# mcan1999/vulkan-raytracing

Measured on AMD Instinct MI355X. Metric: Mrays/sec (primary+secondary) at 1920×1080 depth 4; 1/2/4/8-GPU scaling, higher is better.
Workload: dtype f32

## Files before the change

vulkan_raytracing_amd/api.py:

```python
import ctypes as C

import numpy as np

from . import _native

HIT_DTYPE = np.dtype([("t", np.float32), ("u", np.float32), ("v", np.float32), ("prim", np.int32), ("inst", np.int32)])
MESH_RANGE_DTYPE = np.dtype([("first_float", np.uint64), ("first_index", np.uint64), ("prim_count", np.uint32), ("reserved", np.uint32)])
INSTANCE_DTYPE = np.dtype([("transform", np.float32, 12), ("custom_index_and_mask", np.uint32), ("sbt_offset_and_flags", np.uint32), ("mesh", np.uint64)])
UNIFORMS_DTYPE = np.dtype([("position", np.float32, 4), ("right", np.float32, 4), ("up", np.float32, 4), ("forward", np.float32, 4),
                           ("light_position", np.float32, 3), ("light_intensity", np.float32),
                           ("max_bounce_count", np.uint32), ("samples_per_pixel", np.uint32),
                           ("center_object_type", np.uint32), ("orbiting_object_type", np.uint32),
                           ("orbiting_object_primitive_offset", np.uint32), ("orbiting_object_vertex_offset", np.uint32)])
MATERIAL_DTYPE = np.dtype([("ka", np.float32, 3), ("ns", np.float32), ("kd", np.float32, 3), ("ni", np.float32), ("ks", np.float32, 3), ("type", np.uint32)])
MATERIAL_TYPE_OF_INSTANCE = 0xFFFFFFFF
assert MATERIAL_DTYPE.itemsize == 48
NODEQ_DTYPE = np.dtype([("w", np.uint32, 6), ("child", np.int32, 2)])
TRI_PACKET_DTYPE = np.dtype([("v0", np.float32, 3), ("e1", np.float32, 3), ("e2", np.float32, 3), ("prim", np.uint32), ("pad", np.uint32, 2)])
INSTANCE_DEV_DTYPE = np.dtype([("w2o", np.float32, 12), ("o2w", np.float32, 12), ("blas_root", np.int32), ("mask", np.uint32), ("custom_index", np.int32),
                               ("first_float", np.uint32), ("first_index", np.uint32), ("blas_root4", np.int32), ("q_lo", np.float32, 3), ("q_scale", np.float32, 3),
                               ("type", np.uint32), ("cover_first", np.uint32), ("cover_count", np.uint32), ("pad", np.uint32)])
TLAS_MESH_DTYPE = np.dtype([("blas_root", np.int32), ("blas_root4", np.int32), ("first_float", np.uint32), ("first_index", np.uint32),
                            ("cover_first", np.uint32), ("cover_count", np.uint32), ("prim_count", np.uint32), ("built", np.uint32), ("levels", np.int32),
                            ("q_lo", np.float32, 3), ("q_scale", np.float32, 3), ("lo", np.float32, 3), ("hi", np.float32, 3)])
# ... 225 lines not shown
    def set_uniforms(self, uniforms):
        u = np.ascontiguousarray(uniforms, UNIFORMS_DTYPE).reshape(1)
        self._chk(self.L.rt_set_uniforms(self.h, _p(u)), "rt_set_uniforms")

    def set_skybox(self, faces):
        faces = [np.ascontiguousarray(f, np.uint8) for f in faces]
        assert len(faces) == 6
        h, w = faces[0].shape[:2]
        arr = (C.c_void_p * 6)(*[f.ctypes.data for f in faces])
        self._chk(self.L.rt_set_skybox(self.h, arr, w, h), "rt_set_skybox")

    def trace(self, W, H, counting=False):
        out = np.zeros((H, W, 4), np.uint8 if getattr(self, "_rgba8", False) else np.float32)
        st = RtStats()
        fn = self.L.rt_trace_counting if counting else self.L.rt_trace
        self._chk(fn(self.h, W, H, _p(out), C.byref(st)), "rt_trace")
        return out, st

    def shard_rows(self, H, band_rows, shard, n_shards):
        return self.L.rt_shard_rows(H, band_rows, shard, n_shards)

    def trace_async(self, W, H):
        self._chk(self.L.rt_trace_async(self.h, W, H), "rt_trace_async")
        self._async_shape = (H, W, 4)

    def trace_wait(self, copy=True):
        px = C.c_void_p()
        st = RtStats()
        self._chk(self.L.rt_trace_wait(self.h, C.byref(px), C.byref(st)), "rt_trace_wait")
        H, W, _ = self._async_shape
        ct = C.c_uint8 if getattr(self, "_rgba8", False) else C.c_float
        img = np.ctypeslib.as_array(C.cast(px, C.POINTER(ct)), shape=(H, W, 4))
        return (img.copy() if copy else img), st

    def trace_shard(self, W, H, band_rows, shard, n_shards, d_out_ptr, capacity_bytes, stream_ptr=None):
        self._chk(self.L.rt_trace_shard(self.h, W, H, band_rows, shard, n_shards, C.c_void_p(d_out_ptr), capacity_bytes,
                                        C.c_void_p(stream_ptr) if stream_ptr else None), "rt_trace_shard")

    def set_batch(self, instances, uniforms, update=False):
        inst = np.ascontiguousarray(instances, INSTANCE_DTYPE)
        u = np.ascontiguousarray(uniforms, UNIFORMS_DTYPE).reshape(-1)
        K = len(u)
        inst = inst.reshape(K, -1)
        self._chk(self.L.rt_set_batch(self.h, K, _p(inst), inst.shape[1], _p(u), int(update)), "rt_set_batch")

    def trace_shard_batch(self, W, H, band_rows, shard, n_shards, d_out_ptr, capacity_bytes, stream_ptr=None, frame_stride_bytes=0):
        self._chk(self.L.rt_trace_shard_batch(self.h, W, H, band_rows, shard, n_shards, C.c_void_p(d_out_ptr), frame_stride_bytes, capacity_bytes,
                                              C.c_void_p(stream_ptr) if stream_ptr else None), "rt_trace_shard_batch")

    def assemble_shards(self, d_gathered_ptr, n_shards, shard_stride_bytes, W, H, band_rows, d_frame_ptr, capacity_bytes, stream_ptr=None):
        self._chk(self.L.rt_assemble_shards(self.h, C.c_void_p(d_gathered_ptr), n_shards, shard_stride_bytes, W, H, band_rows, C.c_void_p(d_frame_ptr),
                                            capacity_bytes, C.c_void_p(stream_ptr) if stream_ptr else None), "rt_assemble_shards")

    def synchronize(self):
        self._chk(self.L.rt_synchronize(self.h), "rt_synchronize")

    def stats(self):
        st = RtStats()
        self._chk(self.L.rt_get_stats(self.h, C.byref(st)), "rt_get_stats")
        return st

    def debug_snapshot(self):
        info = np.zeros(SNAPSHOT_INFO_WORDS, np.uint64)
        self._chk(self.L.rt_debug_snapshot(self.h, 0, _p(info), info.nbytes, None), "rt_debug_snapshot")
        i = [int(x) for x in info]

        def item(what, n, dtype):
            a = np.zeros(n, dtype)
            got = C.c_size_t(0)
            self._chk(self.L.rt_debug_snapshot(self.h, what, _p(a) if n else _p(np.zeros(1, np.uint8)), a.nbytes, C.byref(got)), "rt_debug_snapshot")
            assert got.value == a.nbytes, (what, got.value, a.nbytes)
            return a

        bits = info[12:18].astype(np.uint32).view(np.float32)
        return {"n_blas_nodes": i[0], "tlas_base": i[1], "tlas_node_count": i[2], "tlas_stride": i[3], "batch_k": i[4], "inst_per_frame": i[7],
                "tlas_q_lo": bits[:3].copy(), "tlas_q_scale": bits[3:].copy(),
                "blas_nodes": item(1, i[0], NODEQ_DTYPE), "tlas_nodes": item(2, i[18], NODEQ_DTYPE), "packets": item(3, i[5], TRI_PACKET_DTYPE),
                "instances": item(4, i[6], INSTANCE_DEV_DTYPE), "meshes": item(5, i[8], TLAS_MESH_DTYPE), "verts": item(6, i[9], np.float32),
                "idx": item(7, i[10], np.uint32), "cover_boxes": item(8, 6 * i[11], np.float32).reshape(-1, 6)}

    def set_timing(self, on):
        self._chk(self.L.rt_set_timing(self.h, int(on)), "rt_set_timing")

    def set_param(self, name, value):
        self._chk(self.L.rt_set_param(self.h, name.encode(), int(value)), "rt_set_param")
        if name in ("output_rgba8", "output_bgra8"):
            self._rgba8 = bool(value)

    def intersect(self, rays8, any_hit=False, counting=False):
        rays8 = np.ascontiguousarray(rays8, np.float32).reshape(-1, 8)
        out = np.zeros(len(rays8), HIT_DTYPE)
        st = RtStats()
        self._chk(self.L.rt_intersect(self.h, len(rays8), _p(rays8), int(any_hit), _p(out), int(counting), C.byref(st)), "rt_intersect")
        return out, st

    def intersect_device(self, rays, any_hit=False, attributes=False, stream=None, out=None):
        def call(run, hits, attr):
            return self.L.rt_intersect_device(self.h, rays.shape[0], C.c_void_p(rays.data_ptr()), int(any_hit), C.c_void_p(hits.data_ptr()),
                                              C.c_void_p(attr.data_ptr()) if attr is not None else None, C.c_void_p(run.cuda_stream))
        hits, attr = self._device_query(rays, attributes, stream, out, (), call, "rt_intersect_device")
        return RayQuery(hits, attr)

    def intersect_device_flags(self, rays, ray_flags=0, cull_mask=0xFF, words=None, attributes=False, stream=None, out=None):
        import torch
        n = rays.shape[0] if isinstance(rays, torch.Tensor) else 0
        if words is not None:
            if not isinstance(words, torch.Tensor):
                raise TypeError("words must be a torch tensor, got %s" % type(words).__name__)
            if words.dtype not in (torch.int32, getattr(torch, "uint32", torch.int32)):
                raise ValueError("words must be int32 or uint32, not %s" % words.dtype)
            if words.device != getattr(rays, "device", None) or not words.is_contiguous() or tuple(words.shape) != (n,):
                raise ValueError("words must be a contiguous (n,) tensor on the rays' device")

        def call(run, hits, attr):
            return self.L.rt_intersect_device_flags(self.h, n, C.c_void_p(rays.data_ptr()), C.c_void_p(words.data_ptr()) if words is not None and n else None,
                                                    int(ray_flags) & 0xFFFFFFFF, int(cull_mask) & 0xFFFFFFFF, C.c_void_p(hits.data_ptr()),
                                                    C.c_void_p(attr.data_ptr()) if attr is not None else None, C.c_void_p(run.cuda_stream))
        hits, attr = self._device_query(rays, attributes, stream, out, (words,), call, "rt_intersect_device_flags")
        return RayQuery(hits, attr, hit_kind=True)

    def closest_point_device(self, points, cull_mask=0xFF, attributes=False, stream=None, out=None):
        def call(run, hits, attr):
            return self.L.rt_closest_point_device(self.h, points.shape[0], C.c_void_p(points.data_ptr()), int(cull_mask) & 0xFFFFFFFF, C.c_void_p(hits.data_ptr()),
                                                  C.c_void_p(attr.data_ptr()) if attr is not None else None, C.c_void_p(run.cuda_stream))
        hits, attr = self._device_query(points, attributes, stream, out, (), call, "rt_closest_point_device", cols=4)
        return RayQuery(hits, attr, hit_kind=True)

    def closest_point(self, points4, cull_mask=0xFF, counting=False):
        points4 = np.ascontiguousarray(points4, np.float32).reshape(-1, 4)
        out = np.zeros(len(points4), HIT_DTYPE)
        st = RtStats()
        self._chk(self.L.rt_closest_point(self.h, len(points4), _p(points4), int(cull_mask) & 0xFFFFFFFF, _p(out), int(counting), C.byref(st)), "rt_closest_point")
        return out, st

    def sweep_spheres_device(self, sweeps, cull_mask=0xFF, attributes=False, stream=None, out=None):
        def call(run, hits, attr):
            return self.L.rt_sweep_spheres_device(self.h, sweeps.shape[0], C.c_void_p(sweeps.data_ptr()), int(cull_mask) & 0xFFFFFFFF, C.c_void_p(hits.data_ptr()),
                                                  C.c_void_p(attr.data_ptr()) if attr is not None else None, C.c_void_p(run.cuda_stream))
        self._check_rays(sweeps, "sweep_spheres_device", 8, "sweep")
        hits, attr = self._device_query(sweeps, attributes, stream, out, (), call, "rt_sweep_spheres_device")
        return RayQuery(hits, attr, hit_kind=True)

    def sweep_spheres(self, sweeps8, cull_mask=0xFF, counting=False):
        sweeps8 = np.ascontiguousarray(sweeps8, np.float32).reshape(-1, 8)
        out = np.zeros(len(sweeps8), HIT_DTYPE)
        st = RtStats()
        self._chk(self.L.rt_sweep_spheres(self.h, len(sweeps8), _p(sweeps8), int(cull_mask) & 0xFFFFFFFF, _p(out), int(counting), C.byref(st)), "rt_sweep_spheres")
        return out, st

    def point_inside_device(self, points, n_dirs=3, cull_mask=0xFF, counts=False, stream=None, out=None):
        import torch
        self._check_rays(points, "point_inside_device", 4, "point")
        k = int(n_dirs)
        if k not in (1, 3, 5):
            raise ValueError("n_dirs must be 1, 3 or 5, got %d" % k)
        n = points.shape[0]
        cur = torch.cuda.current_stream(points.device)
        if stream is None:
            stream = cur
        shapes = ((n,), (n, k) if counts else None)
        if out is None:
            bufs = [torch.empty(sh, dtype=torch.int32, device=points.device) if sh is not None else None for sh in shapes]
            if stream != cur:
                for t in bufs:
                    if t is not None:
                        t.record_stream(stream)
# ... 322 lines not shown
```

vulkan_raytracing_amd/csrc/kernels.hip:

```cpp
#include <hip/hip_runtime.h>

#include "rt_kernels.h"
#include "../../include/rt_api.h"

namespace rt {

struct F3 { float x, y, z; };
__device__ __forceinline__ F3 mk3(float x, float y, float z) { F3 r; r.x = x; r.y = y; r.z = z; return r; }
__device__ __forceinline__ F3 add3(F3 a, F3 b) { return mk3(a.x + b.x, a.y + b.y, a.z + b.z); }
__device__ __forceinline__ F3 sub3(F3 a, F3 b) { return mk3(a.x - b.x, a.y - b.y, a.z - b.z); }
__device__ __forceinline__ F3 mul3(F3 a, float s) { return mk3(a.x * s, a.y * s, a.z * s); }
__device__ __forceinline__ F3 neg3(F3 a) { return mk3(-a.x, -a.y, -a.z); }
__device__ __forceinline__ float dot3(F3 a, F3 b) { return __builtin_fmaf(a.z, b.z, __builtin_fmaf(a.y, b.y, a.x * b.x)); }
__device__ __forceinline__ F3 cross3(F3 a, F3 b) {
  return mk3(__builtin_fmaf(a.y, b.z, -(a.z * b.y)), __builtin_fmaf(a.z, b.x, -(a.x * b.z)), __builtin_fmaf(a.x, b.y, -(a.y * b.x)));
}
__device__ __forceinline__ float length3(F3 v) { return __builtin_sqrtf(dot3(v, v)); }
__device__ __forceinline__ F3 normalize3(F3 v) { float inv = 1.0f / length3(v); return mul3(v, inv); }
__device__ __forceinline__ F3 fma3(float s, F3 a, F3 b) { return mk3(__builtin_fmaf(s, a.x, b.x), __builtin_fmaf(s, a.y, b.y), __builtin_fmaf(s, a.z, b.z)); }
__device__ __forceinline__ F3 reflect3(F3 I, F3 N) { float k = 2.0f * dot3(N, I); return fma3(-k, N, I); }

__device__ __forceinline__ F3 xform_point(const float* m, F3 p) {
  return mk3(__builtin_fmaf(m[2], p.z, __builtin_fmaf(m[1], p.y, m[0] * p.x)) + m[3],
             __builtin_fmaf(m[6], p.z, __builtin_fmaf(m[5], p.y, m[4] * p.x)) + m[7],
// ... 216 lines not shown
  }
  return true;
}

__device__ __forceinline__ float div255(float x) {
  const float rc = 0x1.010102p-8f;
  const float q = x * rc;
  const float r = __builtin_fmaf(-q, 255.0f, x);
  return __builtin_fmaf(r, rc, q);
}

struct SkyTap { int layer, x, y; };
__device__ __forceinline__ SkyTap sky_neighbour(int layer, int x, int y, int W) {
  const int S = 2 * x + 1 - W, T = 2 * y + 1 - W;
  int px, py, pz;
  switch (layer) {
    case 0: px = W; py = -T; pz = -S; break;
    case 1: px = -W; py = -T; pz = S; break;
    case 2: px = S; py = W; pz = T; break;
    case 3: px = S; py = -W; pz = -T; break;
    case 4: px = S; py = -T; pz = W; break;
    default: px = -S; py = -T; pz = -W; break;
  }
  const int ax = abs(px), ay = abs(py), az = abs(pz);
  int nl, sc, tc, ma;
  if (az >= ax && az >= ay) { ma = az; if (pz >= 0) { nl = 4; sc = px; tc = -py; } else { nl = 5; sc = -px; tc = -py; } }
  else if (ay >= ax)        { ma = ay; if (py >= 0) { nl = 2; sc = px; tc = pz; } else { nl = 3; sc = px; tc = -pz; } }
  else                      { ma = ax; if (px >= 0) { nl = 0; sc = -pz; tc = -py; } else { nl = 1; sc = pz; tc = -py; } }
  SkyTap t;
  t.layer = nl; t.x = min(((sc + ma) * W) / (2 * ma), W - 1); t.y = min(((tc + ma) * W) / (2 * ma), W - 1);
  return t;
}
constexpr uint32_t SKY_CORNER = 0xFFFFFFFFu;
__device__ __noinline__ uint32_t sky_tap_index(int layer, int x, int y, int W, int H) {
  const bool ox = x < 0 || x >= W, oy = y < 0 || y >= H;
  SkyTap t; t.layer = layer; t.x = x; t.y = y;
  if (W != H) { t.x = max(0, min(x, W - 1)); t.y = max(0, min(y, H - 1)); }
  else if (ox && oy) return SKY_CORNER;
  else if (ox || oy) t = sky_neighbour(layer, x, y, W);
  return ((uint32_t)t.layer * (uint32_t)H + (uint32_t)t.y) * (uint32_t)W + (uint32_t)t.x;
}

__device__ __forceinline__ F3 sample_sky(const SceneDev& sc, F3 r) {
  if (sc.sky_w == 0) return mk3(0.f, 0.f, 0.f);
  const float ax = __builtin_fabsf(r.x), ay = __builtin_fabsf(r.y), az = __builtin_fabsf(r.z);
  int layer; float s, t, ma;
  if (az >= ax && az >= ay) { ma = az; if (r.z >= 0.f) { layer = 4; s = r.x; t = -r.y; } else { layer = 5; s = -r.x; t = -r.y; } }
  else if (ay >= ax)        { ma = ay; if (r.y >= 0.f) { layer = 2; s = r.x; t = r.z; } else { layer = 3; s = r.x; t = -r.z; } }
  else                      { ma = ax; if (r.x >= 0.f) { layer = 0; s = -r.z; t = -r.y; } else { layer = 1; s = r.z; t = -r.y; } }
  const float fs = 0.5f * (s / ma + 1.0f), ft = 0.5f * (t / ma + 1.0f);
  const float u = fs * (float)sc.sky_w - 0.5f, v = ft * (float)sc.sky_h - 0.5f;
  const float fu0 = __builtin_floorf(u), fv0 = __builtin_floorf(v);
  const float wu = u - fu0, wv = v - fv0;
  const int W = sc.sky_w, H = sc.sky_h;
  int x0 = (int)fu0, y0 = (int)fv0;
  x0 = max(-1, min(x0, W - 1)); y0 = max(-1, min(y0, H - 1));
  uint32_t i00 = ((uint32_t)layer * (uint32_t)H + (uint32_t)y0) * (uint32_t)W + (uint32_t)x0, i10 = i00 + 1u, i01 = i00 + (uint32_t)W, i11 = i01 + 1u;
  const bool edge = !(x0 >= 0 && x0 + 1 < W && y0 >= 0 && y0 + 1 < H);
  if (edge) {
    i00 = sky_tap_index(layer, x0, y0, W, H); i10 = sky_tap_index(layer, x0 + 1, y0, W, H);
    i01 = sky_tap_index(layer, x0, y0 + 1, W, H); i11 = sky_tap_index(layer, x0 + 1, y0 + 1, W, H);
  }
  auto tap = [&](uint32_t i) -> uchar4 {
    if (RT_NT_STREAMS & 4) { const uint32_t w = __builtin_nontemporal_load(reinterpret_cast<const uint32_t*>(sc.sky) + i); uchar4 r; r.x = w & 255u; r.y = (w >> 8) & 255u; r.z = (w >> 16) & 255u; r.w = w >> 24; return r; }
    return sc.sky[i];
  };
  const uchar4 a = tap(i00 == SKY_CORNER ? 0u : i00), b = tap(i10 == SKY_CORNER ? 0u : i10);
  const uchar4 c = tap(i01 == SKY_CORNER ? 0u : i01), d = tap(i11 == SKY_CORNER ? 0u : i11);
  float c00x = (float)a.x, c00y = (float)a.y, c00z = (float)a.z, c10x = (float)b.x, c10y = (float)b.y, c10z = (float)b.z;
  float c01x = (float)c.x, c01y = (float)c.y, c01z = (float)c.z, c11x = (float)d.x, c11y = (float)d.y, c11z = (float)d.z;
  if (edge) {
    if (i00 == SKY_CORNER) { c00x = ((c10x + c01x) + c11x) / 3.0f; c00y = ((c10y + c01y) + c11y) / 3.0f; c00z = ((c10z + c01z) + c11z) / 3.0f; }
    if (i10 == SKY_CORNER) { c10x = ((c01x + c11x) + c00x) / 3.0f; c10y = ((c01y + c11y) + c00y) / 3.0f; c10z = ((c01z + c11z) + c00z) / 3.0f; }
    if (i01 == SKY_CORNER) { c01x = ((c11x + c00x) + c10x) / 3.0f; c01y = ((c11y + c00y) + c10y) / 3.0f; c01z = ((c11z + c00z) + c10z) / 3.0f; }
    if (i11 == SKY_CORNER) { c11x = ((c00x + c10x) + c01x) / 3.0f; c11y = ((c00y + c10y) + c01y) / 3.0f; c11z = ((c00z + c10z) + c01z) / 3.0f; }
  }
  const float iu = 1.0f - wu, iv = 1.0f - wv;
  float ra = __builtin_fmaf(c10x, wu, c00x * iu), rb = __builtin_fmaf(c11x, wu, c01x * iu);
  float ga = __builtin_fmaf(c10y, wu, c00y * iu), gb = __builtin_fmaf(c11y, wu, c01y * iu);
  float ba = __builtin_fmaf(c10z, wu, c00z * iu), bb = __builtin_fmaf(c11z, wu, c01z * iu);
  return mk3(div255(__builtin_fmaf(rb, wv, ra * iv)), div255(__builtin_fmaf(gb, wv, ga * iv)), div255(__builtin_fmaf(bb, wv, ba * iv)));
}

__device__ __forceinline__ void store_pixel(const FrameDev& f, uint32_t p, float4 px) {
  if (f.out_rgba8) {
    auto q = [](float v) -> unsigned char { v = fminf(fmaxf(v, 0.0f), 1.0f); return (unsigned char)(v * 255.0f + 0.5f); };
    reinterpret_cast<uchar4*>(f.out)[p] = f.out_rgba8 == 2 ? make_uchar4(q(px.z), q(px.y), q(px.x), q(px.w)) : make_uchar4(q(px.x), q(px.y), q(px.z), q(px.w));
  } else {
    f.out[p] = px;
  }
}
constexpr float PIXEL_DONE = 2.0f;

__global__ __launch_bounds__(256) void k_cover(SceneDev sc, CoverViews views, uint32_t* mask_block) {
  const CoverArgs& a = views.v[blockIdx.z];
  uint32_t* const mask = mask_block + a.mask_offset;
  const InstanceDev* I = sc.inst + a.inst_base + blockIdx.y;
  const uint32_t b = blockIdx.x * blockDim.x + threadIdx.x;
  if (b >= I->cover_count || (I->mask & 0xFFu) == 0u) return;
  const float* bx = sc.cover_boxes + 6u * (size_t)(I->cover_first + b);
  float x0 = 3e38f, x1 = -3e38f, y0 = 3e38f, y1 = -3e38f, az_min = 3e38f;
  bool all = false;
#pragma unroll
  for (int k = 0; k < 8; k++) {
    const F3 p = mk3(bx[(k & 1) ? 3 : 0], bx[(k & 2) ? 4 : 1], bx[(k & 4) ? 5 : 2]);
    const F3 w = xform_point(I->o2w, p);
    const F3 v = mk3(w.x - a.cam[0], w.y - a.cam[1], w.z - a.cam[2]);
    const float ax = a.inv[0] * v.x + a.inv[1] * v.y + a.inv[2] * v.z;
    const float ay = a.inv[3] * v.x + a.inv[4] * v.y + a.inv[5] * v.z;
    const float az = a.inv[6] * v.x + a.inv[7] * v.y + a.inv[8] * v.z;
    if (!(az > 1e-20f)) { all = true; continue; }
    az_min = fminf(az_min, az);
    const float ux = a.kf * ax / az, uy = a.kf * ay / az;
    const float px = (ux + 1.0f) * 0.5f * (float)a.width, py = (1.0f - uy) * 0.5f * (float)a.height;
    if (!(__builtin_fabsf(px) < 1e9f) || !(__builtin_fabsf(py) < 1e9f)) { all = true; continue; }
    x0 = fminf(x0, px); x1 = fmaxf(x1, px); y0 = fminf(y0, py); y1 = fmaxf(y1, py);
  }
  if (!all) {
    float mx = 1.0f + 1e-4f * (__builtin_fabsf(x0) + __builtin_fabsf(x1)), my = 1.0f + 1e-4f * (__builtin_fabsf(y0) + __builtin_fabsf(y1));
    if (a.apex_radius > 0.0f) {
      if (!(az_min > 4.0f * a.apex_radius)) all = true;
      else {
        const float g = a.apex_radius / (az_min - a.apex_radius) * 1.01f;
        const float uxm = fmaxf(__builtin_fabsf(2.0f * x0 / (float)a.width - 1.0f), __builtin_fabsf(2.0f * x1 / (float)a.width - 1.0f));
        const float uym = fmaxf(__builtin_fabsf(2.0f * y0 / (float)a.height - 1.0f), __builtin_fabsf(2.0f * y1 / (float)a.height - 1.0f));
        mx += g * (a.kf + uxm) * 0.5f * (float)a.width; my += g * (a.kf + uym) * 0.5f * (float)a.height;
      }
    }
    const int ix0 = (int)floorf(x0 - mx), ix1 = (int)floorf(x1 + mx), iy0 = (int)floorf(y0 - my), iy1 = (int)floorf(y1 + my);
    if (ix1 < 0 || iy1 < 0 || ix0 >= a.width || iy0 >= a.height) return;
    const int tx0 = max(ix0, 0) >> 3, tx1 = min(ix1, a.width - 1) >> 3, ty0 = max(iy0, 0) >> 3, ty1 = min(iy1, a.height - 1) >> 3;
    if ((tx1 - tx0 + 1) * (ty1 - ty0 + 1) > COVER_MAX_TILES) all = true;
    else {
      for (int ty = ty0; ty <= ty1; ty++) {
        const uint32_t t0 = (uint32_t)(ty * a.tiles_x + tx0), t1 = (uint32_t)(ty * a.tiles_x + tx1);
        for (uint32_t w = t0 >> 5; w <= (t1 >> 5); w++) {
          const uint32_t lo = w == (t0 >> 5) ? (t0 & 31u) : 0u, hi = w == (t1 >> 5) ? (t1 & 31u) : 31u;
          const uint32_t bits = (hi == 31u ? 0xFFFFFFFFu : ((1u << (hi + 1u)) - 1u)) & ~((1u << lo) - 1u);
          __hip_atomic_fetch_or(mask + 1u + w, bits, __ATOMIC_RELAXED, __HIP_MEMORY_SCOPE_AGENT);
        }
      }
    }
  }
  if (all) atomicOr(mask, 1u);
}

constexpr int REF_DONE = (int)0x80000000;
constexpr int REF_MARK = (int)0x80000001;

struct Plane5 {
  float nx[5], ny[5], nz[5], d[5], slack[5];
  F3 qs, qb; uint3 rot;
};

__device__ __forceinline__ void beam_world(const EntryArgs& e, float ux0, float ux1, float uy0, float uy1, float wn[5][3], float wd[5], float wmag[5]) {
  const float* ia = e.inv; const float* ib = e.inv + 3; const float* ic = e.inv + 6;
#pragma unroll
  for (int k = 0; k < 3; k++) {
    wn[0][k] = e.kf * ia[k] - ux0 * ic[k];
    wn[1][k] = ux1 * ic[k] - e.kf * ia[k];
    wn[2][k] = e.kf * ib[k] - uy0 * ic[k];
    wn[3][k] = uy1 * ic[k] - e.kf * ib[k];
    wn[4][k] = ic[k];
  }
#pragma unroll
  for (int j = 0; j < 5; j++) {
    wd[j] = -(wn[j][0] * e.cam[0] + wn[j][1] * e.cam[1] + wn[j][2] * e.cam[2]);
    wmag[j] = __builtin_fabsf(wn[j][0] * e.cam[0]) + __builtin_fabsf(wn[j][1] * e.cam[1]) + __builtin_fabsf(wn[j][2] * e.cam[2]);
  }
}
__device__ __forceinline__ void beam_fold(const float wn[5][3], const float wd[5], const float wmag[5], float apex_radius, const float* m, const float* q_lo, const float* q_scale, Plane5& P) {
#pragma unroll
  for (int j = 0; j < 5; j++) {
// ... 166 lines not shown
    const int wi = s_xw[grp][i]; const float ki = s_xk[grp][i];
    if (wi != ENTRY_FREE) { nb++; if (w != ENTRY_FREE && (ki < key || (ki == key && (uint32_t)i < sub))) rank++; }
  }
  if (!work) return;
  if (nb == 0) inst = ENTRY_NO_INST;
  if (nb == 0 && n_rest == 0) { if (sub == 0u) rec->w[0] = (int)ENTRY_EMPTY; return; }
  if (nb > 0) {
    if (w != ENTRY_FREE) rec->w[rank == 0 ? 1 : 2 + n_rest + 1 + (nb - 1 - rank)] = w;
    if (sub == 0u) {
#pragma unroll
      for (int i = 0; i < ENTRY_TLAS_CAP; i++) if (i < n_rest) rec->w[2 + (n_rest - 1 - i)] = rest[i];
      rec->w[2 + n_rest] = REF_MARK;
      rec->w[0] = (int)((uint32_t)(n_rest + nb) | ((uint32_t)(n_rest + 1) << 4) | (inst << 8));
    }
  } else if (sub == 0u) {
    rec->w[1] = rest[0];
#pragma unroll
    for (int i = 1; i < ENTRY_TLAS_CAP; i++) if (i < n_rest) rec->w[2 + (n_rest - 1 - i)] = rest[i];
    rec->w[0] = (int)((uint32_t)(n_rest - 1) | ((uint32_t)(n_rest - 1) << 4) | (ENTRY_NO_INST << 8));
  }
}

__device__ __forceinline__ float2 sample_uv(uint32_t x, uint32_t y, uint32_t i, uint32_t spp, int width, int height) {
  const float fx = (float)x, fy = (float)y;
  const float seed0 = (float)(spp + i), seed1 = seed0 + 0.5f;
  float ux = (fx + jitter_hash(fx, fy, seed0)) / (float)width;
  float uy = (fy + jitter_hash(fx, fy, seed1)) / (float)height;
  ux = __builtin_fmaf(ux, 2.0f, -1.0f);
  uy = -__builtin_fmaf(uy, 2.0f, -1.0f);
  return make_float2(ux, uy);
}
__device__ __forceinline__ uint32_t frame_row(const FrameDev& f, uint32_t ly) {
  if (f.n_shards == 1) return ly;
  const uint32_t band = ly / (uint32_t)f.band_rows, within = ly - band * (uint32_t)f.band_rows;
  return (band * (uint32_t)f.n_shards + (uint32_t)f.shard) * (uint32_t)f.band_rows + within;
}
__device__ __forceinline__ size_t jitter_index(uint32_t tile, uint32_t i, uint32_t spp, uint32_t lane) { return ((size_t)tile * spp + i) * 64u + lane; }

__device__ __forceinline__ bool tile_is_sky(const FrameDev& f, uint32_t fi, uint32_t tx, uint32_t by, uint32_t rec) {
  if (f.cover != nullptr) {
    const uint32_t* const cover = f.cover + (size_t)fi * f.cover_view_words;
    if (cover[0] == 0u) {
      uint32_t fty = by;
      if (f.n_shards != 1) {
        const uint32_t tiles_per_band = (uint32_t)f.band_rows >> 3;
        const uint32_t band = by / tiles_per_band, sub = by - band * tiles_per_band;
        fty = (band * (uint32_t)f.n_shards + (uint32_t)f.shard) * tiles_per_band + sub;
      }
      const uint32_t t = fty * (uint32_t)f.cover_tiles_x + tx;
      if (((cover[1u + (t >> 5)] >> (t & 31u)) & 1u) == 0u) return true;
    }
  }
  return f.entry != nullptr && (uint32_t)f.entry[rec].w[0] == ENTRY_EMPTY;
}

__global__ __launch_bounds__(256) void k_jitter_table(FrameDev f, uint32_t spp, float2* table) {
  const uint32_t lane = threadIdx.x;
  const uint32_t i = blockIdx.z * blockDim.y + threadIdx.y;
  const uint32_t x = blockIdx.x * 8u + (lane & 7u), ly = blockIdx.y * 8u + (lane >> 3);
  if (i >= spp) return;
  float2 uv = make_float2(0.f, 0.f);
  if (x < (uint32_t)f.width && ly < (uint32_t)f.rows) uv = sample_uv(x, frame_row(f, ly), i, spp, f.width, f.height);
  table[jitter_index(blockIdx.y * gridDim.x + blockIdx.x, i, spp, lane)] = uv;
}

__global__ __launch_bounds__(256) void k_raygen(SceneDev sc, FrameDev f, UniformsDev u, BatchTab bt) {
  const uint32_t spp = u.samples_per_pixel;
  const uint32_t lane = threadIdx.x;
  const uint32_t i = blockIdx.z * blockDim.y + threadIdx.y;
  const uint32_t x = blockIdx.x * 8u + (lane & 7u);
  uint32_t fi = 0, by = blockIdx.y;
  if (f.batch_k > 1) { const uint32_t tile_rows1 = ((uint32_t)f.rows + 7u) >> 3; fi = blockIdx.y / tile_rows1; by = blockIdx.y - fi * tile_rows1; }
  const uint32_t npx1 = (uint32_t)(f.rows * f.width);
  const uint32_t ly = by * 8u + (lane >> 3);
  const bool live = i < spp && x < (uint32_t)f.width && ly < (uint32_t)f.rows;
  const uint32_t tile = blockIdx.y * gridDim.x + blockIdx.x;
  const uint32_t tile1 = by * gridDim.x + blockIdx.x;
  const bool covered = !tile_is_sky(f, fi, blockIdx.x, by, tile);
  __shared__ float4 s_col[4][64];
  if (!covered) {
    F3 right = mk3(u.right[0], u.right[1], u.right[2]), up = mk3(u.up[0], u.up[1], u.up[2]), fwd = mk3(u.forward[0], u.forward[1], u.forward[2]);
    if (f.batch_k > 1) { right = mk3(bt.right[fi][0], bt.right[fi][1], bt.right[fi][2]); up = mk3(bt.up[fi][0], bt.up[fi][1], bt.up[fi][2]); fwd = mk3(bt.forward[fi][0], bt.forward[fi][1], bt.forward[fi][2]); }
    const uint32_t fy = frame_row(f, ly);
    const float nn = (float)spp;
    float r = 0.f, g = 0.f, b = 0.f, al = 0.f;
    if (gridDim.z == 1u) {
      float4 col = make_float4(0.f, 0.f, 0.f, 0.f);
      if (live) {
        const float2 uv = f.jitter != nullptr ? f.jitter[jitter_index(tile1, i, spp, lane)] : sample_uv(x, fy, i, spp, f.width, f.height);
        const F3 d = normalize3(fma3(2.5f, fwd, fma3(uv.y, up, mul3(right, uv.x))));
        const F3 c = sample_sky(sc, mk3(d.x, d.y, -d.z));
        col = make_float4(c.x, c.y, c.z, 1.0f);
      }
      s_col[threadIdx.y][lane] = col;
      __syncthreads();
      if (threadIdx.y != 0u || !live) return;
      for (uint32_t w = 0; w < blockDim.y; w++) { const float4 c = s_col[w][lane]; r += c.x; g += c.y; b += c.z; al += c.w; }
    } else {
      if (threadIdx.y != 0u || blockIdx.z != 0u || x >= (uint32_t)f.width || ly >= (uint32_t)f.rows) return;
      for (uint32_t k = 0; k < spp; k++) {
        const float2 uv = f.jitter != nullptr ? f.jitter[jitter_index(tile1, k, spp, lane)] : sample_uv(x, fy, k, spp, f.width, f.height);
        const F3 d = normalize3(fma3(2.5f, fwd, fma3(uv.y, up, mul3(right, uv.x))));
        const F3 c = sample_sky(sc, mk3(d.x, d.y, -d.z));
        r += c.x; g += c.y; b += c.z; al += 1.0f;
      }
    }
    store_pixel(f, fi * f.out_frame_stride + ly * (uint32_t)f.width + x, make_float4(r / nn, g / nn, b / nn, al / nn));
    return;
  }
#ifdef RT_ALT_KERNELS
  if (f.tile_blob != nullptr && covered && f.tile_blob[tile] != BLOB_NONE) return;
#endif
  bool survive = false;
  F3 d = mk3(0.f, 0.f, 1.f);
  uint32_t sid = 0;
  float4 miss_col = make_float4(0.f, 0.f, 0.f, 0.f);
  if (live) {
    const float2 uv = f.jitter != nullptr ? f.jitter[jitter_index(tile1, i, spp, lane)] : sample_uv(x, frame_row(f, ly), i, spp, f.width, f.height);
    const float ux = uv.x, uy = uv.y;
    F3 right = mk3(u.right[0], u.right[1], u.right[2]), up = mk3(u.up[0], u.up[1], u.up[2]), fwd = mk3(u.forward[0], u.forward[1], u.forward[2]);
    if (f.batch_k > 1) { right = mk3(bt.right[fi][0], bt.right[fi][1], bt.right[fi][2]); up = mk3(bt.up[fi][0], bt.up[fi][1], bt.up[fi][2]); fwd = mk3(bt.forward[fi][0], bt.forward[fi][1], bt.forward[fi][2]); }
    d = normalize3(fma3(2.5f, fwd, fma3(uy, up, mul3(right, ux))));
    sid = (fi * spp + i) * npx1 + ly * (uint32_t)f.width + x;
    {
      const F3 o = f.batch_k > 1 ? mk3(bt.position[fi][0], bt.position[fi][1], bt.position[fi][2]) : mk3(u.position[0], u.position[1], u.position[2]);
      F3 qs, qb; uint3 rot;
      quant_space(o, d, sc.tlas_q_lo, sc.tlas_q_scale, qs, qb, rot);
      const bool far = f.far_possible != 0 && quant_far(qs, qb);
      const uint4* rp = reinterpret_cast<const uint4*>(sc.blas_nodes + sc.tlas_root + (int)fi * sc.tlas_stride);
      const uint4 Q0 = rp[0], Q1 = rp[1];
      float tn;
      const bool h0 = far || slab_q(Q0.x, Q0.y, Q0.z, qs, qb, rot, 0.001f, 10000.0f, tn);
      const bool h1 = (far || slab_q(Q0.w, Q1.x, Q1.y, qs, qb, rot, 0.001f, 10000.0f, tn)) && Q1.w != Q1.z;
      const int c0 = (int)Q1.z, c1 = (int)Q1.w;
      survive = (h0 && c0 < 0) || (h1 && c1 < 0);
#pragma unroll
      for (int k = 0; k < 2; k++) {
        const int ch = k ? c1 : c0;
        if ((k ? h1 : h0) && ch >= 0 && !survive) {
          const uint4* np = reinterpret_cast<const uint4*>(sc.blas_nodes + ch);
          const uint4 N0 = np[0], N1 = np[1];
          survive = far || slab_q(N0.x, N0.y, N0.z, qs, qb, rot, 0.001f, 10000.0f, tn) || slab_q(N0.w, N1.x, N1.y, qs, qb, rot, 0.001f, 10000.0f, tn);
        }
      }
    }
    if (!survive) {
      const F3 c = sample_sky(sc, mk3(d.x, d.y, -d.z));
      miss_col = make_float4(c.x, c.y, c.z, 1.0f);
    }
  }
  const bool missed = live && !survive;
  const bool fuse = gridDim.z == 1u;
  __shared__ unsigned long long s_miss[4];
  if (fuse) {
    s_col[threadIdx.y][lane] = miss_col;
    const uint64_t mm = __ballot(missed);
    if (lane == 0) s_miss[threadIdx.y] = mm;
  } else if (missed) st_stream(&f.sample_color[sid], miss_col);
  const uint32_t shard = (blockIdx.x + gridDim.x * (blockIdx.y + gridDim.y * blockIdx.z)) & (N_SHARDS - 1);
  __shared__ uint32_t s_run[5];
  const uint64_t smask = __ballot(survive);
  if (lane == 0) s_run[threadIdx.y] = (uint32_t)__builtin_popcountll(smask);
  __syncthreads();
  if (threadIdx.x == 0 && threadIdx.y == 0) {
    uint32_t tot = 0;
    for (uint32_t w = 0; w < blockDim.y; w++) { const uint32_t c = s_run[w]; s_run[w] = tot; tot += c; }
    if (f.pixel_runs && tot) {
      const uint32_t run = 64u * blockDim.y;
      __hip_atomic_fetch_add(f.counters + cnt_tail(Q_DEAD, (int)shard), run - tot, __ATOMIC_RELAXED, __HIP_MEMORY_SCOPE_AGENT);
      tot = run;
    }
    s_run[4] = tot ? atomicAdd(f.counters + cnt_tail(0, (int)shard), tot) : 0u;
    if (f.pixel_runs && tot) {
      const F3 o = f.batch_k > 1 ? mk3(bt.position[fi][0], bt.position[fi][1], bt.position[fi][2]) : mk3(u.position[0], u.position[1], u.position[2]);
      f.ray_o[0][shard * f.shard_cap + s_run[4]] = make_float4(o.x, o.y, o.z, f.entry != nullptr ? __uint_as_float(tile) : 10000.0f);
    }
    s_run[0] = f.pixel_runs ? tot : s_run[0];
  }
  __syncthreads();
  const bool run_tile = f.pixel_runs && s_run[0] != 0u;
  const uint32_t slot = f.pixel_runs ? s_run[4] + 64u * threadIdx.y + lane : s_run[4] + s_run[threadIdx.y] + prefix_rank(smask);
  if (fuse) {
    bool all = true;
    for (uint32_t w = 0; w < blockDim.y; w++) all = all && ((s_miss[w] >> lane) & 1ull) != 0ull;
    if (all) {
      if (threadIdx.y == 0) {
        float r = 0.f, g = 0.f, b = 0.f, al = 0.f;
        for (uint32_t w = 0; w < blockDim.y; w++) { const float4 c = s_col[w][lane]; r += c.x; g += c.y; b += c.z; al += c.w; }
        const float nn = (float)spp;
        const uint32_t p = ly * (uint32_t)f.width + x;
        store_pixel(f, fi * f.out_frame_stride + p, make_float4(r / nn, g / nn, b / nn, al / nn));
        st_stream(&f.sample_color[fi * spp * npx1 + p], make_float4(0.f, 0.f, 0.f, PIXEL_DONE));
      }
    } else if (missed) st_stream(&f.sample_color[sid], miss_col);
  }
  if (survive || run_tile) {
    const uint32_t v = shard * f.shard_cap + slot;
    if (!f.pixel_runs) {
      const F3 o = f.batch_k > 1 ? mk3(bt.position[fi][0], bt.position[fi][1], bt.position[fi][2]) : mk3(u.position[0], u.position[1], u.position[2]);
      st_stream(&f.ray_o[0][v], make_float4(o.x, o.y, o.z, f.entry != nullptr ? __uint_as_float(tile) : 10000.0f));
    }
    st_stream(&f.ray_d[0][v], survive ? make_float4(d.x, d.y, d.z, __uint_as_float(sid)) : make_float4(0.f, 0.f, 0.f, __uint_as_float(SID_DEAD)));
  }
}

struct TraceArgs {
  SceneDev sc;
  const float4* ray_o;
  const float4* ray_d;
  const uint32_t* tails;
  uint32_t* work;
  uint32_t shard_cap;
  float4* hit_a;
  int32_t* hit_inst;
  const float4* sh_c;
  float4* sample_color;
  HitRec* raw_out;
  int32_t* ovf_stack;
  uint32_t* counters;
  union {
    float tmin;
    uint32_t query_word;
  };
  uint32_t rays_per_lane;
  uint32_t min_blocks;
  const EntryRec* entry;
  union {
    const uint32_t* sh_e;
    const uint32_t* ray_words;
  };
};

constexpr int MODE_CLOSEST = 0;
constexpr int MODE_SHADOW = 1;
constexpr int MODE_QUERY = 3;
constexpr int MODE_QUERY_FLAGS = 4;


#ifndef RT_REFILL_MIN
#define RT_REFILL_MIN 16
#endif
#ifndef RT_KEEP_NUM
#define RT_KEEP_NUM 5
#endif
#ifndef RT_INTERIOR_UNROLL
#define RT_INTERIOR_UNROLL 2
#endif
#ifndef RT_WIDE_UNROLL
#define RT_WIDE_UNROLL 1
#endif
#ifndef RT_WAVES_PER_EU
#define RT_WAVES_PER_EU 5
#endif
#ifndef RT_LEAF_CHAIN
#define RT_LEAF_CHAIN 1
#endif
#ifndef RT_STACK2_LDS
#define RT_STACK2_LDS 12
#endif
constexpr int STACK2_LDS = RT_STACK2_LDS;
constexpr uint32_t REFILL_MIN = RT_REFILL_MIN;

#ifdef RT_EXP_PHASE_SEL
#define PH_BEGIN(k) uint64_t ph_b##k = 0; if (COUNT && RT_EXP_PHASE_SEL == k) ph_b##k = __builtin_readcyclecounter();
#define PH_END(k) if (COUNT && RT_EXP_PHASE_SEL == k && lane == 0) { diag_iters++; diag_busy += __builtin_readcyclecounter() - ph_b##k; }
#else
#define PH_BEGIN(k)
#define PH_END(k)
#endif

template <int MODE, bool ANY, bool COUNT, bool WIDE, bool ENTRY = false, bool FAR = true, bool CONT = false>
__device__ __forceinline__ void trace_body(const TraceArgs& a) {
  constexpr bool RAYS8 = MODE == MODE_QUERY || MODE == MODE_QUERY_FLAGS;
  constexpr bool QF = MODE == MODE_QUERY_FLAGS;
  __shared__ int s_stack[4][STACK2_LDS + 1][64];
  __shared__ float4 s_rays[4][2][64];
  __shared__ float4 s_out[4][64];
  __shared__ int2 s_outq[4][64];
  __shared__ uint32_t s_ent[((ENTRY && MODE == MODE_SHADOW) || QF) ? 4 : 1][64];
  __shared__ float4 s_inst[LDS_INSTANCES ? LDS_INSTANCES : 1][5];
  {
    uint32_t total = 0;
#pragma unroll
    for (int t = 0; t < N_SHARDS; t++) total += ld_cursor(a.tails + t * CNT_STRIDE);
    uint32_t want = (total + 256u * a.rays_per_lane - 1u) / (256u * a.rays_per_lane);
    want = (want + (N_SHARDS - 1)) & ~(uint32_t)(N_SHARDS - 1);
    if (want < a.min_blocks) want = a.min_blocks;
    if (blockIdx.x >= want) return;
  }
  const int n_lds_inst = a.sc.n_inst < LDS_INSTANCES ? a.sc.n_inst : LDS_INSTANCES;
  if ((int)threadIdx.x < n_lds_inst) {
    const InstanceDev* I = a.sc.inst + threadIdx.x;
    const float4* mp = reinterpret_cast<const float4*>(I->w2o);
    s_inst[threadIdx.x][0] = mp[0]; s_inst[threadIdx.x][1] = mp[1]; s_inst[threadIdx.x][2] = mp[2];
    s_inst[threadIdx.x][3] = make_float4(I->q_lo[0], I->q_lo[1], I->q_lo[2], __int_as_float(I->blas_root));
    s_inst[threadIdx.x][4] = make_float4(I->q_scale[0], I->q_scale[1], I->q_scale[2], __uint_as_float(I->mask));
  }
  __syncthreads();
  const uint32_t lane = threadIdx.x & 63u, wave = threadIdx.x >> 6;
  int* const stk = &s_stack[wave][0][lane];
  int32_t* const ovf = a.ovf_stack + (size_t)(blockIdx.x * 256u + threadIdx.x) * a.sc.ovf_stride;
  uint64_t cnt_nodes = 0, cnt_tris = 0, diag_iters = 0, diag_busy = 0;
  const uint64_t diag_t0 = COUNT ? __builtin_readcyclecounter() : 0;

  uint32_t shard = blockIdx.x & (N_SHARDS - 1), tried = 0;
  uint32_t pf_base = 0, pf_count = 0;
  float4 pf_o = make_float4(0, 0, 0, 0), pf_d = pf_o;
  uint32_t pf_e = ENTRY_FROM_ROOT;
  uint32_t chunk_base = 0, chunk_count = 0, chunk_pos = 0;
  auto prefetch = [&]() {
    pf_count = 0;
    while (tried < (uint32_t)N_SHARDS) {
      const uint32_t size = ld_cursor(a.tails + shard * CNT_STRIDE);
      uint32_t off = 0;
      if (lane == 0 && size) off = atomicAdd(a.work + shard * CNT_STRIDE, 64u);
      off = (uint32_t)__builtin_amdgcn_readfirstlane((int)off);
      if (size && off < size) { pf_base = shard * a.shard_cap + off; pf_count = (size - off) < 64u ? (size - off) : 64u; break; }
      shard = (shard + 1u) & (N_SHARDS - 1); tried++;
    }
    if (lane < pf_count) {
      if constexpr (RAYS8) {
        const size_t r = 2u * (size_t)(pf_base + lane);
        pf_o = ld_stream(&a.ray_o[r]); pf_d = ld_stream(&a.ray_o[r + 1u]);
        if (QF) {
          const uint32_t w = a.ray_words ? (uint32_t)ld_stream(reinterpret_cast<const int*>(a.ray_words) + pf_base + lane) : 0xFF000000u;
          pf_e = ((a.query_word | w) & QF_FLAGS) | (a.query_word & w & 0xFF000000u);
        }
      } else {
        pf_o = ld_stream(&a.ray_o[pf_base + lane]); pf_d = ld_stream(&a.ray_d[pf_base + lane]);
      }
      if (ENTRY && MODE == MODE_SHADOW) pf_e = (uint32_t)ld_stream(reinterpret_cast<const int*>(a.sh_e) + pf_base + lane);
    }
  };
  auto promote = [&]() {
    s_rays[wave][0][lane] = pf_o; s_rays[wave][1][lane] = pf_d;
    if ((ENTRY && MODE == MODE_SHADOW) || QF) s_ent[wave][lane] = pf_e;
    chunk_base = pf_base; chunk_count = pf_count; chunk_pos = 0;
    prefetch();
  };
  prefetch();
  promote();

  uint32_t out_count = 0;
  auto flush = [&]() {
    if (lane < out_count) {
      const float4 r = s_out[wave][lane];
      const int2 k = s_outq[wave][lane];
      if (MODE == MODE_CLOSEST) { st_stream(&a.hit_a[k.x], r); st_stream(&a.hit_inst[k.x], k.y); }
      else if (MODE == MODE_SHADOW) {
        float cr = 0.08f, cg = 0.24f, cb = 0.08f;
        if (r.x != 0.0f || a.sc.n_materials != 0) {
          const float4 shc = ld_stream(&a.sh_c[(uint32_t)k.y]);
          if (r.x != 0.0f) { cr = shc.x; cg = shc.y; cb = shc.z; }
          else { const F3 amb = ambient_of(a.sc, __float_as_uint(shc.w)); cr = amb.x; cg = amb.y; cb = amb.z; }
        }
        st_stream(&a.sample_color[(uint32_t)k.x], make_float4(cr, cg, cb, 1.0f));
      }
      else { HitRec h; h.t = r.x; h.u = r.y; h.v = r.z; h.prim = (int)__float_as_uint(r.w); h.inst = k.y; a.raw_out[k.x] = h; }
    }
    out_count = 0;
  };

  bool need = true;
  uint32_t q = 0, sid = 0;
  float tmin_ray = 0.f, tmax = 0.f;
  uint32_t qword = 0;
  F3 wo = mk3(0, 0, 0), wd = mk3(0, 0, 1), co = wo, cd = wd, qs = mk3(1, 1, 1), qb = mk3(0, 0, 0);
  uint3 rot = make_uint3(0u, 0u, 0u);
  bool far = false;
  float best_t = 0.f, best_u = 0.f, best_v = 0.f;
  int best_prim = -1, best_inst = -1, cur_inst = -1, sp = 0, cur = REF_DONE;
  const char* const node_bytes = WIDE ? reinterpret_cast<const char*>(a.sc.wide_nodes) : reinterpret_cast<const char*>(a.sc.blas_nodes);

  auto push = [&](int v) {
    if (sp < STACK2_LDS) stk[sp * 64] = v;
    else *reinterpret_cast<volatile int32_t*>(ovf + (sp - STACK2_LDS)) = v;
    sp++;
  };
  auto pop = [&]() {
    sp--;
    if (sp < STACK2_LDS) cur = stk[sp * 64];
    else cur = *reinterpret_cast<volatile int32_t*>(ovf + (sp - STACK2_LDS));
  };

  auto to_instance = [&](int ii, int& root, uint32_t& imask) {
    float4 m0, m1, m2, ql, qsc;
    if (ii < n_lds_inst) { m0 = s_inst[ii][0]; m1 = s_inst[ii][1]; m2 = s_inst[ii][2]; ql = s_inst[ii][3]; qsc = s_inst[ii][4]; }
    else {
      const InstanceDev* I = a.sc.inst + ii;
      const float4* mp = reinterpret_cast<const float4*>(I->w2o);
      m0 = mp[0]; m1 = mp[1]; m2 = mp[2];
      ql = make_float4(I->q_lo[0], I->q_lo[1], I->q_lo[2], __int_as_float(I->blas_root));
      qsc = make_float4(I->q_scale[0], I->q_scale[1], I->q_scale[2], __uint_as_float(I->mask));
    }
    root = __float_as_int(ql.w); imask = __float_as_uint(qsc.w);
    if ((imask & 0xFFu) != 0u) {
      float m[12];
      m[0] = m0.x; m[1] = m0.y; m[2] = m0.z; m[3] = m0.w; m[4] = m1.x; m[5] = m1.y; m[6] = m1.z; m[7] = m1.w;
      m[8] = m2.x; m[9] = m2.y; m[10] = m2.z; m[11] = m2.w;
      co = xform_point(m, wo); cd = xform_vec(m, wd);
      const float qlo3[3] = {ql.x, ql.y, ql.z}, qsc3[3] = {qsc.x, qsc.y, qsc.z};
      quant_space(co, cd, qlo3, qsc3, qs, qb, rot); far = FAR && quant_far_o(co, qlo3, qsc3);
    }
  };

  for (;;) {
    PH_BEGIN(5)
    const uint64_t need_mask = __ballot(need);
    const uint32_t n_need = (uint32_t)__builtin_popcountll(need_mask);
    if (n_need >= REFILL_MIN || n_need == 64u) {
      if (chunk_pos == chunk_count && pf_count > 0) promote();
      if (chunk_pos < chunk_count) {
        const uint32_t rank = prefix_rank(need_mask);
        const uint32_t avail = chunk_count - chunk_pos;
        if (need && rank < avail) {
          const uint32_t ci = chunk_pos + rank;
          q = chunk_base + ci;
          const float4 ro = s_rays[wave][0][ci], rd = s_rays[wave][1][ci];
          if (RAYS8) { tmin_ray = ro.w; tmax = rd.w; }
          else { tmax = ro.w; sid = __float_as_uint(rd.w); }
          if (QF) qword = s_ent[wave][ci];
          wo = mk3(ro.x, ro.y, ro.z); wd = mk3(rd.x, rd.y, rd.z);
          co = wo; cd = wd;
          cur_inst = -1;
          stk[0] = REF_DONE;
          bool handed_on = false;
          if (CONT && (__float_as_uint(ro.w) & CONT_FLAG) != 0u) {
            handed_on = true;
            const uint32_t ent = __float_as_uint(ro.w);
            const uint32_t tile = ent & 0xFFFFFFu, mask = (ent >> 24) & 15u;
            const int4* rp = reinterpret_cast<const int4*>(a.entry + tile);
            const int4 r0 = rp[0], r1 = rp[1];
            const uint32_t n_rest = (((uint32_t)r0.x >> 4) & 15u) - 1u;
            const int wk[4] = {r0.z, r0.w, r1.x, r1.y};
            sp = 1;
#pragma unroll
            for (uint32_t k = 0; k < 4u; k++)
              if (k < n_rest && ((mask >> (n_rest - 1u - k)) & 1u) != 0u) { stk[sp * 64] = wk[k]; sp++; }
            sp--; cur = stk[sp * 64];
// ... 232 lines not shown
      } else {
        push(REF_MARK);
        cur_inst = ii; cur = root;
      }
    }

    PH_END(3)
    PH_BEGIN(4)
    const bool fin = !need && cur == REF_DONE;
    const uint64_t fin_mask = __ballot(fin);
    if (fin_mask != 0) {
      const uint32_t n_fin = (uint32_t)__builtin_popcountll(fin_mask);
      if (out_count + n_fin > 64u) flush();
      if (fin) {
        const uint32_t slot = out_count + prefix_rank(fin_mask);
        if (MODE == MODE_SHADOW) {
          s_out[wave][slot].x = best_inst < 0 ? 1.0f : 0.0f;
          s_outq[wave][slot] = make_int2((int)sid, (int)q);
        } else {
          s_out[wave][slot] = make_float4(best_t, best_u, best_v, __uint_as_float((uint32_t)best_prim));
          s_outq[wave][slot] = make_int2((int)q, best_inst);
        }
        need = true;
      }
      out_count += n_fin;
    }
    PH_END(4)
  }
  if (COUNT) {
    for (int off = 32; off > 0; off >>= 1) {
      cnt_nodes += __shfl_down((unsigned long long)cnt_nodes, off);
      cnt_tris += __shfl_down((unsigned long long)cnt_tris, off);
    }
    if (lane == 0) {
      const int off = ANY ? (CNT_NODE_VISITS_SH - CNT_NODE_VISITS) : 0;
      atomicAdd(reinterpret_cast<unsigned long long*>(a.counters + CNT_NODE_VISITS + off), (unsigned long long)cnt_nodes);
      atomicAdd(reinterpret_cast<unsigned long long*>(a.counters + CNT_TRI_TESTS + off), (unsigned long long)cnt_tris);
      const int dg = ANY ? CNT_DIAG_SH : CNT_DIAG;
      atomicAdd(reinterpret_cast<unsigned long long*>(a.counters + dg), (unsigned long long)diag_iters);
      atomicAdd(reinterpret_cast<unsigned long long*>(a.counters + dg + 2), (unsigned long long)diag_busy);
      atomicAdd(reinterpret_cast<unsigned long long*>(a.counters + dg + 4), (unsigned long long)(__builtin_readcyclecounter() - diag_t0));
    }
  }
}

template <int MODE, bool ANY, bool WIDE, bool ENTRY = false, bool FAR = true, bool CONT = false>
__global__ __launch_bounds__(256) __attribute__((amdgpu_waves_per_eu(RT_WAVES_PER_EU, RT_WAVES_PER_EU))) void k_trace(TraceArgs a) { trace_body<MODE, ANY, false, WIDE, ENTRY, FAR, CONT>(a); }
template <int MODE, bool ANY, bool WIDE, bool ENTRY = false, bool FAR = true, bool CONT = false>
__global__ __launch_bounds__(256) void k_trace_count(TraceArgs a) { trace_body<MODE, ANY, true, WIDE, ENTRY, FAR, CONT>(a); }

#ifdef RT_ALT_KERNELS
#include "kernels_alt.inc"
#include "kernels_tile.inc"
#endif

struct ShadeArgs {
  SceneDev sc;
  FrameDev f;
  UniformsDev u;
  int bounce;
  BatchTab bt;
};

struct Surface { F3 P, N; };
__device__ __forceinline__ Surface hit_surface(const SceneDev& sc, const InstanceDev* I, uint32_t prim, float hu, float hv) {
  const uint32_t* ix = sc.idx + I->first_index + 3u * prim;
  const uint32_t ia = ix[0], ib = ix[1], ic = ix[2];
  const float* vb = sc.verts + I->first_float;
  const float bx = (1.0f - hu) - hv, by = hu, bz = hv;
  const float* pa = vb + 6u * ia; const float* pb = vb + 6u * ib; const float* pc = vb + 6u * ic;
  const F3 pos = fma3(bz, mk3(pc[0], pc[1], pc[2]), fma3(by, mk3(pb[0], pb[1], pb[2]), mul3(mk3(pa[0], pa[1], pa[2]), bx)));
  const F3 nrm = fma3(bz, mk3(pc[3], pc[4], pc[5]), fma3(by, mk3(pb[3], pb[4], pb[5]), mul3(mk3(pa[3], pa[4], pa[5]), bx)));
  Surface s;
  s.P = xform_point(I->o2w, pos);
  s.N = normalize3(xform_normal(I->w2o, nrm));
  return s;
}

template <bool PIN> __device__ __forceinline__ float4 ambient_default() {
  float r = 0.08f;
  if constexpr (PIN) asm volatile("" : "+v"(r));
  return make_float4(r, 0.24f, r, 1.0f);
}
template <bool TILE, bool BATCH, bool RUNS, bool REG, typename A>
__device__ __forceinline__ void shade_slot(const A& a, const int bounce, const uint32_t shard, const uint32_t q, const bool in_range, const int inst_r, const float4 h_r) {
  const auto& f = a.f;
  const auto& U = a.u;
  const int cur = bounce & 1, nxt = cur ^ 1;
  const uint32_t lane = threadIdx.x & 63u;
  bool push_next = false, push_shadow = false, settled = false;
  F3 no = mk3(0, 0, 0), nd = mk3(0, 0, 1);
  float sh_tmax = 0.f; F3 sh_c = mk3(0, 0, 0); float sh_w = 0.f;
  uint32_t sh_ent = ENTRY_FROM_ROOT;
  uint32_t sid = SID_DEAD;
  int inst = HIT_DEAD;
  if (in_range) { if constexpr (REG) inst = inst_r; else inst = ld_stream(&f.hit_inst[q]); }
  if (inst != HIT_DEAD) {
    const float4 rd = ld_stream(&f.ray_d[cur][q]);
    sid = __float_as_uint(rd.w);
    const F3 d = mk3(rd.x, rd.y, rd.z);
    if (inst < 0) {
      const F3 c = sample_sky(a.sc, mk3(d.x, d.y, -d.z));
      st_stream(&f.sample_color[sid], make_float4(c.x, c.y, c.z, 1.0f));
    } else {
      float4 h = h_r;
      if constexpr (!REG) h = ld_stream(&f.hit_a[q]);
      const InstanceDev* I = a.sc.inst + inst;
      const uint32_t prim = __float_as_uint(h.w);
      const Surface S = hit_surface(a.sc, I, prim, h.y, h.z);
      const F3 P = S.P;
      F3 N = S.N;
      const int objectIndex = I->custom_index;
      uint32_t type = I->type != TYPE_BY_OBJECT_INDEX ? I->type : (objectIndex == 0 ? U.center_object_type : U.orbiting_object_type);
      const MaterialDev* M = nullptr;
      uint32_t mat = MATERIAL_NONE;
      if (a.sc.n_materials != 0) {
        mat = a.sc.prim_material[I->first_index / 3u + prim];
        M = a.sc.materials + mat;
        if (M->type != TYPE_BY_INSTANCE) type = M->type;
      }
      const bool last = (uint32_t)bounce >= U.max_bounce_count;
      if (type == 0u) {
        if (dot3(d, N) >= 0.0f) {
          st_stream(&f.sample_color[sid], ambient_default<REG>());
        } else {
          no = fma3(0.01f, N, P);
          F3 light = mk3(U.light_position[0], U.light_position[1], U.light_position[2]);
          float Iv = U.light_intensity;
          uint32_t fi = 0;
          if constexpr (BATCH) { fi = frame_of(sid, a.sc.batch_samples); light = mk3(a.bt.light[fi][0], a.bt.light[fi][1], a.bt.light[fi][2]); Iv = a.bt.light[fi][3]; }
          const F3 toL = sub3(light, P);
          const float dist = length3(toL);
          const F3 L = mul3(toL, 1.0f / dist);
          const F3 Hh = normalize3(add3(L, neg3(d)));
          const float NdotL = dot3(N, L), NdotH = dot3(N, Hh);
          const float dl = fmaxf(0.0f, NdotL);
          const float sp = M ? pow_int(fmaxf(0.0f, NdotH), (uint32_t)M->ns) : pow100(fmaxf(0.0f, NdotH));
          const uint32_t i = sid / (uint32_t)(f.rows * f.width) - fi * U.samples_per_pixel;
          float w = 1.0f;
          for (uint32_t k = 0; k < i; k++) w = w * 0.9f;
          const F3 kd = M ? mk3(M->kd[0], M->kd[1], M->kd[2]) : mk3(0.2f, 1.0f, 0.2f);
          const F3 ks = M ? mk3(M->ks[0], M->ks[1], M->ks[2]) : mk3(0.8f, 0.8f, 0.8f);
          const F3 diff = mk3((Iv * kd.x) * dl, (Iv * kd.y) * dl, (Iv * kd.z) * dl);
          const F3 spec = mk3((Iv * ks.x) * sp, (Iv * ks.y) * sp, (Iv * ks.z) * sp);
          const F3 amb = ambient_of(a.sc, mat);
          sh_c = fma3(w, add3(diff, spec), amb); sh_w = __uint_as_float(mat);
          nd = L; sh_tmax = dist;
          push_shadow = true;
          if (f.settle_dead_shadow_rays && __float_as_uint(sh_c.x) == __float_as_uint(amb.x) && __float_as_uint(sh_c.y) == __float_as_uint(amb.y) &&
              __float_as_uint(sh_c.z) == __float_as_uint(amb.z)) {
            st_stream(&f.sample_color[sid], make_float4(amb.x, amb.y, amb.z, 1.0f));
            push_shadow = false; settled = true;
          }
          if (f.light_entry != nullptr) {
            const F3 v = sub3(no, light);
            const float ax = __builtin_fabsf(v.x), ay = __builtin_fabsf(v.y), az = __builtin_fabsf(v.z);
            const int axis = (ax >= ay && ax >= az) ? 0 : (ay >= az ? 1 : 2);
            const float vc = axis == 0 ? v.x : (axis == 1 ? v.y : v.z), va = axis == 0 ? v.y : (axis == 1 ? v.z : v.x), vb = axis == 0 ? v.z : (axis == 1 ? v.x : v.y);
            const float c = __builtin_fabsf(vc);
            if (c > 0.0f) {
              const float T8 = (float)(8 * f.light_tiles);
              const float px = (va / c + 1.0f) * 0.5f * T8, py = (1.0f - vb / c) * 0.5f * T8;
              const int tx = min(max((int)(px * 0.125f), 0), f.light_tiles - 1), ty = min(max((int)(py * 0.125f), 0), f.light_tiles - 1);
              const int face = 2 * axis + (vc < 0.0f ? 1 : 0);
              sh_ent = (uint32_t)((face * f.light_tiles + ty) * f.light_tiles + tx) | (NdotL < 0.0f ? ENTRY_REVERSE : 0u);
            }
          }
        }
      } else if (type == 1u) {
        no = fma3(0.01f, N, P);
        nd = reflect3(d, N);
        push_next = true;
      } else if (type == 2u) {
        float ndoti = dot3(d, N);
        const bool outwards = ndoti > 0.0f;
        if (outwards) { N = neg3(N); ndoti = -ndoti; }
        const float ratio = M ? (outwards ? M->ni : 1.0f / M->ni) : (outwards ? 1.52f : (1.0f / 1.52f));
        const float k = 1.0f - (ratio * ratio) * (1.0f - ndoti * ndoti);
        if (k < 0.0f) { nd = reflect3(d, N); no = fma3(0.01f, N, P); }
        else {
          const float c = __builtin_fmaf(ratio, ndoti, __builtin_sqrtf(k));
          nd = normalize3(fma3(-c, N, mul3(d, ratio)));
          no = fma3(-0.01f, N, P);
        }
        push_next = true;
      } else {
        if (bounce == 0 && f.pixel_runs) {
          no = mk3(U.position[0], U.position[1], U.position[2]);
          if constexpr (BATCH) { const uint32_t fk = frame_of(sid, a.sc.batch_samples); no = mk3(a.bt.position[fk][0], a.bt.position[fk][1], a.bt.position[fk][2]); }
        } else {
          const float4 ro = ld_stream(&f.ray_o[cur][q]);
          no = mk3(ro.x, ro.y, ro.z);
        }
        nd = d; push_next = true;
      }
      if (push_next && last) {
        push_next = false;
        st_stream(&f.sample_color[sid], ambient_default<REG>());
      }
    }
  }
  {
    const uint64_t m_st = __ballot(settled);
    if (lane == 0 && m_st != 0ull) {
      __hip_atomic_fetch_add(f.counters + cnt_tail(Q_SHADOW0, (int)shard), (uint32_t)__builtin_popcountll(m_st), __ATOMIC_RELAXED, __HIP_MEMORY_SCOPE_AGENT);
      __hip_atomic_fetch_add(f.counters + cnt_work(Q_DEAD, (int)shard), (uint32_t)__builtin_popcountll(m_st), __ATOMIC_RELAXED, __HIP_MEMORY_SCOPE_AGENT);
    }
  }
  const uint32_t slot_n = wave_alloc(push_next, f.counters + cnt_tail(bounce + 1, (int)shard));
  if (push_next) {
    const uint32_t v = shard * f.shard_cap + slot_n;
    st_stream(&f.ray_o[nxt][v], make_float4(no.x, no.y, no.z, 10000.0f));
    st_stream(&f.ray_d[nxt][v], make_float4(nd.x, nd.y, nd.z, __uint_as_float(sid)));
  }
  if constexpr (RUNS) {
    if (in_range) {
      if (push_shadow) {
        st_stream(&f.sh_o[q], make_float4(no.x, no.y, no.z, sh_tmax));
        st_stream(&f.sh_c[q], make_float4(sh_c.x, sh_c.y, sh_c.z, sh_w));
        if (f.sh_e != nullptr) f.sh_e[q] = sh_ent;
      }
      st_stream(&f.sh_d[q], push_shadow ? make_float4(nd.x, nd.y, nd.z, __uint_as_float(sid)) : make_float4(0.f, 0.f, 0.f, __uint_as_float(SID_DEAD)));
    }
    const uint64_t m_sh = __ballot(push_shadow);
    if (lane == 0 && m_sh != 0ull) __hip_atomic_fetch_add(f.counters + cnt_tail(Q_SHADOW0, (int)shard), (uint32_t)__builtin_popcountll(m_sh), __ATOMIC_RELAXED, __HIP_MEMORY_SCOPE_AGENT);
  } else {
    const uint32_t slot_s = wave_alloc(push_shadow, f.counters + cnt_tail(Q_SHADOW, (int)shard));
    if (push_shadow) {
      const uint32_t v = f.sh_base + shard * f.shard_cap + slot_s;
      st_stream(&f.sh_o[v], make_float4(no.x, no.y, no.z, sh_tmax));
      st_stream(&f.sh_d[v], make_float4(nd.x, nd.y, nd.z, __uint_as_float(sid)));
      st_stream(&f.sh_c[v], make_float4(sh_c.x, sh_c.y, sh_c.z, sh_w));
      if (f.sh_e != nullptr) f.sh_e[v] = sh_ent;
    }
  }
}

template <bool TILE = false, bool BATCH = false, bool RUNS = false>
__device__ __forceinline__ void shade_body(const ShadeArgs& a, const int bounce) {
  const FrameDev& f = a.f;
  const UniformsDev& U = a.u;
  const uint32_t lane = threadIdx.x & 63u, wave = threadIdx.x >> 6;
  const int n_pass = TILE ? 2 : 1;
  for (int pass = 0; pass < n_pass; pass++) {
  uint32_t cnt[N_SHARDS], maxb = 0;
#pragma unroll
  for (int t = 0; t < N_SHARDS; t++) {
    if (TILE && pass) {
      uint32_t blobs = 0;
#pragma unroll
      for (int k = 0; k < BLOB_CLASSES; k++) blobs += ld_cursor(f.counters + cnt_tail(Q_BLOB_LIST + k, t));
      cnt[t] = blobs * (256u * ((U.samples_per_pixel + 3u) / 4u));
    } else cnt[t] = ld_cursor(f.counters + cnt_tail(bounce, t));
    maxb = max(maxb, (cnt[t] + 63u) >> 6);
  }
  const uint32_t n_waves = gridDim.x * 4u;
  for (uint32_t g = blockIdx.x * 4u + wave; g < maxb * N_SHARDS; g += n_waves) {
    const uint32_t shard = g & (N_SHARDS - 1), base = (g >> 3) << 6;
    uint32_t n = 0;
#pragma unroll
    for (int t = 0; t < N_SHARDS; t++) n = (shard == (uint32_t)t) ? cnt[t] : n;
    if (base >= n) continue;
    const uint32_t q = shard * f.shard_cap + ((TILE && pass) ? f.shard_cap - n : 0u) + base + lane;
    shade_slot<TILE, BATCH, RUNS, false>(a, bounce, shard, q, base + lane < n, HIT_DEAD, make_float4(0.f, 0.f, 0.f, 0.f));
  }
  }
}

template <bool TILE, bool BATCH, bool RUNS = false>
__global__ __launch_bounds__(256) void k_shade(ShadeArgs a) { shade_body<TILE, BATCH, RUNS>(a, a.bounce); }

#include "kernels_beam.inc"

struct TailArgs {
  TraceArgs tr;
  ShadeArgs sh;
  uint32_t first_bounce;
  uint32_t* barrier;
  uint32_t* fault;
};

__device__ __forceinline__ void grid_barrier(uint32_t* bar, uint32_t* fault, uint32_t& phase) {
  __syncthreads();
  phase++;
  if (threadIdx.x == 0) {
    __threadfence();
    const uint32_t target = phase * gridDim.x;
    __hip_atomic_fetch_add(bar, 1u, __ATOMIC_RELAXED, __HIP_MEMORY_SCOPE_AGENT);
    uint32_t spins = 0;
    while (__hip_atomic_load(bar, __ATOMIC_RELAXED, __HIP_MEMORY_SCOPE_AGENT) < target) {
      __builtin_amdgcn_s_sleep(8);
      if (++spins > (1u << 24)) { __hip_atomic_store(fault, 1u, __ATOMIC_RELAXED, __HIP_MEMORY_SCOPE_AGENT); break; }
    }
    __threadfence();
  }
  __syncthreads();
}

template <bool COUNT, bool WIDE, bool BATCH = false>
__global__ __launch_bounds__(256) void k_tail(TailArgs t) {
  uint32_t phase = 0;
  const uint32_t max_bounce = t.sh.u.max_bounce_count;
  for (uint32_t b = t.first_bounce; b <= max_bounce; b++) {
    uint32_t live = 0;
#pragma unroll
    for (int k = 0; k < N_SHARDS; k++) live += ld_cursor(t.tr.counters + cnt_tail((int)b, k));
    if (live == 0 || ld_cursor(t.fault) != 0u) break;
    TraceArgs a = t.tr;
    a.ray_o = t.sh.f.ray_o[b & 1u]; a.ray_d = t.sh.f.ray_d[b & 1u];
    a.tails = t.tr.counters + cnt_tail((int)b, 0);
    a.work = t.tr.counters + cnt_work((int)b, 0);
    trace_body<MODE_CLOSEST, false, COUNT, WIDE>(a);
    grid_barrier(t.barrier, t.fault, phase);
    if (ld_cursor(t.fault) != 0u) return;
    shade_body<false, BATCH>(t.sh, (int)b);
    grid_barrier(t.barrier, t.fault, phase);
    if (ld_cursor(t.fault) != 0u) return;
  }
}

__global__ __launch_bounds__(256) void k_resolve(FrameDev f, UniformsDev u) {
  const uint32_t npx1 = (uint32_t)(f.rows * f.width);
  const uint32_t lane = threadIdx.x & 63u, wave = (uint32_t)__builtin_amdgcn_readfirstlane((int)(threadIdx.x >> 6));
  const uint32_t tile_rows1 = ((uint32_t)f.rows + 7u) >> 3;
  const uint32_t trow = blockIdx.y * 4u + wave;
  if (trow < tile_rows1 * (uint32_t)f.batch_k) {
    const uint32_t fi = f.batch_k > 1 ? trow / tile_rows1 : 0u, by = trow - fi * tile_rows1;
    const uint32_t x = blockIdx.x * 8u + (lane & 7u), ly = by * 8u + (lane >> 3);
    if (!tile_is_sky(f, fi, blockIdx.x, by, trow * gridDim.x + blockIdx.x) && x < (uint32_t)f.width && ly < (uint32_t)f.rows) {
      const uint32_t p1 = ly * (uint32_t)f.width + x;
      const size_t s0 = (size_t)fi * u.samples_per_pixel * npx1 + p1;
      if (f.sample_color[s0].w != PIXEL_DONE) {
        float r = 0.f, g = 0.f, b = 0.f, al = 0.f;
        for (uint32_t i = 0; i < u.samples_per_pixel; i++) {
          const float4 c = ld_stream(&f.sample_color[s0 + (size_t)i * npx1]);
          r += c.x; g += c.y; b += c.z; al += c.w;
        }
        const float nn = (float)u.samples_per_pixel;
        store_pixel(f, fi * f.out_frame_stride + p1, make_float4(r / nn, g / nn, b / nn, al / nn));
      }
    }
  }
  const uint32_t p = (blockIdx.y * gridDim.x + blockIdx.x) * blockDim.x + threadIdx.x, n_threads = gridDim.x * gridDim.y * blockDim.x;
  if (f.counters_next)
    for (uint32_t i = p; i < (uint32_t)CNT_WORDS; i += n_threads) f.counters_next[i] = 0u;
  if (f.cover_next)
    for (uint32_t i = p; i < f.cover_words; i += n_threads) f.cover_next[i] = 0u;
  if (blockIdx.x == 0 && blockIdx.y == 0 && f.stats_out) {
    __shared__ unsigned long long s_q[N_QUEUES];
    const uint32_t t = threadIdx.x;
    if (t < (uint32_t)N_QUEUES) {
      unsigned long long n = 0;
      for (int k = 0; k < N_SHARDS; k++) n += ld_cursor(f.counters + cnt_tail((int)t, k));
      s_q[t] = n;
    }
    __syncthreads();
    if (f.hint && t >= 1u && t < (uint32_t)CNT_MAX_BOUNCES)
      __hip_atomic_store(f.hint + t, (uint32_t)(s_q[t] > 0xFFFFFFFFull ? 0xFFFFFFFFull : s_q[t]), __ATOMIC_RELAXED, __HIP_MEMORY_SCOPE_SYSTEM);
    auto cnt64 = [&](int word) { return (unsigned long long)ld_cursor(f.counters + word) | ((unsigned long long)ld_cursor(f.counters + word + 1) << 32); };
    if (t < (uint32_t)STAT_WORDS) {
      unsigned long long v = 0;
      if (t == STAT_QUEUE0) { v = s_q[0] + s_q[Q_TILE_RAYS] - s_q[Q_DEAD]; for (int k = 0; k < N_SHARDS; k++) v -= ld_cursor(f.counters + cnt_work(Q_TILE_RAYS, k)); }
      else if (t == STAT_TILE_RAYS) v = s_q[Q_TILE_RAYS];
      else if (t == STAT_CONT_RAYS) { for (int k = 0; k < N_SHARDS; k++) v += ld_cursor(f.counters + cnt_work(Q_TILE_RAYS, k)); }
      else if (t >= STAT_BLOB && t < STAT_BLOB + 5) v = ld_cursor(f.counters + CNT_BLOB_STATS + (int)(t - STAT_BLOB));
      else if (t >= STAT_TILE_DIAG && t < STAT_TILE_DIAG + 6) v = cnt64(CNT_TILE_DIAG + 2 * (int)(t - STAT_TILE_DIAG));
      else if (t == STAT_SECONDARY) { for (uint32_t b = 1; b <= u.max_bounce_count && b < (uint32_t)CNT_MAX_BOUNCES; b++) v += s_q[b]; }
      else if (t == STAT_SHADOW) v = s_q[Q_SHADOW] + s_q[Q_SHADOW0];
      else if (t == STAT_SHADOW_UNTRACED) { for (int k = 0; k < N_SHARDS; k++) v += ld_cursor(f.counters + cnt_work(Q_DEAD, k)); }
      else if (t == STAT_QUEUE1) v = s_q[1];
      else if (t == STAT_FAULT) v = ld_cursor(f.counters + CNT_FAULT);
      else if (t == STAT_FAULT_TOTAL) {
        uint32_t total = f.fault_total ? f.fault_total[0] : 0u;
        if (f.fault_total && ld_cursor(f.counters + CNT_FAULT) != 0u) { total++; f.fault_total[0] = total; }
        v = total;
      }
      else if (t == STAT_NODE_VISITS) v = cnt64(CNT_NODE_VISITS);
      else if (t == STAT_TRI_TESTS) v = cnt64(CNT_TRI_TESTS);
      else if (t == STAT_NODE_VISITS_SH) v = cnt64(CNT_NODE_VISITS_SH);
      else if (t == STAT_TRI_TESTS_SH) v = cnt64(CNT_TRI_TESTS_SH);
      else if (t >= STAT_DIAG && t < STAT_DIAG + 3) v = cnt64(CNT_DIAG + 2 * (int)(t - STAT_DIAG));
      else if (t >= STAT_DIAG + 3 && t < STAT_DIAG + 6) v = cnt64(CNT_DIAG_SH + 2 * (int)(t - STAT_DIAG - 3));
      __hip_atomic_store(f.stats_out + t, v, __ATOMIC_RELAXED, __HIP_MEMORY_SCOPE_SYSTEM);
    }
  }
}

int trace_threads_per_block() { return 256; }

static dim3 raygen_grid(int width, int rows, uint32_t spp, int batch_k, dim3& block) {
  const uint32_t wpb = spp < 4u ? spp : 4u;
  block = dim3(64, wpb);
  return dim3(((uint32_t)width + 7u) >> 3, (((uint32_t)rows + 7u) >> 3) * (uint32_t)batch_k, (spp + wpb - 1u) / wpb);
}
size_t raygen_block_count(int width, int rows, uint32_t spp, int batch_k) {
  dim3 b; const dim3 g = raygen_grid(width, rows, spp, batch_k, b);
  return (size_t)g.x * g.y * g.z;
}
void launch_raygen(const SceneDev& sc, const FrameDev& f, const UniformsDev& u, const BatchTab& bt, hipStream_t s) {
  dim3 b; const dim3 g = raygen_grid(f.width, f.rows, u.samples_per_pixel, f.batch_k, b);
  hipLaunchKernelGGL(k_raygen, g, b, 0, s, sc, f, u, bt);
}
size_t jitter_table_elems(int width, int rows, uint32_t spp) {
  return (size_t)(((uint32_t)width + 7u) >> 3) * (size_t)(((uint32_t)rows + 7u) >> 3) * spp * 64u;
}
void launch_jitter_table(const FrameDev& f, uint32_t spp, float2* table, hipStream_t s) {
  dim3 b; const dim3 g = raygen_grid(f.width, f.rows, spp, 1, b);
  hipLaunchKernelGGL(k_jitter_table, g, b, 0, s, f, spp, table);
}

void launch_cover(const SceneDev& sc, const CoverViews& a, uint32_t max_boxes_per_instance, uint32_t* mask_block, hipStream_t s) {
  if (a.n <= 0 || a.v[0].n_inst <= 0 || max_boxes_per_instance == 0) return;
  hipLaunchKernelGGL(k_cover, dim3((max_boxes_per_instance + 255u) / 256u, (unsigned)a.v[0].n_inst, (unsigned)a.n), dim3(256), 0, s, sc, a, mask_block);
}

static TraceArgs make_args(const SceneDev& sc, uint32_t* counters, int queue, uint32_t shard_cap, int32_t* ovf) {
  TraceArgs a{};
  a.sc = sc;
  a.tmin = 0.001f;
  a.counters = counters;
  a.tails = counters + cnt_tail(queue, 0);
  a.work = counters + cnt_work(queue, 0);
// ... 16 lines not shown
  }
  if (cfg.variant == 1) {
    if (counting) hipLaunchKernelGGL((k_trace4<MODE, ANY, true>), g, b, 0, s, a);
    else hipLaunchKernelGGL((k_trace4<MODE, ANY, false>), g, b, 0, s, a);
    return;
  }
#endif
  if (counting) hipLaunchKernelGGL((k_trace_count<MODE, ANY, false>), g, b, 0, s, a);
  else if constexpr (MODE == MODE_QUERY) hipLaunchKernelGGL((k_trace<MODE, ANY, false, false, true>), g, b, 0, s, a);
  else if (cfg.far) hipLaunchKernelGGL((k_trace<MODE, ANY, false, false, true>), g, b, 0, s, a);
  else hipLaunchKernelGGL((k_trace<MODE, ANY, false, false, false>), g, b, 0, s, a);
}

bool alt_kernels_built() {
#ifdef RT_ALT_KERNELS
  return true;
#else
  return false;
#endif
}

void launch_trace_closest(const SceneDev& sc, const FrameDev& f, int bounce, bool counting, const LaunchCfg& cfg, hipStream_t s) {
  TraceArgs a = make_args(sc, f.counters, bounce, f.shard_cap, f.ovf_stack);
  a.ray_o = f.ray_o[bounce & 1]; a.ray_d = f.ray_d[bounce & 1];
  a.hit_a = f.hit_a; a.hit_inst = f.hit_inst;
#ifdef RT_ALT_KERNELS
  if (bounce == 0 && cfg.packet != 0 && cfg.variant == 0) {
    a.entry = f.entry;
    a.rays_per_lane = (uint32_t)cfg.rays_per_lane; a.min_blocks = (uint32_t)cfg.min_blocks;
    const dim3 g(cfg.packet_blocks), b(256);
    if (f.entry != nullptr) {
      if (counting) hipLaunchKernelGGL((k_packet<MODE_CLOSEST, false, true, true>), g, b, 0, s, a);
      else hipLaunchKernelGGL((k_packet<MODE_CLOSEST, false, false, true>), g, b, 0, s, a);
    } else {
      if (counting) hipLaunchKernelGGL((k_packet<MODE_CLOSEST, false, true, false>), g, b, 0, s, a);
      else hipLaunchKernelGGL((k_packet<MODE_CLOSEST, false, false, false>), g, b, 0, s, a);
    }
    return;
  }
#endif
  if (bounce == 0 && f.pixel_runs && cfg.variant == 0) {
    a.entry = f.entry;
    const dim3 g(cfg.trace_blocks), b(256);
    if (counting) hipLaunchKernelGGL(k_beam_count, g, b, 0, s, a, (uint32_t)f.pixel_runs);
    else hipLaunchKernelGGL(k_beam, g, b, 0, s, a, (uint32_t)f.pixel_runs);
    return;
  }
  if (bounce == 0 && f.entry != nullptr && cfg.variant == 0) {
    a.entry = f.entry;
    a.rays_per_lane = (uint32_t)cfg.rays_per_lane; a.min_blocks = (uint32_t)cfg.min_blocks;
    const dim3 g(cfg.trace_blocks), b(256);
#ifdef RT_ALT_KERNELS
    if (f.tile_blob != nullptr) {
      if (counting) hipLaunchKernelGGL((k_trace_count<MODE_CLOSEST, false, false, true, false, true>), g, b, 0, s, a);
      else hipLaunchKernelGGL((k_trace<MODE_CLOSEST, false, false, true, false, true>), g, b, 0, s, a);
      return;
    }
#endif
    if (counting) hipLaunchKernelGGL((k_trace_count<MODE_CLOSEST, false, false, true>), g, b, 0, s, a);
    else if (cfg.far) hipLaunchKernelGGL((k_trace<MODE_CLOSEST, false, false, true, true>), g, b, 0, s, a);
    else hipLaunchKernelGGL((k_trace<MODE_CLOSEST, false, false, true, false>), g, b, 0, s, a);
    return;
  }
  launch_trace<MODE_CLOSEST, false>(a, counting, cfg, s);
}

void launch_beam_shade(const SceneDev& sc, const FrameDev& f, const UniformsDev& u, const LaunchCfg& cfg, hipStream_t s) {
  BeamShadeArgs a{};
  a.sc = sc;
  a.ray_o = f.ray_o[0]; a.ray_d = f.ray_d[0];
  a.tails = f.counters + cnt_tail(0, 0); a.work = f.counters + cnt_work(0, 0);
  a.shard_cap = f.shard_cap; a.ovf_stack = f.ovf_stack; a.counters = f.counters;
  a.tmin = 0.001f;
  a.entry = f.entry;
  a.next_o = f.ray_o[1]; a.next_d = f.ray_d[1];
  a.sh_o = f.sh_o; a.sh_d = f.sh_d; a.sh_c = f.sh_c; a.sh_e = f.sh_e;
  a.sample_color = f.sample_color;
  a.light_entry = f.light_entry;
  a.width = f.width; a.rows = f.rows; a.light_tiles = f.light_tiles; a.settle_dead_shadow_rays = f.settle_dead_shadow_rays;
  for (int k = 0; k < 3; k++) { a.u.position[k] = u.position[k]; a.u.light_position[k] = u.light_position[k]; }
  a.u.light_intensity = u.light_intensity;
  a.u.max_bounce_count = u.max_bounce_count; a.u.samples_per_pixel = u.samples_per_pixel;
  a.u.center_object_type = u.center_object_type; a.u.orbiting_object_type = u.orbiting_object_type;
  hipLaunchKernelGGL(k_beam_shade, dim3(cfg.trace_blocks), dim3(256), 0, s, a, (uint32_t)f.pixel_runs);
}

void launch_entry(const SceneDev& sc, const EntryViews& a, hipStream_t s) {
  uint32_t n = 0;
  for (int v = 0; v < a.n; v++) n = max(n, (uint32_t)(a.v[v].tiles_x * a.v[v].tile_rows));
  if (n == 0) return;
  hipLaunchKernelGGL(k_entry, dim3((n + 7u) / 8u, (unsigned)a.n), dim3(64), 0, s, sc, a);
}

void launch_trace_shadow(const SceneDev& sc, const FrameDev& f, bool counting, const LaunchCfg& cfg, hipStream_t s) {
  TraceArgs a = make_args(sc, f.counters, Q_SHADOW, f.shard_cap, f.ovf_stack);
  a.ray_o = f.sh_o + f.sh_base; a.ray_d = f.sh_d + f.sh_base; a.sh_c = f.sh_c + f.sh_base;
  a.sample_color = f.sample_color;
#ifdef RT_ALT_KERNELS
  if (cfg.packet != 0 && cfg.variant == 0) {
    const bool le = f.light_entry != nullptr && f.sh_e != nullptr;
    a.entry = le ? f.light_entry : nullptr; a.sh_e = le ? f.sh_e + f.sh_base : nullptr;
    a.rays_per_lane = (uint32_t)cfg.rays_per_lane; a.min_blocks = (uint32_t)cfg.min_blocks;
    const dim3 g(cfg.packet_blocks), b(256);
    if (le) {
      if (counting) hipLaunchKernelGGL((k_packet<MODE_SHADOW, true, true, true>), g, b, 0, s, a);
      else hipLaunchKernelGGL((k_packet<MODE_SHADOW, true, false, true>), g, b, 0, s, a);
    } else {
      if (counting) hipLaunchKernelGGL((k_packet<MODE_SHADOW, true, true, false>), g, b, 0, s, a);
      else hipLaunchKernelGGL((k_packet<MODE_SHADOW, true, false, false>), g, b, 0, s, a);
    }
    return;
  }
#endif
  if (f.light_entry != nullptr && f.sh_e != nullptr && cfg.variant == 0) {
    a.entry = f.light_entry; a.sh_e = f.sh_e + f.sh_base;
    a.rays_per_lane = (uint32_t)cfg.rays_per_lane; a.min_blocks = (uint32_t)cfg.min_blocks;
    const dim3 g(cfg.trace_blocks), b(256);
    if (counting) hipLaunchKernelGGL((k_trace_count<MODE_SHADOW, true, false, true>), g, b, 0, s, a);
    else if (cfg.far) hipLaunchKernelGGL((k_trace<MODE_SHADOW, true, false, true, true>), g, b, 0, s, a);
    else hipLaunchKernelGGL((k_trace<MODE_SHADOW, true, false, true, false>), g, b, 0, s, a);
    return;
  }
  launch_trace<MODE_SHADOW, true>(a, counting, cfg, s);
}

#ifdef RT_ALT_KERNELS
void launch_blob(const SceneDev& sc, const EntryArgs& e, const FrameDev& f, bool counting, hipStream_t s) {
  const uint32_t n = (uint32_t)(e.tiles_x * e.tile_rows);
  if (n == 0 || f.tile_blob == nullptr) return;
  BlobArgs a{sc, e, f.tile_blob, f.blob_arena, f.blob_slots / N_SHARDS, f.blob_list, f.counters};
  if (counting) hipLaunchKernelGGL((k_blob<true>), dim3(n), dim3(64), 0, s, a);
  else hipLaunchKernelGGL((k_blob<false>), dim3(n), dim3(64), 0, s, a);
}

template <int CLS>
static void launch_tile_class(const TileArgs& t, uint32_t blocks, bool counting, hipStream_t s) {
  if (counting) hipLaunchKernelGGL((k_tile<CLS, true>), dim3(blocks), dim3(256), 0, s, t);
  else hipLaunchKernelGGL((k_tile<CLS, false>), dim3(blocks), dim3(256), 0, s, t);
}
void launch_tile(const SceneDev& sc, const FrameDev& f, const UniformsDev& u, bool counting, hipStream_t s) {
  if (f.tile_blob == nullptr) return;
  TileArgs t{};
  t.sc = sc; t.f = f; t.u = u; t.sub_slots = f.blob_slots / N_SHARDS; t.tmin = 0.001f;
  const uint32_t blocks = f.blob_slots / N_SHARDS * N_SHARDS;
  launch_tile_class<0>(t, blocks, counting, s);
  launch_tile_class<1>(t, blocks, counting, s);
  launch_tile_class<2>(t, blocks, counting, s);
}

void launch_beam_shadow(const SceneDev& sc, const FrameDev& f, const UniformsDev& u, bool counting, const LaunchCfg& cfg, hipStream_t s) {
  if (!f.shadow_runs || !f.pixel_runs) return;
  BeamShadowArgs A{};
  A.t = make_args(sc, f.counters, 0, f.shard_cap, f.ovf_stack);
  A.t.work = f.counters + cnt_work(Q_SHADOW0, 0);
  A.t.ray_o = f.sh_o; A.t.ray_d = f.sh_d; A.t.sh_c = f.sh_c; A.t.sample_color = f.sample_color;
  const bool le = f.light_entry != nullptr && f.sh_e != nullptr;
  A.t.entry = le ? f.light_entry : nullptr; A.t.sh_e = le ? f.sh_e : nullptr;
  for (int k = 0; k < 3; k++) A.light[k] = u.light_position[k];
  A.run = (uint32_t)f.pixel_runs;
  const dim3 g(cfg.trace_blocks), b(256);
  if (counting) hipLaunchKernelGGL(k_beam_shadow_count, g, b, 0, s, A);
  else hipLaunchKernelGGL(k_beam_shadow, g, b, 0, s, A);
}
#else
void launch_blob(const SceneDev&, const EntryArgs&, const FrameDev&, bool, hipStream_t) {}
void launch_tile(const SceneDev&, const FrameDev&, const UniformsDev&, bool, hipStream_t) {}
void launch_beam_shadow(const SceneDev&, const FrameDev&, const UniformsDev&, bool, const LaunchCfg&, hipStream_t) {}
#endif

__global__ __launch_bounds__(64) void k_query_init(uint32_t* counters, uint32_t n) {
  const uint32_t t = threadIdx.x;
  if (t < (uint32_t)N_SHARDS) { counters[cnt_tail(0, (int)t)] = t == 0u ? n : 0u; counters[cnt_work(0, (int)t)] = 0u; }
}

void launch_query(const SceneDev& sc, const float4* rays, HitRec* out, uint32_t n, int32_t* ovf_stack, uint32_t* counters, bool any_hit,
                  bool counting, const LaunchCfg& cfg, hipStream_t s) {
  hipLaunchKernelGGL(k_query_init, dim3(1), dim3(64), 0, s, counters, n);
  TraceArgs a = make_args(sc, counters, 0, n, ovf_stack);
  a.ray_o = rays; a.raw_out = out;
#ifdef RT_ALT_KERNELS
// ... 226 lines not shown
```

vulkan_raytracing_amd/csrc/kernels_beam.inc:

```
struct BeamSpace { F3 s0, b0, s1, b1; uint3 rot; };

__device__ __forceinline__ bool slab_beam(uint32_t wx, uint32_t wy, uint32_t wz, const BeamSpace& B, float tmin, float tlim, float& tn) {
  wx = __builtin_amdgcn_alignbit(wx, wx, B.rot.x); wy = __builtin_amdgcn_alignbit(wy, wy, B.rot.y); wz = __builtin_amdgcn_alignbit(wz, wz, B.rot.z);
  const float nx = (float)(wx & 0xFFFFu), fx = (float)(wx >> 16), ny = (float)(wy & 0xFFFFu), fy = (float)(wy >> 16), nz = (float)(wz & 0xFFFFu), fz = (float)(wz >> 16);
  const float x0 = fminf(__builtin_fmaf(nx, B.s0.x, B.b0.x), __builtin_fmaf(nx, B.s1.x, B.b1.x)), x1 = fmaxf(__builtin_fmaf(fx, B.s0.x, B.b0.x), __builtin_fmaf(fx, B.s1.x, B.b1.x));
  const float y0 = fminf(__builtin_fmaf(ny, B.s0.y, B.b0.y), __builtin_fmaf(ny, B.s1.y, B.b1.y)), y1 = fmaxf(__builtin_fmaf(fy, B.s0.y, B.b0.y), __builtin_fmaf(fy, B.s1.y, B.b1.y));
  const float z0 = fminf(__builtin_fmaf(nz, B.s0.z, B.b0.z), __builtin_fmaf(nz, B.s1.z, B.b1.z)), z1 = fmaxf(__builtin_fmaf(fz, B.s0.z, B.b0.z), __builtin_fmaf(fz, B.s1.z, B.b1.z));
  tn = fmaxf(fmaxf(x0, y0), fmaxf(z0, tmin));
  const float tf = fminf(fminf(x1, y1), fminf(z1, tlim));
  return tn <= tf * 1.00002f;
}
__device__ __forceinline__ void beam_axis(float lo, float hi, float da, float t_far, float q_lo_minus_o, float q_scale, float& s0, float& b0, float& s1, float& b1, uint32_t& rot) {
  if (lo < 0.0f && hi > 0.0f) {
    const float K = 1.0e30f, inv = 1.0f / q_scale, r = t_far * da;
    const float U = (r - q_lo_minus_o) * inv + 1.0f, L = (-r - q_lo_minus_o) * inv - 1.0f;
    s0 = K; s1 = K; b0 = -K * U; b1 = -K * L; rot = 0u;
  }
  else { s0 = q_scale * lo; b0 = q_lo_minus_o * lo; s1 = q_scale * hi; b1 = q_lo_minus_o * hi; rot = lo < 0.0f ? 16u : 0u; }
}

#define RT_BEAM_EACH(M) M(0) M(1) M(2) M(3)
#ifndef RT_BEAM_KEEP_NUM
#define RT_BEAM_KEEP_NUM RT_KEEP_NUM
#endif
#ifndef RT_BEAM_UNROLL
#define RT_BEAM_UNROLL RT_INTERIOR_UNROLL
#endif

struct BeamShadeUniforms {
  float position[3], light_position[3], light_intensity;
  uint32_t max_bounce_count, samples_per_pixel, center_object_type, orbiting_object_type;
};
struct BeamShadeArgs {
  SceneDev sc;
  const float4* ray_o;
  const float4* ray_d;
  const uint32_t* tails;
  uint32_t* work;
  uint32_t shard_cap;
  int32_t* ovf_stack;
  uint32_t* counters;
  float tmin;
  const EntryRec* entry;
  float4* next_o;
  float4* next_d;
  float4* sh_o;
  float4* sh_d;
  float4* sh_c;
  uint32_t* sh_e;
  float4* sample_color;
  const EntryRec* light_entry;
  int width, rows, light_tiles, settle_dead_shadow_rays;
  BeamShadeUniforms u;
};
struct BeamShadeFrame {
  float4* ray_o[2]; float4* ray_d[2];
  float4* sh_o; float4* sh_d; float4* sh_c; uint32_t* sh_e;
  float4* sample_color;
  uint32_t* counters;
  const EntryRec* light_entry;
  uint32_t shard_cap;
  int width, rows, light_tiles, settle_dead_shadow_rays;
  static constexpr int pixel_runs = 64;
  static constexpr uint32_t sh_base = 0u;
};
struct BeamShadeView { const SceneDev& sc; const BeamShadeFrame& f; const BeamShadeUniforms& u; };

template <bool COUNT, bool SHADE = false, typename Args = TraceArgs>
__device__ __forceinline__ void beam_body(const Args& a, const uint32_t run) {
  __shared__ int s_stack[4][STACK2_LDS + 1][64];
  __shared__ float s_best[4][16][64];
  __shared__ float4 s_inst[LDS_INSTANCES ? LDS_INSTANCES : 1][5];
  const int n_lds_inst = a.sc.n_inst < LDS_INSTANCES ? a.sc.n_inst : LDS_INSTANCES;
  if ((int)threadIdx.x < n_lds_inst) {
    const InstanceDev* I = a.sc.inst + threadIdx.x;
    const float4* mp = reinterpret_cast<const float4*>(I->w2o);
    s_inst[threadIdx.x][0] = mp[0]; s_inst[threadIdx.x][1] = mp[1]; s_inst[threadIdx.x][2] = mp[2];
    s_inst[threadIdx.x][3] = make_float4(I->q_lo[0], I->q_lo[1], I->q_lo[2], __int_as_float(I->blas_root));
    s_inst[threadIdx.x][4] = make_float4(I->q_scale[0], I->q_scale[1], I->q_scale[2], __uint_as_float(I->mask));
  }
  __syncthreads();
  const uint32_t lane = threadIdx.x & 63u, wave = threadIdx.x >> 6;
  int* const stk = &s_stack[wave][0][lane];
  float* const bst = &s_best[wave][0][lane];
  const char* const node_bytes = reinterpret_cast<const char*>(a.sc.blas_nodes);
  const uint32_t S = run >> 6;
  uint64_t cnt_nodes = 0, cnt_tris = 0, diag_iters = 0, diag_busy = 0;
  const uint64_t diag_t0 = COUNT ? __builtin_readcyclecounter() : 0;
  uint32_t shard = blockIdx.x & (N_SHARDS - 1), tried = 0;

  for (;;) {
    uint32_t base = 0; bool got = false;
    while (tried < (uint32_t)N_SHARDS) {
      const uint32_t size = ld_cursor(a.tails + shard * CNT_STRIDE);
      uint32_t off = 0;
      if (lane == 0 && size) off = atomicAdd(a.work + shard * CNT_STRIDE, run);
      off = (uint32_t)__builtin_amdgcn_readfirstlane((int)off);
      if (size && off < size) { base = shard * a.shard_cap + off; got = true; break; }
      shard = (shard + 1u) & (N_SHARDS - 1); tried++;
    }
    if (!got) break;
    const uint32_t v0 = base + lane;

    uint32_t alive = 0, sid = 0;
    F3 co = mk3(0, 0, 0), cd0 = mk3(0, 0, 1), cd1 = cd0, cd2 = cd0, cd3 = cd0;
    float bt0 = -1.0f, bt1 = -1.0f, bt2 = -1.0f, bt3 = -1.0f;
    BeamSpace B;
    B.s0 = B.s1 = B.b0 = B.b1 = mk3(0, 0, 0); B.rot = make_uint3(0u, 0u, 0u);
    int cur = REF_DONE, sp = 1, cur_inst = -1;
    uint32_t my_visits = 0;

    auto push = [&](int v) {
      if (sp < STACK2_LDS) stk[sp * 64] = v;
      else *reinterpret_cast<volatile int32_t*>(a.ovf_stack + (size_t)(blockIdx.x * 256u + threadIdx.x) * a.sc.ovf_stride + (sp - STACK2_LDS)) = v;
      sp++;
    };
    auto pop = [&]() {
      sp--;
      if (sp < STACK2_LDS) cur = stk[sp * 64];
      else cur = *reinterpret_cast<volatile int32_t*>(a.ovf_stack + (size_t)(blockIdx.x * 256u + threadIdx.x) * a.sc.ovf_stride + (sp - STACK2_LDS));
    };
    auto set_space = [&](int ii, int& root, uint32_t& imask) {
      const float4 ro = a.ray_o[base];
      const F3 wo = mk3(ro.x, ro.y, ro.z);
      F3 w0 = mk3(0, 0, 1), w1 = w0, w2 = w0, w3 = w0;
#define RT_BEAM_LD(j) if (alive & (1u << j)) { const float4 r = a.ray_d[v0 + 64u * j]; w##j = mk3(r.x, r.y, r.z); }
      RT_BEAM_EACH(RT_BEAM_LD)
#undef RT_BEAM_LD
      float qlo3[3] = {a.sc.tlas_q_lo[0], a.sc.tlas_q_lo[1], a.sc.tlas_q_lo[2]}, qsc3[3] = {a.sc.tlas_q_scale[0], a.sc.tlas_q_scale[1], a.sc.tlas_q_scale[2]};
      root = 0; imask = 0xFFu;
      if (ii >= 0) {
        float4 m0, m1, m2, ql, qsc;
        if (ii < n_lds_inst) { m0 = s_inst[ii][0]; m1 = s_inst[ii][1]; m2 = s_inst[ii][2]; ql = s_inst[ii][3]; qsc = s_inst[ii][4]; }
        else {
          const InstanceDev* I = a.sc.inst + ii;
          const float4* mp = reinterpret_cast<const float4*>(I->w2o);
          m0 = mp[0]; m1 = mp[1]; m2 = mp[2];
          ql = make_float4(I->q_lo[0], I->q_lo[1], I->q_lo[2], __int_as_float(I->blas_root));
          qsc = make_float4(I->q_scale[0], I->q_scale[1], I->q_scale[2], __uint_as_float(I->mask));
        }
        root = __float_as_int(ql.w); imask = __float_as_uint(qsc.w);
        if ((imask & 0xFFu) == 0u) return;
        float m[12];
        m[0] = m0.x; m[1] = m0.y; m[2] = m0.z; m[3] = m0.w; m[4] = m1.x; m[5] = m1.y; m[6] = m1.z; m[7] = m1.w;
        m[8] = m2.x; m[9] = m2.y; m[10] = m2.z; m[11] = m2.w;
// ... 73 lines not shown
              if (COUNT) { cnt_nodes++; my_visits++; }
              float t0, t1;
              const bool h0 = slab_beam(Q0.x, Q0.y, Q0.z, B, a.tmin, tlim, t0);
              const bool h1 = slab_beam(Q0.w, Q1.x, Q1.y, B, a.tmin, tlim, t1);
              const bool both = h0 && h1, none = !(h0 || h1), swap = t1 < t0;
              const uint32_t pm = 0u - (uint32_t)both;
              stk_lds[(((uint32_t)sp & pm) | ((uint32_t)STACK2_LDS & ~pm)) * 64u] = swap ? ch.x : ch.y;
              const int one = h0 ? ch.x : ch.y;
              cur = both ? (swap ? ch.y : ch.x) : (none ? top : one);
              sp += (both ? 1 : 0) - (none ? 1 : 0);
            }
        } else {
#pragma unroll
          for (int r = 0; r < RT_BEAM_UNROLL; r++)
            if (cur >= 0) {
              const uint4* np = reinterpret_cast<const uint4*>(node_bytes + ((uint32_t)cur << 5));
              const uint4 Q0 = np[0], Q1 = np[1];
              const int2 ch = make_int2((int)Q1.z, (int)Q1.w);
              if (COUNT) { cnt_nodes++; my_visits++; }
              float t0, t1;
              const bool h0 = slab_beam(Q0.x, Q0.y, Q0.z, B, a.tmin, tlim, t0);
              const bool h1 = slab_beam(Q0.w, Q1.x, Q1.y, B, a.tmin, tlim, t1);
              if (h0 && h1) { const bool swap = t1 < t0; push(swap ? ch.x : ch.y); cur = swap ? ch.y : ch.x; }
              else if (h0) cur = ch.x;
              else if (h1) cur = ch.y;
              else pop();
            }
        }
      }
      if (cur < 0 && cur > REF_MARK && cur_inst >= 0) {
        const uint32_t ref = (uint32_t)(~cur);
        const uint32_t first = ref >> 3, count = (ref & 7u) + 1u;
        for (uint32_t k = 0; k < count; k++) {
          const float4* tp = a.sc.tris + (size_t)(first + k) * 3;
          const float4 T0 = tp[0], T1 = tp[1], T2 = tp[2];
          const int prim = (int)__float_as_uint(T2.y);
#define RT_BEAM_TRI(j) if (alive & (1u << j)) { \
            if (COUNT) cnt_tris++; \
            float tt, uu, vv; \
            if (tri_test(T0, T1, T2, co, cd##j, a.tmin, 10000.0f, tt, uu, vv)) { \
              bool better = tt < bt##j; \
              if (tt == bt##j) { const int bi = __float_as_int(bst[(4 * j + 3) * 64]), bp = __float_as_int(bst[(4 * j + 2) * 64]); \
                                 better = bi < 0 || cur_inst < bi || (cur_inst == bi && prim < bp); } \
              if (better) { bt##j = tt; bst[(4 * j + 0) * 64] = uu; bst[(4 * j + 1) * 64] = vv; bst[(4 * j + 2) * 64] = __int_as_float(prim); bst[(4 * j + 3) * 64] = __int_as_float(cur_inst); } \
            } }
          RT_BEAM_EACH(RT_BEAM_TRI)
#undef RT_BEAM_TRI
        }
        pop();
      }
      if (cur == REF_MARK) {
        cur_inst = -1;
        pop();
        if (cur >= 0) { int root; uint32_t imask; set_space(-1, root, imask); }
      }
      if (cur < 0 && cur > REF_MARK && cur_inst < 0) {
        const int ii = ~cur;
        int root; uint32_t imask;
        set_space(ii, root, imask);
        if ((imask & 0xFFu) == 0u) {
          pop();
          if (cur >= 0) set_space(-1, root, imask);
        } else {
          push(REF_MARK);
          cur_inst = ii; cur = root;
        }
      }
    }

    if (COUNT) {
      uint32_t mx = my_visits;
      for (int off = 32; off > 0; off >>= 1) mx = max(mx, (uint32_t)__shfl_xor((int)mx, off));
      if (lane == 0) {
        atomicMax(a.counters + CNT_TILE_DIAG, mx);
        atomicAdd(reinterpret_cast<unsigned long long*>(a.counters + CNT_TILE_DIAG + 2), (unsigned long long)mx);
        atomicAdd(reinterpret_cast<unsigned long long*>(a.counters + CNT_TILE_DIAG + 4), 1ull);
      }
    }
    if constexpr (SHADE) {
      const uint32_t run_shard = (uint32_t)__builtin_amdgcn_readfirstlane((int)shard);
      const BeamShadeArgs* ka = (const BeamShadeArgs*)__builtin_amdgcn_kernarg_segment_ptr();
      asm volatile("" : "+s"(ka));
      const BeamShadeFrame sf{{const_cast<float4*>(ka->ray_o), ka->next_o}, {const_cast<float4*>(ka->ray_d), ka->next_d}, ka->sh_o, ka->sh_d, ka->sh_c, ka->sh_e, ka->sample_color,
                              ka->counters, ka->light_entry, ka->shard_cap, ka->width, ka->rows, ka->light_tiles, ka->settle_dead_shadow_rays};
      const BeamShadeView sv{ka->sc, sf, ka->u};
#pragma nounroll
      for (uint32_t j = 0; j < S; j++) {
        const float tj = j == 0u ? bt0 : (j == 1u ? bt1 : (j == 2u ? bt2 : bt3));
        const float* const b = bst + 256u * j;
        const int ij = (alive >> j) & 1u ? __float_as_int(b[192]) : HIT_DEAD;
        shade_slot<false, false, false, true>(sv, 0, run_shard, v0 + 64u * j, true, ij, make_float4(tj, b[0], b[64], b[128]));
      }
    } else {
#define RT_BEAM_OUT(j) if (j < S) { \
      const uint32_t v = v0 + 64u * j; \
      if (alive & (1u << j)) { \
        st_stream(&a.hit_a[v], make_float4(bt##j, bst[(4 * j + 0) * 64], bst[(4 * j + 1) * 64], bst[(4 * j + 2) * 64])); \
        st_stream(&a.hit_inst[v], __float_as_int(bst[(4 * j + 3) * 64])); \
      } else st_stream(&a.hit_inst[v], HIT_DEAD); }
    RT_BEAM_EACH(RT_BEAM_OUT)
#undef RT_BEAM_OUT
    }
  }
  if (COUNT) {
    for (int off = 32; off > 0; off >>= 1) {
      cnt_nodes += __shfl_down((unsigned long long)cnt_nodes, off);
      cnt_tris += __shfl_down((unsigned long long)cnt_tris, off);
    }
    if (lane == 0) {
      atomicAdd(reinterpret_cast<unsigned long long*>(a.counters + CNT_NODE_VISITS), (unsigned long long)cnt_nodes);
      atomicAdd(reinterpret_cast<unsigned long long*>(a.counters + CNT_TRI_TESTS), (unsigned long long)cnt_tris);
      atomicAdd(reinterpret_cast<unsigned long long*>(a.counters + CNT_DIAG), (unsigned long long)diag_iters);
      atomicAdd(reinterpret_cast<unsigned long long*>(a.counters + CNT_DIAG + 2), (unsigned long long)diag_busy);
      atomicAdd(reinterpret_cast<unsigned long long*>(a.counters + CNT_DIAG + 4), (unsigned long long)(__builtin_readcyclecounter() - diag_t0));
    }
  }
}

#ifndef RT_BEAM_WAVES
#define RT_BEAM_WAVES 4
#endif
__global__ __launch_bounds__(256) __attribute__((amdgpu_waves_per_eu(RT_BEAM_WAVES, RT_BEAM_WAVES))) void k_beam(TraceArgs a, uint32_t run) { beam_body<false>(a, run); }
__global__ __launch_bounds__(256) void k_beam_count(TraceArgs a, uint32_t run) { beam_body<true>(a, run); }
__global__ __launch_bounds__(256) __attribute__((amdgpu_waves_per_eu(RT_BEAM_WAVES, RT_BEAM_WAVES))) void k_beam_shade(BeamShadeArgs a, uint32_t run) { beam_body<false, true>(a, run); }

#ifdef RT_ALT_KERNELS
struct BeamShadowArgs {
  TraceArgs t;
  float light[3];
  uint32_t run;
};
struct BeamSpaceW { F3 s0, s1, n0, n1, f0, f1; uint3 rot; };

__device__ __forceinline__ bool slab_beam_w(uint32_t wx, uint32_t wy, uint32_t wz, const BeamSpaceW& B, float tmin, float tlim, float& tn, float& tfo) {
  wx = __builtin_amdgcn_alignbit(wx, wx, B.rot.x); wy = __builtin_amdgcn_alignbit(wy, wy, B.rot.y); wz = __builtin_amdgcn_alignbit(wz, wz, B.rot.z);
  const float nx = (float)(wx & 0xFFFFu), fx = (float)(wx >> 16), ny = (float)(wy & 0xFFFFu), fy = (float)(wy >> 16), nz = (float)(wz & 0xFFFFu), fz = (float)(wz >> 16);
  const float x0 = fminf(__builtin_fmaf(nx, B.s0.x, B.n0.x), __builtin_fmaf(nx, B.s1.x, B.n1.x)), x1 = fmaxf(__builtin_fmaf(fx, B.s0.x, B.f0.x), __builtin_fmaf(fx, B.s1.x, B.f1.x));
  const float y0 = fminf(__builtin_fmaf(ny, B.s0.y, B.n0.y), __builtin_fmaf(ny, B.s1.y, B.n1.y)), y1 = fmaxf(__builtin_fmaf(fy, B.s0.y, B.f0.y), __builtin_fmaf(fy, B.s1.y, B.f1.y));
  const float z0 = fminf(__builtin_fmaf(nz, B.s0.z, B.n0.z), __builtin_fmaf(nz, B.s1.z, B.n1.z)), z1 = fmaxf(__builtin_fmaf(fz, B.s0.z, B.f0.z), __builtin_fmaf(fz, B.s1.z, B.f1.z));
  tn = fmaxf(fmaxf(x0, y0), fmaxf(z0, tmin));
  const float tf = fminf(fminf(x1, y1), fminf(z1, tlim));
  tfo = tf;
  return tn <= tf * 1.00002f + 1.0e-6f;
}
__device__ __forceinline__ void beam_axis_w(float lo, float hi, float da, float t_far, float delta, float q_lo_minus_o, float q_scale,
                                            float& s0, float& s1, float& n0, float& n1, float& f0, float& f1, uint32_t& rot) {
  if (lo < 0.0f && hi > 0.0f) {
    const float K = 1.0e30f, inv = 1.0f / q_scale, r = __builtin_fmaf(t_far, da, delta);
    const float U = (r - q_lo_minus_o) * inv + 1.0f, L = (-r - q_lo_minus_o) * inv - 1.0f;
    s0 = K; s1 = K; n0 = -K * U; f0 = n0; n1 = -K * L; f1 = n1; rot = 0u;
  } else {
    s0 = q_scale * lo; s1 = q_scale * hi;
    const float b0 = q_lo_minus_o * lo, b1 = q_lo_minus_o * hi, e0 = delta * __builtin_fabsf(lo), e1 = delta * __builtin_fabsf(hi);
    n0 = b0 - e0; n1 = b1 - e1; f0 = b0 + e0; f1 = b1 + e1;
    rot = lo < 0.0f ? 16u : 0u;
  }
}

template <bool COUNT>
__device__ __forceinline__ void beam_shadow_body(const BeamShadowArgs& A) {
  const TraceArgs& a = A.t;
  __shared__ int s_stack[4][STACK2_LDS + 1][64];
  __shared__ float s_ray[4][24][64];
  __shared__ float4 s_inst[LDS_INSTANCES ? LDS_INSTANCES : 1][5];
  const int n_lds_inst = a.sc.n_inst < LDS_INSTANCES ? a.sc.n_inst : LDS_INSTANCES;
  if ((int)threadIdx.x < n_lds_inst) {
    const InstanceDev* I = a.sc.inst + threadIdx.x;
    const float4* mp = reinterpret_cast<const float4*>(I->w2o);
    s_inst[threadIdx.x][0] = mp[0]; s_inst[threadIdx.x][1] = mp[1]; s_inst[threadIdx.x][2] = mp[2];
    s_inst[threadIdx.x][3] = make_float4(I->q_lo[0], I->q_lo[1], I->q_lo[2], __int_as_float(I->blas_root));
    s_inst[threadIdx.x][4] = make_float4(I->q_scale[0], I->q_scale[1], I->q_scale[2], __uint_as_float(I->mask));
  }
  __syncthreads();
  const uint32_t lane = threadIdx.x & 63u, wave = threadIdx.x >> 6;
// ... 244 lines not shown
```

vulkan_raytracing_amd/csrc/rt_api.cpp:

```cpp
#include "../../include/rt_api.h"

#include <hip/hip_runtime.h>

#include <algorithm>
#include <cmath>
#include <cstdio>
#include <cstring>
#include <map>
#include <mutex>
#include <queue>
#include <string>
#include <vector>

#include "blas_refit.h"
#include "bvh_build.h"
#include "bvh_gpu.h"
#include "rt_device.h"
#include "rt_kernels.h"
#include "tlas_gpu.h"

using namespace rt;

static_assert(sizeof(rt_instance) == 64, "rt_instance must mirror VkAccelerationStructureInstanceKHR (64 B)");
static_assert(sizeof(rt_uniforms) == 104, "rt_uniforms must mirror UniformStructure (104 B)");
// ... 67 lines not shown
  BvhNodeQ* d_blas_nodes = nullptr;
  std::vector<Bvh4Node> h_blas4;
  Bvh4Node* d_nodes4 = nullptr;
  std::vector<WideNodeQ> h_wide;
  WideNodeQ* d_wide = nullptr;
  float4* d_tris = nullptr;
  size_t n_blas_nodes = 0, n_blas4 = 0, n_tris = 0;
  float* d_cover_boxes = nullptr;
  uint32_t max_cover_count = 0;
  uint32_t tlas_cap = 1024;
  bool arrays_ready = false;
  int variant = 0;

  uchar4* d_sky = nullptr;
  int sky_w = 0, sky_h = 0;

  MaterialDev* d_materials = nullptr;
  uint32_t* d_prim_material = nullptr;
  int n_materials = 0;
  size_t n_prim_material = 0;

  TlasMeshDev* d_mesh_table = nullptr;
  uint32_t* d_cover_src = nullptr;
  BlasRefitScratch refit;
};

enum { INST_NONE = 0, INST_HOST = 1, INST_DEVICE = 2 };
constexpr int MAX_DEVICE_INSTANCES = 1 << 20;

struct rt_ctx {
  int device = 0;
  hipStream_t stream = nullptr;
  std::string error;
  std::string info;
  int n_cu = 0;
  Scene* scene = nullptr;
  int slot = 0;

  std::vector<rt_instance> h_inst;
  std::vector<uint32_t> inst_types;
  BuiltBvh tlas;
  Bvh4 tlas4;
  bool tlas_valid = false;
  bool tlas_stale = false;
  int inst_source = INST_NONE;
  int n_inst = 0;
  TlasGpu tgpu;
  bool dev_far = true;
  double dev_g_lo[3] = {0, 0, 0}, dev_g_hi[3] = {0, 0, 0};
  InstanceDev* d_inst[2] = {nullptr, nullptr};
  size_t cap_inst[2] = {0, 0};
  int parity = 0;
  int tlas_node_count[2] = {0, 0};
  int batch_k = 1;
  uint32_t batch_out_stride = 0;
  int inst_per_frame = 0;
  int tlas_stride[2] = {0, 0};
  std::vector<UniformsDev> batch_uni;
  hipEvent_t ev_frame[2] = {nullptr, nullptr};
  bool ev_frame_valid[2] = {false, false};
  float tlas_q_lo[3] = {0, 0, 0}, tlas_q_scale[3] = {1, 1, 1};
  uint32_t ovf_stride = STACK_OVF, ovf_alloc_stride = 0;
  int stack_need = 0;
  int ovf_alloc_blocks = 0;
  char* h_stage[2] = {nullptr, nullptr};
  size_t stage_bytes[2] = {0, 0};
  hipEvent_t ev_upload[2] = {nullptr, nullptr};
  bool upload_inflight[2] = {false, false};
  bool upload_pending = false;

  UniformsDev uni{};
  bool have_uni = false;

  FrameDev frame{};
  size_t frame_capacity = 0;
  size_t out_capacity = 0;
  float4* d_out_own = nullptr;
  float4* h_out_pinned = nullptr;
  size_t pinned_capacity = 0;
  bool out_rgba8 = false;
  bool out_bgra = false;
  bool async_pending = false;
  int async_w = 0, async_h = 0;
  uint32_t* d_counters = nullptr;
  int cnt_parity = 0;
  int32_t* d_ovf = nullptr;
  LaunchCfg cfg{};
  bool grid_user_set = false;
  int closest_blocks_per_cu = -1, shadow_blocks_per_cu = -1;
  int tail_blocks = TAIL_BLOCKS;
  int tail_resident_per_cu = 0;
  int tail_mode = 1;
  int jitter_table = 1;
  const float2* jitter_waited = nullptr; hipStream_t jitter_waited_stream = nullptr;
  int primary_cover = 1;
  int tail_min_blocks = 1;
  bool tail_full_grid = false;
  int entry_max_instances = 32;
  int entry_points = 1;
  int shadow_entry = 2;
  int light_tiles = LIGHT_TILES_DEFAULT;
  EntryRec* d_entry = nullptr;
  size_t entry_alloc_tiles = 0;
  int camera_records = 1;
  int dead_shadow_rays = 1;
  int shadow_beams = 0;
  bool sh_double = false;
  int fused_shade = 1;
  int pixel_beams = 1;
  int tile_blobs = 0;
  uint32_t* d_tile_blob = nullptr;
  char* d_blob_arena = nullptr;
  uint32_t blob_slots = 0;
  uint4* d_blob_list = nullptr;
  size_t tile_dir_alloc = 0;
  EntryRec* d_light_entry = nullptr;
  size_t light_alloc_tiles = 0;
  uint32_t* d_cover_mask = nullptr;
  uint32_t cover_alloc_words = 0;
  int cover_parity = 0;
  unsigned long long* h_stats = nullptr;
  unsigned long long* d_stats = nullptr;
  bool last_empty = false;
  uint32_t* h_hint = nullptr;
  uint32_t* d_hint = nullptr;
  int blas_builder = 1;
  int timing = 0;
  bool counting = false;
  std::vector<hipEvent_t> ev_pool;
  size_t ev_used = 0;
  std::vector<TimedSpan> spans;
  uint32_t timed_frames = 0;
  rt_stats last{};
  bool frame_pending = false;
  hipStream_t frame_stream = nullptr;
  struct LastFrame { int W, H, band_rows, shard, n_shards; float4* d_out; bool counting; SceneDev sc; UniformsDev uni; int parity; uint64_t inst_gen; int batch_k; BatchTab bt; uint32_t out_frame_stride; } last_frame{};
  uint64_t inst_gen[2] = {0, 0};
  struct LightKey {
    float light[3] = {0, 0, 0}; uint64_t gen = 0; int parity = -1, n_inst = 0, tiles = 0;
    bool operator==(const LightKey& o) const { return light[0] == o.light[0] && light[1] == o.light[1] && light[2] == o.light[2] && gen == o.gen && parity == o.parity && n_inst == o.n_inst && tiles == o.tiles; }
  };
  LightKey light_key_seen, light_key_built;
  bool light_built = false, light_seen_valid = false;
  bool tail_disabled = false;
  bool frame_rerendered = false;
  uint32_t tail_faults = 0;
  uint32_t* d_fault_total = nullptr;
  uint64_t faults_seen = 0;
  bool debug_force_tail_fault = false;
  uint32_t last_max_bounce = 0;
  uint64_t last_primary = 0;
  uint32_t* d_q_counters = nullptr;
  int32_t* d_q_ovf = nullptr;
  size_t q_ovf_alloc = 0;
  float* d_q_scale = nullptr;
  size_t q_scale_alloc = 0;
  uint32_t* d_q_words = nullptr;
  size_t q_words_alloc = 0;
  hipEvent_t ev_query[2] = {nullptr, nullptr};
  bool ev_query_valid[2] = {false, false};
  int query_last = -1;
  FrameDev shade{};
  size_t shade_capacity = 0;
  size_t shade_colors = 0;
};

namespace {

int fail(rt_ctx* c, int code, const std::string& msg) {
  if (c) c->error = msg; else g_create_error = msg;
  return code;
}
#define HIP_TRY(c, expr)                                                                          \
  do {                                                                                            \
    hipError_t e_ = (expr);                                                                       \
    if (e_ != hipSuccess)                                                                         \
      return fail(c, e_ == hipErrorOutOfMemory ? RT_ERR_OUT_OF_MEMORY : RT_ERR_DEVICE,            \
                  std::string("HIP runtime exception: return code ") + std::to_string((int)e_) +  \
                      " (" + hipGetErrorString(e_) + ") in " #expr);                              \
  } while (0)

void invert_affine(const float m[12], float out[12]) {
  double a = m[0], b = m[1], c = m[2], d = m[4], e = m[5], f = m[6], g = m[8], h = m[9], i = m[10];
  double tx = m[3], ty = m[7], tz = m[11];
  double c00 = e * i - f * h, c01 = c * h - b * i, c02 = b * f - c * e;
  double c10 = f * g - d * i, c11 = a * i - c * g, c12 = c * d - a * f;
  double c20 = d * h - e * g, c21 = b * g - a * h, c22 = a * e - b * d;
// ... 438 lines not shown
  if (parity < 0 || p == m->query_last) { m->ev_query_valid[0] = m->ev_query_valid[1] = false; m->query_last = -1; }
  return RT_OK;
}
int quiesce_scene(rt_ctx* c) {
  for (rt_ctx* m : c->scene->members) {
    { int q = wait_queries(c, m); if (q) return q; }
    if (m->async_pending) return fail(c, RT_ERR_NOT_READY, "a frame slot of this scene has a frame pending (rt_trace_async): collect it with rt_trace_wait first");
    if (m->frame_pending) { int r = collect_stats(m); if (r) { if (m != c) c->error = m->error; return r; } }
    for (int k = 0; k < 2; k++)
      if (m->upload_inflight[k]) { HIP_TRY(c, hipEventSynchronize(m->ev_upload[k])); m->upload_inflight[k] = false; }
    m->upload_pending = false;
  }
  return RT_OK;
}
void invalidate_tlas(Scene* S) { for (rt_ctx* m : S->members) { m->tlas_valid = false; m->tlas_stale = false; } }

int ready_to_trace(rt_ctx* c, bool batch = false) {
  if (!c->scene->d_verts) return fail(c, RT_ERR_NOT_READY, "rt_upload_geometry has not been called");
  if (!c->tlas_valid) return fail(c, RT_ERR_NOT_READY, "rt_set_instances has not been called");
  if (c->tlas_stale) return fail(c, RT_ERR_NOT_READY, "a BLAS was refitted (rt_refit_blas_device) since the TLAS was set: update it with rt_set_instances, rt_set_instances_device or rt_set_batch first");
  if (!batch && c->batch_k != 1) return fail(c, RT_ERR_NOT_READY, "the context holds a frame batch (rt_set_batch): render it with rt_trace_shard_batch, or call rt_set_instances for a single frame");
  return RT_OK;
}

int ensure_common(rt_ctx* c) {
  if (!c->d_counters) {
    HIP_TRY(c, hipMalloc((void**)&c->d_counters, 2 * CNT_WORDS * sizeof(uint32_t)));
    HIP_TRY(c, hipMemsetAsync(c->d_counters, 0, 2 * CNT_WORDS * sizeof(uint32_t), c->stream));
    HIP_TRY(c, hipStreamSynchronize(c->stream));
    c->cnt_parity = 0;
  }
  if (!c->d_fault_total) {
    HIP_TRY(c, hipMalloc((void**)&c->d_fault_total, sizeof(uint32_t)));
    HIP_TRY(c, hipMemsetAsync(c->d_fault_total, 0, sizeof(uint32_t), c->stream));
    HIP_TRY(c, hipStreamSynchronize(c->stream));
    c->faults_seen = 0;
  }
  if (!c->h_hint) {
    HIP_TRY(c, hipHostMalloc((void**)&c->h_hint, CNT_MAX_BOUNCES * sizeof(uint32_t), hipHostMallocMapped));
    for (int b = 0; b < CNT_MAX_BOUNCES; b++) c->h_hint[b] = 0xFFFFFFFFu;
    HIP_TRY(c, hipHostGetDevicePointer((void**)&c->d_hint, c->h_hint, 0));
  }
  if (!c->h_stats) {
    HIP_TRY(c, hipHostMalloc((void**)&c->h_stats, STAT_WORDS * sizeof(unsigned long long), hipHostMallocMapped));
    memset(c->h_stats, 0, STAT_WORDS * sizeof(unsigned long long));
    HIP_TRY(c, hipHostGetDevicePointer((void**)&c->d_stats, c->h_stats, 0));
  }
  if (c->d_ovf && (c->ovf_alloc_stride < c->ovf_stride || c->ovf_alloc_blocks < std::max(c->cfg.trace_blocks, c->tail_blocks))) { HIP_TRY(c, hipFree(c->d_ovf)); c->d_ovf = nullptr; }
  if (!c->d_ovf) {
    HIP_TRY(c, hipMalloc((void**)&c->d_ovf, ovf_elems(c->cfg.trace_blocks, c->tail_blocks, c->ovf_stride) * sizeof(int32_t)));
    c->ovf_alloc_stride = c->ovf_stride; c->ovf_alloc_blocks = std::max(c->cfg.trace_blocks, c->tail_blocks);
  }
  return RT_OK;
}

int alloc_queues(rt_ctx* c, FrameDev& f, size_t capacity, size_t sh_cap, size_t colors) {
  void** ptrs[] = {(void**)&f.ray_o[0], (void**)&f.ray_o[1], (void**)&f.ray_d[0], (void**)&f.ray_d[1], (void**)&f.hit_a};
  void** sh_ptrs[] = {(void**)&f.sh_o, (void**)&f.sh_d, (void**)&f.sh_c};
  for (void** p : ptrs) { if (*p) HIP_TRY(c, hipFree(*p)); *p = nullptr; }
  for (void** p : sh_ptrs) { if (*p) HIP_TRY(c, hipFree(*p)); *p = nullptr; }
  if (f.sample_color) { HIP_TRY(c, hipFree(f.sample_color)); f.sample_color = nullptr; }
  if (f.hit_inst) { HIP_TRY(c, hipFree(f.hit_inst)); f.hit_inst = nullptr; }
  if (f.sh_e) { HIP_TRY(c, hipFree(f.sh_e)); f.sh_e = nullptr; }
  for (void** p : ptrs) HIP_TRY(c, hipMalloc(p, capacity * sizeof(float4)));
  if (colors) HIP_TRY(c, hipMalloc((void**)&f.sample_color, colors * sizeof(float4)));
  for (void** p : sh_ptrs) HIP_TRY(c, hipMalloc(p, sh_cap * sizeof(float4)));
  HIP_TRY(c, hipMalloc((void**)&f.hit_inst, capacity * sizeof(int32_t)));
  HIP_TRY(c, hipMalloc((void**)&f.sh_e, sh_cap * sizeof(uint32_t)));
  return RT_OK;
}
void free_queues(FrameDev& f) {
  void* ptrs[] = {f.ray_o[0], f.ray_o[1], f.ray_d[0], f.ray_d[1], f.hit_a, f.hit_inst, f.sh_o, f.sh_d, f.sh_c, f.sh_e, f.sample_color};
  for (void* p : ptrs) if (p) hipFree(p);
}

int ensure_frame(rt_ctx* c, size_t capacity) {
  int r = ensure_common(c); if (r) return r;
  const bool want_double = c->shadow_beams != 0;
  if (capacity <= c->frame_capacity && (!want_double || c->sh_double)) return RT_OK;
  capacity = std::max(capacity, c->frame_capacity);
  c->frame_capacity = 0;
  const size_t sh_cap = (want_double ? 2 : 1) * capacity;
  r = alloc_queues(c, c->frame, capacity, sh_cap, capacity); if (r) return r;
  c->sh_double = want_double;
  c->frame_capacity = capacity;
  return RT_OK;
}

hipEvent_t take_event(rt_ctx* c) {
  if (c->ev_used == c->ev_pool.size()) { hipEvent_t e; hipEventCreate(&e); c->ev_pool.push_back(e); }
  return c->ev_pool[c->ev_used++];
}

int jitter_table_for(rt_ctx* c, const FrameDev& f, uint32_t spp, hipStream_t s, const float2** out) {
  Scene* S = c->scene;
  *out = nullptr;
  JitterTable* t = nullptr;
  for (JitterTable& k : S->jitter_tables)
    if (k.W == f.width && k.H == f.height && k.rows == f.rows && k.spp == spp && k.band_rows == f.band_rows && k.shard == f.shard && k.n_shards == f.n_shards) { t = &k; break; }
  if (!t) {
    if (S->jitter_tables.size() >= MAX_JITTER_TABLES) {
      HIP_TRY(c, hipDeviceSynchronize());
      size_t lru = 0;
      for (size_t k = 1; k < S->jitter_tables.size(); k++) if (S->jitter_tables[k].last_use < S->jitter_tables[lru].last_use) lru = k;
      hipFree(S->jitter_tables[lru].d); hipEventDestroy(S->jitter_tables[lru].ready);
      S->jitter_tables.erase(S->jitter_tables.begin() + (long)lru);
      for (rt_ctx* m : S->members) m->jitter_waited = nullptr;
    }
    JitterTable n;
    n.W = f.width; n.H = f.height; n.rows = f.rows; n.spp = spp; n.band_rows = f.band_rows; n.shard = f.shard; n.n_shards = f.n_shards;
    HIP_TRY(c, hipMalloc((void**)&n.d, jitter_table_elems(f.width, f.rows, spp) * sizeof(float2)));
    if (hipEventCreateWithFlags(&n.ready, hipEventDisableTiming) != hipSuccess) { hipFree(n.d); return fail(c, RT_ERR_DEVICE, "hipEventCreate failed"); }
    launch_jitter_table(f, spp, n.d, s);
    HIP_TRY(c, hipEventRecord(n.ready, s));
    S->jitter_tables.push_back(n);
    t = &S->jitter_tables.back();
    c->jitter_waited = t->d; c->jitter_waited_stream = s;
  }
  if (c->jitter_waited != t->d || c->jitter_waited_stream != s) {
    HIP_TRY(c, hipStreamWaitEvent(s, t->ready, 0));
    c->jitter_waited = t->d; c->jitter_waited_stream = s;
  }
  t->last_use = ++S->jitter_clock;
  *out = t->d;
  return RT_OK;
}

struct Span {
  rt_ctx* c; int cat; hipStream_t s; hipEvent_t a = nullptr;
  bool on() const { return c->timing == 1 || (c->timing == 2 && cat == CAT_TRACE); }
  Span(rt_ctx* c_, int cat_, hipStream_t s_) : c(c_), cat(cat_), s(s_) {
    if (on()) { a = take_event(c); hipEventRecord(a, s); }
  }
  ~Span() {
    if (on()) { hipEvent_t b = take_event(c); hipEventRecord(b, s); c->spans.push_back({cat, a, b}); }
  }
};

int enqueue_frame(rt_ctx* c, int W, int H, int band_rows, int shard, int n_shards, float4* d_out, hipStream_t s, const rt_ctx::LastFrame* again = nullptr) {
  const int rows = rt_shard_rows(H, band_rows, shard, n_shards);
  const bool no_tail = again != nullptr;
  const int K = again ? again->batch_k : c->batch_k;
  SceneDev sc = again ? again->sc : scene_dev(c);
  const UniformsDev u = again ? again->uni : c->uni;
  BatchTab bt{};
  if (again) bt = again->bt;
  else if (K > 1)
    for (int k = 0; k < K; k++) {
      const UniformsDev& uk = c->batch_uni[k];
      for (int j = 0; j < 4; j++) { bt.position[k][j] = uk.position[j]; bt.right[k][j] = uk.right[j]; bt.up[k][j] = uk.up[j]; bt.forward[k][j] = uk.forward[j]; }
      for (int j = 0; j < 3; j++) bt.light[k][j] = uk.light_position[j];
      bt.light[k][3] = uk.light_intensity;
    }
  if (K > 1) sc.batch_samples = (uint32_t)((size_t)u.samples_per_pixel * (size_t)rows * (size_t)W);
  const int n_inst1 = K > 1 ? sc.n_inst / K : sc.n_inst;
  const int frame_parity = again ? again->parity : c->parity;
  if (!again) { c->last_frame = {W, H, band_rows, shard, n_shards, d_out, c->counting, sc, u, c->parity, c->inst_gen[c->parity], K, bt, c->batch_out_stride ? c->batch_out_stride : (uint32_t)((size_t)rows * W)}; c->frame_rerendered = false; }
  if (u.samples_per_pixel == 0) return fail(c, RT_ERR_INVALID_ARGUMENT, "samplesPerPixel must be >= 1");
  if (u.max_bounce_count + 2 > (uint32_t)CNT_MAX_BOUNCES) return fail(c, RT_ERR_INVALID_ARGUMENT, "maxBounceCount too large (max 69)");
  const size_t tiles = (size_t)((W + 7) / 8) * (size_t)((rows + 7) / 8) * (size_t)K;
  const size_t samples = tiles * u.samples_per_pixel * 64;
  if (samples >= 0xF0000000ull) return fail(c, RT_ERR_INVALID_ARGUMENT, "frame too large for 32-bit sample ids");
  if (rows > 8 * 65535 || u.samples_per_pixel > 4u * 65535u) return fail(c, RT_ERR_INVALID_ARGUMENT, "frame too large for the raygen grid");
  if ((size_t)rows * K > 8u * 65535u) return fail(c, RT_ERR_INVALID_ARGUMENT, "frame batch too tall for the raygen grid");
  const size_t raygen_blocks = raygen_block_count(W, rows, u.samples_per_pixel, K);
  const size_t shard_cap = std::max<size_t>(256, ((raygen_blocks + N_SHARDS - 1) / N_SHARDS) * 256) * (c->tile_blobs ? 2 : 1);
// ... 73 lines not shown
    f.entry = entry_on ? c->d_entry : nullptr;
    if (tile_on) {
      const uint32_t want_slots = (uint32_t)(((std::min<size_t>(tiles_local, tiles_local / 2 + 2048) + N_SHARDS - 1) / N_SHARDS + 8) * N_SHARDS);
      if (tiles_local > c->tile_dir_alloc || want_slots > c->blob_slots) {
        HIP_TRY(c, hipStreamSynchronize(c->stream)); if (s != c->stream) HIP_TRY(c, hipStreamSynchronize(s));
        if (c->d_tile_blob) HIP_TRY(c, hipFree(c->d_tile_blob));
        if (c->d_blob_arena) HIP_TRY(c, hipFree(c->d_blob_arena));
        if (c->d_blob_list) HIP_TRY(c, hipFree(c->d_blob_list));
        c->d_tile_blob = nullptr; c->d_blob_arena = nullptr; c->d_blob_list = nullptr; c->tile_dir_alloc = 0; c->blob_slots = 0;
        const size_t dir = std::max(tiles_local, c->entry_alloc_tiles);
        HIP_TRY(c, hipMalloc((void**)&c->d_tile_blob, dir * sizeof(uint32_t)));
        HIP_TRY(c, hipMalloc((void**)&c->d_blob_arena, (size_t)want_slots * BLOB_SLOT_BYTES));
        HIP_TRY(c, hipMalloc((void**)&c->d_blob_list, (size_t)BLOB_CLASSES * want_slots * sizeof(uint4)));
        c->tile_dir_alloc = dir; c->blob_slots = want_slots;
      }
      f.tile_blob = c->d_tile_blob; f.blob_arena = c->d_blob_arena; f.blob_slots = c->blob_slots; f.blob_list = c->d_blob_list;
    }
    if (entry_on)
      for (int fk = 0; fk < K; fk++) {
        EntryArgs& ea = ev.v[fk];
        const CoverArgs& cak = cv.v[fk];
        const float* right = K > 1 ? bt.right[fk] : u.right; const float* up = K > 1 ? bt.up[fk] : u.up; const float* fwd = K > 1 ? bt.forward[fk] : u.forward;
        for (int k = 0; k < 3; k++) ea.cam[k] = cak.cam[k];
        for (int k = 0; k < 9; k++) ea.inv[k] = cak.inv[k];
        for (int k = 0; k < 3; k++) { ea.basis[k] = right[k]; ea.basis[3 + k] = up[k]; ea.basis[6 + k] = fwd[k]; }
        ea.kf = 2.5f; ea.apex_radius = 0.0f;
        ea.width = W; ea.height = H; ea.tiles_x = (W + 7) / 8; ea.tile_rows = (rows + 7) / 8;
        ea.band_rows = band_rows; ea.shard = shard; ea.n_shards = n_shards;
        ea.records = c->d_entry + (size_t)fk * tiles_local; ea.cover = f.cover + (size_t)fk * cam_words; ea.cover_tiles_x = f.cover_tiles_x;
        ea.tlas_root_offset = fk * sc.tlas_stride;
      }
    ev.n = entry_on ? K : 1;
    if (light_on) {
      const size_t light_tiles_total = (size_t)6 * LT * LT;
      if (light_tiles_total > c->light_alloc_tiles) {
        if (c->d_light_entry) { HIP_TRY(c, hipStreamSynchronize(c->stream)); if (s != c->stream) HIP_TRY(c, hipStreamSynchronize(s)); HIP_TRY(c, hipFree(c->d_light_entry)); c->d_light_entry = nullptr; c->light_alloc_tiles = 0; }
        HIP_TRY(c, hipMalloc((void**)&c->d_light_entry, light_tiles_total * sizeof(EntryRec)));
        c->light_alloc_tiles = light_tiles_total; c->light_built = false;
      }
      f.light_entry = c->d_light_entry; f.light_tiles = LT;
      const float apex_radius = 0.0102f;
      for (int face = 0; face < 6; face++) {
        const int axis = face >> 1, a1 = (axis + 1) % 3, a2 = (axis + 2) % 3;
        const float sgn = (face & 1) ? -1.0f : 1.0f;
        float basis[9] = {0, 0, 0, 0, 0, 0, 0, 0, 0};
        basis[a1] = 1.0f; basis[3 + a2] = 1.0f; basis[6 + axis] = sgn;
        CoverArgs& lc = cv.v[1 + face];
        EntryArgs& le = ev.v[1 + face];
        for (int k = 0; k < 3; k++) lc.cam[k] = le.cam[k] = u.light_position[k];
        for (int k = 0; k < 9; k++) { lc.inv[k] = le.inv[k] = basis[k]; le.basis[k] = basis[k]; }
        lc.kf = le.kf = 1.0f; lc.apex_radius = le.apex_radius = apex_radius;
        lc.width = lc.height = le.width = le.height = 8 * LT;
        lc.tiles_x = lc.tiles_y = LT; lc.n_inst = ca.n_inst;
        lc.mask_offset = cam_words + (uint32_t)face * face_words;
        le.tiles_x = le.tile_rows = LT; le.band_rows = 8 * LT; le.shard = 0; le.n_shards = 1;
        le.records = c->d_light_entry + (size_t)face * LT * LT;
        le.cover = f.cover + lc.mask_offset; le.cover_tiles_x = LT;
      }
      bool build = true;
      if (c->shadow_entry == 2) {
        rt_ctx::LightKey key;
        for (int k = 0; k < 3; k++) key.light[k] = u.light_position[k];
        key.gen = c->inst_gen[frame_parity]; key.parity = frame_parity; key.n_inst = sc.n_inst; key.tiles = LT;
        const bool have = c->light_built && key == c->light_key_built;
        const bool stable = !c->light_seen_valid || key == c->light_key_seen;
        if (!again) { c->light_key_seen = key; c->light_seen_valid = true; }
        if (again != nullptr) { build = false; if (!have) { f.light_entry = nullptr; f.light_tiles = 0; } }
        else if (have) build = false;
        else if (stable) { c->light_key_built = key; c->light_built = true; }
        else { build = false; c->light_built = false; f.light_entry = nullptr; f.light_tiles = 0; }
      }
      if (build) { cv.n = ENTRY_VIEWS; ev.n = ENTRY_VIEWS; }
    }
  }
  LaunchCfg cfg = c->cfg;
  if (c->stack_need > 120) cfg.packet = 0;
  if (K > 1) cfg.packet = 0;
  cfg.far = far_frame ? 1 : 0;
  f.far_possible = cfg.far;
  f.settle_dead_shadow_rays = c->dead_shadow_rays;
  f.pixel_runs = beam_on ? 64 * (int)std::min<uint32_t>(u.samples_per_pixel, 4u) : 0;
  f.shadow_runs = (beam_on && c->shadow_beams && K == 1 && std::isfinite(u.light_position[0]) && std::isfinite(u.light_position[1]) && std::isfinite(u.light_position[2])) ? 1u : 0u;
  f.sh_base = f.shadow_runs ? (uint32_t)capacity : 0u;
  if (c->jitter_table && rows > 0) { r = jitter_table_for(c, f, u.samples_per_pixel, s, &f.jitter); if (r) return r; }
  if (!c->timing || c->timed_frames >= 64) { c->ev_used = 0; c->spans.clear(); c->timed_frames = 0; }
  if (c->timing) c->timed_frames++;
  c->frame_stream = s; c->frame_pending = true;
  c->last_max_bounce = u.max_bounce_count;
  c->last_primary = (uint64_t)W * rows * u.samples_per_pixel * (uint64_t)K;
  c->last_empty = rows == 0;
  if (c->upload_pending && s != c->stream) HIP_TRY(c, hipStreamWaitEvent(s, c->ev_upload[c->parity], 0));
  if (rows == 0) return RT_OK;
  c->cnt_parity ^= 1;
  if (f.cover_next) c->cover_parity ^= 1;
  int cap_closest = c->closest_blocks_per_cu, cap_shadow = c->shadow_blocks_per_cu;
  {
    constexpr unsigned long long GRID_SMALL_RAYS = 2500000ull;
    const bool crowded = c->scene->members.size() >= 3 && !c->grid_user_set && !c->last_empty;
    const unsigned long long prev_q0 = ((volatile unsigned long long*)c->h_stats)[STAT_QUEUE0], prev_sh = ((volatile unsigned long long*)c->h_stats)[STAT_SHADOW];
    if (cap_closest < 0) cap_closest = (crowded && prev_q0 > 0 && prev_q0 <= GRID_SMALL_RAYS) ? 2 : 0;
    if (cap_shadow < 0) cap_shadow = (crowded && f.light_entry != nullptr && prev_sh > 0 && prev_sh <= GRID_SMALL_RAYS) ? 2 : 0;
  }
  {
    Span frame_span(c, CAT_FRAME, s);
    {
      Span sp(c, CAT_RAYGEN, s);
      if (f.cover) launch_cover(sc, cv, c->scene->max_cover_count, const_cast<uint32_t*>(f.cover), s);
      if (f.entry || ev.n > 1) launch_entry(sc, ev, s);
      if (f.tile_blob) launch_blob(sc, ev.v[0], f, c->counting, s);
      launch_raygen(sc, f, u, bt, s);
    }
    uint32_t tail_start = 0xFFFFFFFFu;
    const bool tail_ok = c->cfg.variant != 1 && c->tail_blocks > 0 && !no_tail && !c->tail_disabled;
    if (tail_ok && c->tail_mode == 2) tail_start = 1;
    else if (tail_ok && c->tail_mode == 1)
      for (uint32_t b = 1; b <= u.max_bounce_count && b < (uint32_t)CNT_MAX_BOUNCES; b++)
        if (((volatile uint32_t*)c->h_hint)[b] <= TAIL_MAX_RAYS) { tail_start = b; break; }
    const bool fused0 = c->fused_shade && beam_on && c->camera_records && K == 1 && !c->counting && !f.tile_blob && !f.shadow_runs && tail_start != 0u;
    for (uint32_t b = 0; b <= u.max_bounce_count; b++) {
      if (b == tail_start) {
        int tb = std::min(c->tail_blocks, tail_grid(c->n_cu, c->tail_resident_per_cu, live_slots_on(c->device)));
        if (tb <= 0) { { Span sp(c, CAT_TRACE, s); launch_trace_closest(sc, f, (int)b, c->counting, cfg, s); } { Span sp(c, CAT_SHADE, s); launch_shade(sc, f, u, bt, (int)b, cfg, s); } continue; }
        const uint32_t expect = ((volatile uint32_t*)c->h_hint)[b];
        if (c->tail_mode == 1 && expect != 0xFFFFFFFFu && !c->tail_full_grid && c->scene->members.size() >= 3) {
          long want = ((long)expect + 255) / 256;
          const long lo = c->tail_min_blocks;
          if (lo >= N_SHARDS) want = (want + (N_SHARDS - 1)) / N_SHARDS * N_SHARDS;
          tb = (int)std::min<long>(tb, std::max<long>(lo, want));
        }
        Span sp(c, CAT_TAIL, s); launch_tail(sc, f, u, bt, (int)b, c->counting, cfg, tb, s);
        break;
      }
      { LaunchCfg cc = cfg; if (b == 0 && cap_closest > 0) cc.trace_blocks = std::min(cfg.trace_blocks, c->n_cu * cap_closest);
        Span sp(c, CAT_TRACE, s);
        if (b == 0 && f.tile_blob) launch_tile(sc, f, u, c->counting, s);
        if (b == 0 && fused0) launch_beam_shade(sc, f, u, cc, s);
        else launch_trace_closest(sc, f, (int)b, c->counting, cc, s); }
      if (!(b == 0 && fused0)) { Span sp(c, CAT_SHADE, s); launch_shade(sc, f, u, bt, (int)b, cfg, s); }
      if (b >= 7 && (b & 3) == 3 && b < u.max_bounce_count) {
        uint32_t tails[N_SHARDS * CNT_STRIDE];
        HIP_TRY(c, hipMemcpyAsync(tails, f.counters + cnt_tail((int)b + 1, 0), sizeof(tails), hipMemcpyDeviceToHost, s));
        HIP_TRY(c, hipStreamSynchronize(s));
        uint32_t live = 0;
        for (int t = 0; t < N_SHARDS; t++) live += tails[t * CNT_STRIDE];
        if (live == 0) break;
      }
    }
    { LaunchCfg cs = cfg; if (cap_shadow > 0) cs.trace_blocks = std::min(cfg.trace_blocks, c->n_cu * cap_shadow);
      Span sp(c, CAT_SHADOW, s); launch_beam_shadow(sc, f, u, c->counting, cs, s); launch_trace_shadow(sc, f, c->counting, cs, s); }
    { Span sp(c, CAT_RESOLVE, s); launch_resolve(f, u, s); }
  }
  HIP_TRY(c, hipGetLastError());
  if (!c->ev_frame[frame_parity]) HIP_TRY(c, hipEventCreateWithFlags(&c->ev_frame[frame_parity], hipEventDisableTiming));
  HIP_TRY(c, hipEventRecord(c->ev_frame[frame_parity], s));
  c->ev_frame_valid[frame_parity] = true;
  return RT_OK;
}

int collect_stats(rt_ctx* c) {
  if (!c->frame_pending) return RT_OK;
  HIP_TRY(c, hipStreamSynchronize(c->frame_stream));
  c->upload_pending = false;
  const unsigned long long* hs = c->h_stats;
  rt_stats st{};
  st.rays_primary = c->last_primary;
  if (!c->last_empty) {
// ... 60 lines not shown
  return RT_OK;
}

}

extern "C" {

int rt_abi_version(void) { return 7; }

static void size_traversal_grids(Scene* S) {
  const int per_cu = S->members.size() >= 3 ? 3 : 5;
  for (rt_ctx* m : S->members)
    if (!m->grid_user_set) m->cfg.trace_blocks = m->n_cu * per_cu;
}

static int create_context(rt_ctx** out_ctx, int device_id, rt_ctx* parent) {
  if (!out_ctx) return fail(nullptr, RT_ERR_INVALID_ARGUMENT, "out_ctx is NULL");
  *out_ctx = nullptr;
  int n = 0;
  hipError_t e = hipGetDeviceCount(&n);
  if (e != hipSuccess || n == 0)
    return fail(nullptr, RT_ERR_NO_DEVICE, "no HIP device available (librt_mi355x has no CPU fallback)");
  if (device_id < 0 || device_id >= n) return fail(nullptr, RT_ERR_INVALID_ARGUMENT, "device_id out of range");
  HIP_TRY(nullptr, hipSetDevice(device_id));
  hipDeviceProp_t prop;
  HIP_TRY(nullptr, hipGetDeviceProperties(&prop, device_id));
  if (std::string(prop.gcnArchName).find("gfx950") == std::string::npos)
    return fail(nullptr, RT_ERR_NO_DEVICE, std::string("device is ") + prop.gcnArchName + ", this library contains gfx950 code only");
  int slot = 0;
  if (parent) {
    while (slot < MAX_SLOTS && (parent->scene->slot_mask >> slot & 1u)) slot++;
    if (slot == MAX_SLOTS) return fail(nullptr, RT_ERR_INVALID_ARGUMENT, "a scene holds at most " + std::to_string(MAX_SLOTS) + " frame slots");
  }
  rt_ctx* c = new rt_ctx();
  c->device = device_id;
  c->n_cu = prop.multiProcessorCount;
  c->info = std::string("gfx950 ") + prop.name + " CUs=" + std::to_string(prop.multiProcessorCount);
  if (hipStreamCreateWithFlags(&c->stream, hipStreamNonBlocking) != hipSuccess) { delete c; return fail(nullptr, RT_ERR_DEVICE, "hipStreamCreate failed"); }
  c->cfg.trace_blocks = c->n_cu * 4;
  c->cfg.shade_blocks = c->n_cu * 8;
  c->cfg.rays_per_lane = 4; c->cfg.min_blocks = c->n_cu;
  c->cfg.variant = 0;
  c->cfg.packet = 0; c->cfg.packet_blocks = c->n_cu * 8;
  if (const char* env = getenv("RT_PACKET")) c->cfg.packet = alt_kernels_built() ? std::max(0, std::min(2, atoi(env))) : 0;
  if (const char* env = getenv("RT_PACKET_BLOCKS_PER_CU")) { const int v = atoi(env); if (v > 0 && v <= 16) c->cfg.packet_blocks = c->n_cu * v; }
  c->tail_resident_per_cu = tail_blocks_per_cu();
  live_slots_add(device_id, 1);
  c->tail_blocks = tail_grid(c->n_cu, c->tail_resident_per_cu, live_slots_on(device_id));
  if (const char* env = getenv("RT_BLAS_BUILDER")) c->blas_builder = atoi(env) ? 1 : 0;
  if (const char* env = getenv("RT_TAIL_MIN_BLOCKS")) c->tail_min_blocks = std::max(1, atoi(env));
  if (getenv("RT_TAIL_FULL_GRID")) c->tail_full_grid = true;
  if (const char* env = getenv("RT_TRACE_VARIANT")) { const int v = atoi(env); c->cfg.variant = (v >= 0 && v <= 2 && alt_kernels_built()) ? v : 0; }
  if (const char* env = getenv("RT_TRACE_BLOCKS_PER_CU")) { int v = atoi(env); if (v > 0 && v <= 8) c->cfg.trace_blocks = c->n_cu * v; }
  if (parent) {
    c->scene = parent->scene;
    c->cfg = parent->cfg; c->blas_builder = parent->blas_builder; c->tail_mode = parent->tail_mode; c->tail_min_blocks = parent->tail_min_blocks; c->tail_full_grid = parent->tail_full_grid; c->primary_cover = parent->primary_cover; c->jitter_table = parent->jitter_table; c->tile_blobs = parent->tile_blobs; c->pixel_beams = parent->pixel_beams; c->camera_records = parent->camera_records; c->dead_shadow_rays = parent->dead_shadow_rays; c->shadow_beams = parent->shadow_beams; c->entry_points = parent->entry_points; c->shadow_entry = parent->shadow_entry; c->entry_max_instances = parent->entry_max_instances; c->light_tiles = parent->light_tiles; c->out_rgba8 = parent->out_rgba8; c->out_bgra = parent->out_bgra;
  } else {
    c->scene = new Scene();
    c->scene->device = device_id;
  }
  c->slot = slot;
  c->scene->slot_mask |= 1u << slot;
  c->scene->members.push_back(c);
  if (getenv("RT_TRACE_BLOCKS_PER_CU")) c->grid_user_set = true;
  if (parent) c->grid_user_set = parent->grid_user_set;
  size_traversal_grids(c->scene);
  *out_ctx = c;
  return RT_OK;
}

int rt_create(rt_ctx** out_ctx, int device_id) { return create_context(out_ctx, device_id, nullptr); }

int rt_create_frame_slot(rt_ctx* parent, rt_ctx** out_ctx) {
  if (!parent) return fail(nullptr, RT_ERR_INVALID_ARGUMENT, "parent context is NULL");
  return create_context(out_ctx, parent->device, parent);
}

void rt_destroy(rt_ctx* c) {
  if (!c) return;
  live_slots_add(c->device, -1);
  hipSetDevice(c->device);
  wait_queries(c, c);
  hipDeviceSynchronize();
  void* ptrs[] = {c->d_inst[0], c->d_inst[1], c->d_out_own, c->d_counters, c->d_ovf, c->d_cover_mask, c->d_entry, c->d_light_entry, c->d_fault_total, c->d_tile_blob, c->d_blob_arena, c->d_blob_list};
  for (void* p : ptrs) if (p) hipFree(p);
  free_queues(c->frame);
  free_queues(c->shade);
  if (c->h_hint) hipHostFree(c->h_hint);
  if (c->h_out_pinned) hipHostFree(c->h_out_pinned);
  if (c->h_stats) hipHostFree(c->h_stats);
  for (int k = 0; k < 2; k++) { if (c->h_stage[k]) hipHostFree(c->h_stage[k]); if (c->ev_frame[k]) hipEventDestroy(c->ev_frame[k]); }
  for (int k = 0; k < 2; k++) if (c->ev_upload[k]) hipEventDestroy(c->ev_upload[k]);
  if (c->d_q_counters) hipFree(c->d_q_counters);
  if (c->d_q_ovf) hipFree(c->d_q_ovf);
  if (c->d_q_scale) hipFree(c->d_q_scale);
  if (c->d_q_words) hipFree(c->d_q_words);
  for (int k = 0; k < 2; k++) if (c->ev_query[k]) hipEventDestroy(c->ev_query[k]);
  tlas_gpu_free(c->tgpu);
  for (auto e : c->ev_pool) hipEventDestroy(e);
  if (c->stream) hipStreamDestroy(c->stream);
  Scene* S = c->scene;
  S->members.erase(std::remove(S->members.begin(), S->members.end(), c), S->members.end());
  S->slot_mask &= ~(1u << c->slot);
  size_traversal_grids(S);
  if (S->members.empty()) {
    void* sp[] = {S->d_wide, S->d_nodes4, S->d_verts, S->d_idx, S->d_blas_nodes, S->d_tris, S->d_sky, S->d_materials, S->d_prim_material, S->d_cover_boxes, S->d_mesh_table,
                  S->d_cover_src};
    for (void* p : sp) if (p) hipFree(p);
    blas_refit_free(S->refit);
    for (JitterTable& t : S->jitter_tables) { hipFree(t.d); hipEventDestroy(t.ready); }
    delete S;
  }
  delete c;
}

const char* rt_last_error(const rt_ctx* c) { return c ? c->error.c_str() : g_create_error.c_str(); }
const char* rt_device_info(const rt_ctx* c) { return c ? c->info.c_str() : ""; }

int rt_upload_geometry(rt_ctx* c, const float* verts6, size_t n_floats, const uint32_t* idx, size_t n_idx,
                       const rt_mesh_range* ranges, int n_meshes) {
  if (!c) return RT_ERR_INVALID_ARGUMENT;
  if (!verts6 || !idx || !ranges || n_meshes <= 0) return fail(c, RT_ERR_INVALID_ARGUMENT, "null geometry pointers or no meshes");
  { int q = quiesce_scene(c); if (q) return q; }
  Scene* S = c->scene;
  if (n_floats % 6 != 0) return fail(c, RT_ERR_INVALID_ARGUMENT, "vertex buffer must hold 6 floats per vertex");
  HIP_TRY(c, hipSetDevice(c->device));
  for (int m = 0; m < n_meshes; m++) {
    const rt_mesh_range& r = ranges[m];
    if (r.first_index + 3ull * r.prim_count > n_idx || r.first_float % 6 != 0 || r.first_float > n_floats)
      return fail(c, RT_ERR_INVALID_ARGUMENT, "mesh range " + std::to_string(m) + " exceeds the buffers");
    const uint64_t nv = (n_floats - r.first_float) / 6;
    for (uint64_t k = 0; k < 3ull * r.prim_count; k++)
      if (idx[r.first_index + k] >= nv) return fail(c, RT_ERR_INVALID_ARGUMENT, "index out of range in mesh " + std::to_string(m));
  }
  S->h_verts.assign(verts6, verts6 + n_floats);
  S->h_idx.assign(idx, idx + n_idx);
  if (S->d_verts) HIP_TRY(c, hipFree(S->d_verts));
  if (S->d_idx) HIP_TRY(c, hipFree(S->d_idx));
  S->d_verts = nullptr; S->d_idx = nullptr;
  HIP_TRY(c, hipMalloc((void**)&S->d_verts, std::max<size_t>(n_floats, 6) * sizeof(float)));
  HIP_TRY(c, hipMalloc((void**)&S->d_idx, std::max<size_t>(n_idx, 3) * sizeof(uint32_t)));
  HIP_TRY(c, hipMemcpy(S->d_verts, verts6, n_floats * sizeof(float), hipMemcpyHostToDevice));
  HIP_TRY(c, hipMemcpy(S->d_idx, idx, n_idx * sizeof(uint32_t), hipMemcpyHostToDevice));
  S->meshes.assign(n_meshes, Mesh{});
  for (int m = 0; m < n_meshes; m++) {
    Mesh& mm = S->meshes[m];
    mm.range = ranges[m];
    uint64_t top = 0;
    for (uint64_t k = 0; k < 3ull * mm.range.prim_count; k++) top = std::max<uint64_t>(top, (uint64_t)idx[mm.range.first_index + k] + 1);
    mm.span_floats = (uint32_t)(6 * top);
  }
  for (int a = 0; a < n_meshes; a++)
    for (int b = 0; b < n_meshes && S->meshes[a].span_shared_with < 0; b++) {
      const Mesh &ma = S->meshes[a], &mb = S->meshes[b];
      if (a != b && ma.span_floats && mb.span_floats && ma.range.first_float < mb.range.first_float + mb.span_floats && mb.range.first_float < ma.range.first_float + ma.span_floats)
        S->meshes[a].span_shared_with = b;
    }
  S->blas_linked = false; invalidate_tlas(S);
  if (S->d_materials) { HIP_TRY(c, hipFree(S->d_materials)); S->d_materials = nullptr; }
  if (S->d_prim_material) { HIP_TRY(c, hipFree(S->d_prim_material)); S->d_prim_material = nullptr; }
  S->n_materials = 0; S->n_prim_material = 0;
  return RT_OK;
}

int rt_build_blas(rt_ctx* c, int mesh) {
  if (!c) return RT_ERR_INVALID_ARGUMENT;
  Scene* S = c->scene;
// ... 282 lines not shown
  HIP_TRY(c, hipMalloc((void**)&S->d_sky, 6 * face_bytes));
  for (int f = 0; f < 6; f++)
    HIP_TRY(c, hipMemcpy((uint8_t*)S->d_sky + f * face_bytes, faces[f], face_bytes, hipMemcpyHostToDevice));
  S->sky_w = w; S->sky_h = h;
  return RT_OK;
}

int rt_shard_rows(int height, int band_rows, int shard, int n_shards) {
  if (height <= 0 || band_rows <= 0 || n_shards <= 0 || shard < 0 || shard >= n_shards) return 0;
  const int n_bands = (height + band_rows - 1) / band_rows;
  int rows = 0;
  for (int b = shard; b < n_bands; b += n_shards) rows += std::min(band_rows, height - b * band_rows);
  return rows;
}

int rt_set_param(rt_ctx* c, const char* name, int value) {
  if (!c || !name) return RT_ERR_INVALID_ARGUMENT;
  std::string k(name);
  if (k == "trace_variant") {
    if (value < 0 || value > 2) return fail(c, RT_ERR_INVALID_ARGUMENT, "trace_variant must be 0, 1 or 2");
    if (value != 0 && !alt_kernels_built()) return fail(c, RT_ERR_INVALID_ARGUMENT, "trace_variant 1 / 2 are not in the product library (measured slower): build librt_mi355x_alt.so with `make alt` and load it (RT_LIB_VARIANT=alt)");
    { int q = quiesce_scene(c); if (q) return q; }
    Scene* S = c->scene;
    const int before = c->cfg.variant;
    for (rt_ctx* m : S->members) m->cfg.variant = value;
    bool relink = (value == 2 && before != 2 && S->blas_linked);
    if (value != 0) {
      for (size_t mi = 0; mi < S->meshes.size(); mi++) {
        Mesh& m = S->meshes[mi];
        if (!m.built || !((value == 1 && m.gpu_built) || m.refitted)) continue;
        { int r = sync_host_verts(c, m); if (r) return r; }
        m.refitted = false; m.poisoned = false;
        build_blas(S->h_verts.data() + m.range.first_float, S->h_idx.data() + m.range.first_index, m.range.prim_count, m.bvh, m.tris);
        collapse_bvh4(m.bvh, true, false, m.bvh4);
        m.bounds = m.bvh.bounds; m.gpu_built = false; relink = true;
      }
    }
    if (relink) {
      S->blas_linked = false;
      for (rt_ctx* m : S->members) {
        if (!m->tlas_valid) continue;
        int r;
        if (m->inst_source == INST_DEVICE) {
          m->tlas_valid = false;
          r = set_instances_device(m, m->tgpu.d_rec, m->n_inst, 0, nullptr);
        } else {
          std::vector<rt_instance> keep = m->h_inst;
          m->tlas_valid = false;
          r = rt_set_instances(m, keep.data(), (int)keep.size(), 0);
        }
        if (r) { if (m != c) c->error = m->error; return r; }
      }
    }
    return RT_OK;
  }
  if (k == "closest_blocks_per_cu" || k == "shadow_blocks_per_cu") {
    if (value < -1 || value > 8) return fail(c, RT_ERR_INVALID_ARGUMENT, k + " must be -1 (automatic), 0 (the persistent grid) or 1..8");
    (k[0] == 'c' ? c->closest_blocks_per_cu : c->shadow_blocks_per_cu) = value; return RT_OK;
  }
  if (k == "trace_blocks_per_cu") {
    if (value < 1 || value > 8) return fail(c, RT_ERR_INVALID_ARGUMENT, "trace_blocks_per_cu must be 1..8");
    { int q = quiesce(c); if (q) return q; }
    c->cfg.trace_blocks = c->n_cu * value; c->grid_user_set = true; return RT_OK;
  }
  if (k == "output_rgba8") {
    if (value != 0 && value != 1) return fail(c, RT_ERR_INVALID_ARGUMENT, "output_rgba8 must be 0 or 1");
    if (c->async_pending) return fail(c, RT_ERR_NOT_READY, "output_rgba8 cannot change while a frame is pending");
    c->out_rgba8 = value != 0; c->out_bgra = false; return RT_OK;
  }
  if (k == "output_bgra8") {
    if (value != 0 && value != 1) return fail(c, RT_ERR_INVALID_ARGUMENT, "output_bgra8 must be 0 or 1");
    if (c->async_pending) return fail(c, RT_ERR_NOT_READY, "output_bgra8 cannot change while a frame is pending");
    c->out_rgba8 = value != 0; c->out_bgra = value != 0; return RT_OK;
  }
  if (k == "primary_cover") { c->primary_cover = value != 0; return RT_OK; }
  if (k == "jitter_table") { c->jitter_table = value != 0; return RT_OK; }
  if (k == "tile_blobs") {
    if (value != 0 && !alt_kernels_built()) return fail(c, RT_ERR_INVALID_ARGUMENT, "tile_blobs is not in the product library (measured slower): build librt_mi355x_alt.so with `make alt` and load it (RT_LIB_VARIANT=alt)");
    c->tile_blobs = value != 0; return RT_OK;
  }
  if (k == "pixel_beams") { c->pixel_beams = value != 0; return RT_OK; }
  if (k == "fused_shade") { c->fused_shade = value != 0; return RT_OK; }
  if (k == "camera_records") { c->camera_records = value != 0; return RT_OK; }
  if (k == "dead_shadow_rays") { c->dead_shadow_rays = value != 0; return RT_OK; }
  if (k == "shadow_beams") {
    if (value != 0 && !alt_kernels_built()) return fail(c, RT_ERR_INVALID_ARGUMENT, "shadow_beams is not in the product library (measured slower): build librt_mi355x_alt.so with `make alt` and load it (RT_LIB_VARIANT=alt)");
    c->shadow_beams = value != 0; return RT_OK;
  }

  if (k == "entry_points") { c->entry_points = value != 0; return RT_OK; }
  if (k == "packet_trace") {
    if (value < 0 || value > 2) return fail(c, RT_ERR_INVALID_ARGUMENT, "packet_trace must be 0, 1 or 2");
    if (value != 0 && !alt_kernels_built()) return fail(c, RT_ERR_INVALID_ARGUMENT, "packet_trace is not in the product library (measured slower): build librt_mi355x_alt.so with `make alt` and load it (RT_LIB_VARIANT=alt)");
    c->cfg.packet = value; return RT_OK;
  }
  if (k == "packet_blocks_per_cu") { if (value < 1 || value > 16) return fail(c, RT_ERR_INVALID_ARGUMENT, "packet_blocks_per_cu must be 1..16"); c->cfg.packet_blocks = c->n_cu * value; return RT_OK; }
  if (k == "shadow_entry") { if (value < 0 || value > 2) return fail(c, RT_ERR_INVALID_ARGUMENT, "shadow_entry must be 0, 1 or 2"); if (value != c->shadow_entry) { c->light_built = false; c->light_seen_valid = false; } c->shadow_entry = value; return RT_OK; }
  if (k == "entry_max_instances") { if (value < 1 || value >= (int)ENTRY_NO_INST) return fail(c, RT_ERR_INVALID_ARGUMENT, "entry_max_instances out of range"); c->entry_max_instances = value; return RT_OK; }
  if (k == "light_tiles") {
    if (value < 8 || value > 512) return fail(c, RT_ERR_INVALID_ARGUMENT, "light_tiles must be 8..512");
    { int q = quiesce(c); if (q) return q; }
    c->light_tiles = value; c->light_built = false; return RT_OK;
  }
  if (k == "tail_kernel") { if (value < 0 || value > 2) return fail(c, RT_ERR_INVALID_ARGUMENT, "tail_kernel must be 0 (off), 1 (auto) or 2 (always)"); c->tail_mode = value; return RT_OK; }
  if (k == "debug_force_tail_fault") { c->debug_force_tail_fault = value != 0; if (value == 2) c->tail_disabled = false; return RT_OK; }
  if (k == "blas_builder") { if (value != 0 && value != 1) return fail(c, RT_ERR_INVALID_ARGUMENT, "blas_builder must be 0 (host SAH) or 1 (device)"); for (rt_ctx* m : c->scene->members) m->blas_builder = value; return RT_OK; }
  if (k == "trace_rays_per_lane") { if (value < 1 || value > 64) return fail(c, RT_ERR_INVALID_ARGUMENT, "trace_rays_per_lane must be 1..64"); c->cfg.rays_per_lane = value; return RT_OK; }
  if (k == "trace_min_blocks") { if (value < 8) return fail(c, RT_ERR_INVALID_ARGUMENT, "trace_min_blocks must be >= 8"); c->cfg.min_blocks = value; return RT_OK; }
  if (k == "shade_blocks_per_cu") { if (value < 1 || value > 16) return fail(c, RT_ERR_INVALID_ARGUMENT, "shade_blocks_per_cu must be 1..16"); c->cfg.shade_blocks = c->n_cu * value; return RT_OK; }
  return fail(c, RT_ERR_INVALID_ARGUMENT, "unknown parameter " + k);
}

int rt_debug_check_builders(const float* verts6, size_t n_floats, const uint32_t* idx, size_t n_idx, uint64_t* out) {
  if (!verts6 || !idx || !out || n_idx % 3 != 0) return RT_ERR_INVALID_ARGUMENT;
  const uint32_t n = (uint32_t)(n_idx / 3);
  for (size_t k = 0; k < n_idx; k++) if ((size_t)idx[k] * 6 + 5 >= n_floats) return RT_ERR_INVALID_ARGUMENT;
  BuiltBvh bvh; std::vector<TriPacket> tris; Bvh4 b4; std::vector<BvhNodeQ> q; float q_lo[3], q_scale[3];
  build_blas(verts6, idx, n, bvh, tris);
  collapse_bvh4(bvh, true, false, b4);
  quantize_bvh2(bvh, q, q_lo, q_scale);
  uint64_t violations = 0, reached = 0, max_leaf = 0;
  std::vector<uint8_t> seen(n, 0);
  auto tri_box = [&](uint32_t leaf_pos, Aabb& b) {
    const TriPacket& t = tris[leaf_pos];
    for (int k = 0; k < 3; k++) {
      float a = t.v0[k], c1 = t.v0[k] + t.e1[k], c2 = t.v0[k] + t.e2[k];
      b.lo[k] = std::min(a, std::min(c1, c2)); b.hi[k] = std::max(a, std::max(c1, c2));
    }
  };
  struct Item { int32_t ref; Aabb box; int depth; };
  std::vector<Item> stack;
  auto child_box = [&](const BvhNode& nd, int which) { Aabb b; if (which == 0) { b.lo[0] = nd.a[0]; b.hi[0] = nd.a[1]; b.lo[1] = nd.a[2]; b.hi[1] = nd.a[3]; b.lo[2] = nd.c[0]; b.hi[2] = nd.c[1]; }
                                                        else { b.lo[0] = nd.b[0]; b.hi[0] = nd.b[1]; b.lo[1] = nd.b[2]; b.hi[1] = nd.b[3]; b.lo[2] = nd.c[2]; b.hi[2] = nd.c[3]; } return b; };
  Aabb all; for (int k = 0; k < 3; k++) { all.lo[k] = -3e38f; all.hi[k] = 3e38f; }
  stack.push_back({0, all, 0});
  int depth = 0;
  while (!stack.empty()) {
    Item it = stack.back(); stack.pop_back();
    depth = std::max(depth, it.depth);
    if (it.ref >= 0) {
      if ((size_t)it.ref >= bvh.nodes.size()) { violations++; continue; }
      const BvhNode& nd = bvh.nodes[it.ref]; const BvhNodeQ& nq = q[it.ref];
      for (int w = 0; w < 2; w++) {
        Aabb cb = child_box(nd, w);
        const int32_t ref = w ? nd.child1 : nd.child0;
        if (cb.lo[0] > 1e37f) continue;
        for (int k = 0; k < 3; k++) {
          if (cb.lo[k] < it.box.lo[k] - 1e-4f || cb.hi[k] > it.box.hi[k] + 1e-4f) violations++;
          const uint32_t wq = nq.w[(w ? 3 : 0) + k];
          const double qlo = (double)q_lo[k] + (double)(wq & 0xFFFFu) * q_scale[k], qhi = (double)q_lo[k] + (double)(wq >> 16) * q_scale[k];
          if (qlo > cb.lo[k] || qhi < cb.hi[k]) violations++;
        }
        if ((w ? nq.child1 : nq.child0) != ref) violations++;
        stack.push_back({ref, cb, it.depth + 1});
      }
    } else {
      const uint32_t r = (uint32_t)(~it.ref), first = r >> 3, count = (r & 7u) + 1u;
      max_leaf = std::max<uint64_t>(max_leaf, count);
      for (uint32_t k = 0; k < count; k++) {
        if (first + k >= n) { violations++; continue; }
        const uint32_t prim = tris[first + k].prim;
        if (prim >= n || seen[prim]) violations++; else { seen[prim] = 1; reached++; }
        Aabb tb; tri_box(first + k, tb);
        for (int a = 0; a < 3; a++) if (tb.lo[a] < it.box.lo[a] - 1e-4f || tb.hi[a] > it.box.hi[a] + 1e-4f) violations++;
      }
    }
  }
  if (reached != n) violations++;
  std::vector<uint8_t> seen4(n, 0); uint64_t reached4 = 0;
  std::vector<int32_t> st4; if (!b4.nodes.empty()) st4.push_back(0);
  while (!st4.empty()) {
    int32_t ref = st4.back(); st4.pop_back();
    if (ref >= 0) { for (int k = 0; k < 4; k++) { int32_t c = b4.nodes[ref].c[k].ref; if (c != 0x7FFFFFFF) st4.push_back(c); } }
    else { const uint32_t r = (uint32_t)(~ref), first = r >> 3, count = (r & 7u) + 1u; for (uint32_t k = 0; k < count && first + k < n; k++) { uint32_t p = tris[first + k].prim; if (p < n && !seen4[p]) { seen4[p] = 1; reached4++; } else violations++; } }
  }
  if (reached4 != n) violations++;
  out[0] = bvh.nodes.size(); out[1] = bvh.leaves; out[2] = (uint64_t)depth; out[3] = max_leaf; out[4] = b4.nodes.size(); out[5] = (uint64_t)b4.stack_need;
  out[6] = violations; out[7] = reached;
  return violations ? RT_ERR_INVALID_ARGUMENT : RT_OK;
}

int rt_debug_host_blas(const float* verts6, size_t n_floats, const uint32_t* idx, size_t n_idx, void* nodes, size_t nodes_capacity_bytes,
                       void* packets, size_t packets_capacity_bytes, uint64_t* out) {
  if (!verts6 || !idx || !nodes || !packets || !out || n_idx == 0 || n_idx % 3 != 0) return RT_ERR_INVALID_ARGUMENT;
  const uint32_t n = (uint32_t)(n_idx / 3);
  for (size_t k = 0; k < n_idx; k++) if ((size_t)idx[k] * 6 + 5 >= n_floats) return RT_ERR_INVALID_ARGUMENT;
  BuiltBvh bvh; std::vector<TriPacket> tris; std::vector<BvhNodeQ> q; float q_lo[3], q_scale[3];
  build_blas(verts6, idx, n, bvh, tris);
  quantize_bvh2(bvh, q, q_lo, q_scale);
  if (q.size() * sizeof(BvhNodeQ) > nodes_capacity_bytes || tris.size() * sizeof(TriPacket) > packets_capacity_bytes) return RT_ERR_INVALID_ARGUMENT;
  memcpy(nodes, q.data(), q.size() * sizeof(BvhNodeQ));
  memcpy(packets, tris.data(), tris.size() * sizeof(TriPacket));
  out[0] = q.size(); out[1] = tris.size();
  for (int k = 0; k < 3; k++) { uint32_t a, b; memcpy(&a, &q_lo[k], 4); memcpy(&b, &q_scale[k], 4); out[2 + k] = a; out[5 + k] = b; }
  return RT_OK;
}

int rt_debug_snapshot(rt_ctx* c, int what, void* out, size_t capacity_bytes, size_t* bytes) {
  if (!c) return RT_ERR_INVALID_ARGUMENT;
  if (!out) return fail(c, RT_ERR_INVALID_ARGUMENT, "rt_debug_snapshot: out is NULL");
  if (what < 0 || what > 8) return fail(c, RT_ERR_INVALID_ARGUMENT, "rt_debug_snapshot: what must be 0..8");
  Scene* S = c->scene;
  if (!c->tlas_valid || !S->blas_linked || !S->arrays_ready) return fail(c, RT_ERR_NOT_READY, "rt_debug_snapshot: the context has no valid TLAS (rt_set_instances)");
  { int q = quiesce_scene(c); if (q) return q; }
  HIP_TRY(c, hipSetDevice(c->device));
  HIP_TRY(c, hipStreamSynchronize(c->stream));
  if (c->tgpu.stream) HIP_TRY(c, hipStreamSynchronize(c->tgpu.stream));
  const int par = c->parity;
  const size_t tlas_nodes = c->batch_k > 1 ? (size_t)c->batch_k * (size_t)c->tlas_stride[par] : (size_t)c->tlas_node_count[par];
  size_t n_cover = 0;
  for (const Mesh& m : S->meshes) n_cover = std::max(n_cover, (size_t)m.cover_first + m.cover_count);
  uint64_t info[20] = {0};
  info[0] = S->n_blas_nodes; info[1] = tlas_base(c); info[2] = (uint64_t)c->tlas_node_count[par]; info[3] = c->batch_k > 1 ? (uint64_t)c->tlas_stride[par] : 0;
  info[4] = (uint64_t)c->batch_k; info[5] = S->n_tris; info[6] = (uint64_t)c->n_inst; info[7] = (uint64_t)c->inst_per_frame; info[8] = S->meshes.size();
  info[9] = S->h_verts.size(); info[10] = S->h_idx.size(); info[11] = n_cover;
  for (int k = 0; k < 3; k++) { uint32_t a, b; memcpy(&a, &c->tlas_q_lo[k], 4); memcpy(&b, &c->tlas_q_scale[k], 4); info[12 + k] = a; info[15 + k] = b; }
  info[18] = tlas_nodes;
  const void* src = nullptr; size_t need = 0; bool host = false;
  switch (what) {
    case 0: src = info; need = sizeof(info); host = true; break;
    case 1: src = S->d_blas_nodes; need = S->n_blas_nodes * sizeof(BvhNodeQ); break;
    case 2: src = S->d_blas_nodes + tlas_base(c); need = tlas_nodes * sizeof(BvhNodeQ); break;
    case 3: src = S->d_tris; need = S->n_tris * sizeof(TriPacket); break;
    case 4: src = c->d_inst[par]; need = (size_t)c->n_inst * sizeof(InstanceDev); break;
    case 5: src = S->d_mesh_table; need = S->meshes.size() * sizeof(TlasMeshDev); break;
    case 6: src = S->d_verts; need = S->h_verts.size() * sizeof(float); break;
    case 7: src = S->d_idx; need = S->h_idx.size() * sizeof(uint32_t); break;
    default: src = S->d_cover_boxes; need = n_cover * 6 * sizeof(float); break;
  }
  if (bytes) *bytes = need;
  if (need > capacity_bytes) return fail(c, RT_ERR_INVALID_ARGUMENT, "rt_debug_snapshot: the buffer holds " + std::to_string(capacity_bytes) + " bytes, item " + std::to_string(what) + " needs " + std::to_string(need));
  if (!need) return RT_OK;
  if (host) { memcpy(out, src, need); return RT_OK; }
  if (!src) return fail(c, RT_ERR_NOT_READY, "rt_debug_snapshot: item " + std::to_string(what) + " is not on the device");
  HIP_TRY(c, hipMemcpy(out, src, need, hipMemcpyDeviceToHost));
  return RT_OK;
}

int rt_debug_sizing(int n_cu, int resident_per_cu, int trace_blocks, uint32_t ovf_stride, uint64_t* out) {
  if (!out || n_cu <= 0 || trace_blocks <= 0) return RT_ERR_INVALID_ARGUMENT;
  const int g = tail_grid(n_cu, resident_per_cu, 0);
  out[0] = (uint64_t)g; out[1] = (uint64_t)ovf_elems(trace_blocks, g, ovf_stride);
  return RT_OK;
}

int rt_set_timing(rt_ctx* c, int enabled) { if (!c) return RT_ERR_INVALID_ARGUMENT; c->timing = enabled == 2 ? 2 : (enabled != 0); return RT_OK; }

int rt_trace_shard(rt_ctx* c, int W, int H, int band_rows, int shard, int n_shards, void* d_out, size_t out_capacity_bytes, void* hip_stream) {
  if (!c) return RT_ERR_INVALID_ARGUMENT;
  if (W <= 0 || H <= 0 || band_rows <= 0 || n_shards <= 0 || shard < 0 || shard >= n_shards || !d_out)
    return fail(c, RT_ERR_INVALID_ARGUMENT, "bad rt_trace_shard arguments");
  if (!c->have_uni) return fail(c, RT_ERR_NOT_READY, "rt_set_uniforms has not been called");
  if (c->async_pending) return fail(c, RT_ERR_NOT_READY, "a frame submitted with rt_trace_async is pending: call rt_trace_wait first");
  HIP_TRY(c, hipSetDevice(c->device));
  int r = ready_to_trace(c); if (r) return r;
  const int rows = rt_shard_rows(H, band_rows, shard, n_shards);
  if ((size_t)rows * W * (c->out_rgba8 ? 4 : 16) > out_capacity_bytes) return fail(c, RT_ERR_INVALID_ARGUMENT, "output buffer too small for this shard");
  hipStream_t s = hip_stream ? (hipStream_t)hip_stream : c->stream;
  if (c->frame_pending && c->frame_stream != s) { int q = collect_stats(c); if (q) return q; }
  return enqueue_frame(c, W, H, band_rows, shard, n_shards, (float4*)d_out, s);
}

int rt_trace_shard_batch(rt_ctx* c, int W, int H, int band_rows, int shard, int n_shards, void* d_out, size_t frame_stride_bytes, size_t out_capacity_bytes, void* hip_stream) {
  if (!c) return RT_ERR_INVALID_ARGUMENT;
  if (W <= 0 || H <= 0 || band_rows <= 0 || n_shards <= 0 || shard < 0 || shard >= n_shards || !d_out)
    return fail(c, RT_ERR_INVALID_ARGUMENT, "bad rt_trace_shard_batch arguments");
  if (!c->have_uni) return fail(c, RT_ERR_NOT_READY, "rt_set_batch has not been called");
  if (c->async_pending) return fail(c, RT_ERR_NOT_READY, "a frame submitted with rt_trace_async is pending: call rt_trace_wait first");
  HIP_TRY(c, hipSetDevice(c->device));
  int r = ready_to_trace(c, true); if (r) return r;
  const int rows = rt_shard_rows(H, band_rows, shard, n_shards);
  const size_t px_bytes = c->out_rgba8 ? 4 : 16, shard_bytes = (size_t)rows * W * px_bytes;
  if (frame_stride_bytes == 0) frame_stride_bytes = shard_bytes;
  if (frame_stride_bytes < shard_bytes || frame_stride_bytes % px_bytes != 0 || frame_stride_bytes / px_bytes > 0xFFFFFFFFull)
    return fail(c, RT_ERR_INVALID_ARGUMENT, "frame_stride_bytes must be 0 (compact) or a whole number of pixels >= one shard");
  if (frame_stride_bytes * (size_t)(c->batch_k - 1) + shard_bytes > out_capacity_bytes) return fail(c, RT_ERR_INVALID_ARGUMENT, "output buffer too small for the shards of this batch");
  hipStream_t s = hip_stream ? (hipStream_t)hip_stream : c->stream;
  if (c->frame_pending && c->frame_stream != s) { int q = collect_stats(c); if (q) return q; }
  c->batch_out_stride = (uint32_t)(frame_stride_bytes / px_bytes);
  r = enqueue_frame(c, W, H, band_rows, shard, n_shards, (float4*)d_out, s);
  c->batch_out_stride = 0;
  return r;
}

int rt_assemble_shards(rt_ctx* c, const void* d_gathered, int n_shards, size_t shard_stride_bytes, int W, int H, int band_rows,
                       void* d_frame, size_t frame_capacity_bytes, void* hip_stream) {
  if (!c) return RT_ERR_INVALID_ARGUMENT;
  const size_t bpp = c->out_rgba8 ? 4 : 16;
  if (!d_gathered || !d_frame || n_shards <= 0 || W <= 0 || H <= 0 || band_rows <= 0 || shard_stride_bytes % bpp != 0)
    return fail(c, RT_ERR_INVALID_ARGUMENT, "bad rt_assemble_shards arguments");
// ... 664 lines not shown
```

vulkan_raytracing_amd/csrc/rt_kernels.h:

```cpp
#pragma once
#include <hip/hip_runtime.h>
#include <stdint.h>

#include "rt_device.h"

namespace rt {

struct SceneDev {
  const BvhNodeQ* blas_nodes;
  int tlas_root;
  int tlas_nodes;
  int tlas_stride;
  uint32_t batch_samples;
  const float4* tris;
  float tlas_q_lo[3], tlas_q_scale[3];
  const WideNodeQ* wide_nodes;
  const Bvh4Node* nodes4;
  int tlas_root4;
  const InstanceDev* inst;
  const float* verts;
  const uint32_t* idx;
  const uchar4* sky;
  int n_inst;
  int sky_w, sky_h;
  uint32_t ovf_stride;
  const MaterialDev* materials;
  const uint32_t* prim_material;
  int n_materials;
  const float* cover_boxes;
};

struct FrameDev {
  float4* ray_o[2];
  float4* ray_d[2];
  float4* hit_a;
  int32_t* hit_inst;
  float4* sh_o;
  float4* sh_d;
  float4* sh_c;
  float4* sample_color;
  uint32_t* counters;
  uint32_t* counters_next;
  int32_t* ovf_stack;
  unsigned long long* stats_out;
  uint32_t* fault_total;
  uint32_t* hint;
  float4* out;
  int out_rgba8;
  uint32_t shard_cap;
  int width, height;
  int rows;
  int band_rows, shard, n_shards;
  const uint32_t* cover;
  uint32_t* cover_next;
  uint32_t cover_words;
  int cover_tiles_x;
  EntryRec* entry;
  const EntryRec* light_entry;
  uint32_t* sh_e;
  int light_tiles;
  int far_possible;
  int settle_dead_shadow_rays;
  const float2* jitter;
  int batch_k;
  uint32_t out_frame_stride;
  uint32_t cover_view_words;
  uint32_t* tile_blob;
  char* blob_arena;
  uint32_t blob_slots;
  uint4* blob_list;
  int pixel_runs;
  uint32_t shadow_runs;
  uint32_t sh_base;
};

struct CoverArgs {
  float cam[3];
  float inv[9];
  float kf;
  float apex_radius;
  int width, height, tiles_x, tiles_y;
  int n_inst;
  uint32_t mask_offset;
  int inst_base;
};
struct CoverViews { CoverArgs v[MAX_VIEWS]; int n; };

struct EntryArgs {
  float cam[3];
  float inv[9];
  float basis[9];
  float kf;
  float apex_radius;
  int width, height;
  int tiles_x, tile_rows;
  int band_rows, shard, n_shards;
  EntryRec* records;
  const uint32_t* cover;
  int cover_tiles_x;
  int tlas_root_offset;
};
struct EntryViews { EntryArgs v[MAX_VIEWS]; int n; };

struct BatchTab {
  float position[BATCH_MAX][4], right[BATCH_MAX][4], up[BATCH_MAX][4], forward[BATCH_MAX][4];
  float light[BATCH_MAX][4];
};

struct LaunchCfg {
  int trace_blocks;
  int shade_blocks;
  int rays_per_lane;
  int min_blocks;
  int variant;
  int far;
  int packet;
  int packet_blocks;
};

size_t raygen_block_count(int width, int rows, uint32_t spp, int batch_k);
void launch_raygen(const SceneDev& sc, const FrameDev& f, const UniformsDev& u, const BatchTab& bt, hipStream_t s);
size_t jitter_table_elems(int width, int rows, uint32_t spp);
void launch_jitter_table(const FrameDev& f, uint32_t spp, float2* table, hipStream_t s);
void launch_trace_closest(const SceneDev& sc, const FrameDev& f, int bounce, bool counting, const LaunchCfg& cfg, hipStream_t s);
void launch_beam_shade(const SceneDev& sc, const FrameDev& f, const UniformsDev& u, const LaunchCfg& cfg, hipStream_t s);
void launch_entry(const SceneDev& sc, const EntryViews& a, hipStream_t s);
void launch_blob(const SceneDev& sc, const EntryArgs& e, const FrameDev& f, bool counting, hipStream_t s);
void launch_tile(const SceneDev& sc, const FrameDev& f, const UniformsDev& u, bool counting, hipStream_t s);
void launch_tail(const SceneDev& sc, const FrameDev& f, const UniformsDev& u, const BatchTab& bt, int first_bounce, bool counting, const LaunchCfg& cfg, int tail_blocks, hipStream_t s);
void launch_shade(const SceneDev& sc, const FrameDev& f, const UniformsDev& u, const BatchTab& bt, int bounce, const LaunchCfg& cfg, hipStream_t s);
void launch_beam_shadow(const SceneDev& sc, const FrameDev& f, const UniformsDev& u, bool counting, const LaunchCfg& cfg, hipStream_t s);
void launch_trace_shadow(const SceneDev& sc, const FrameDev& f, bool counting, const LaunchCfg& cfg, hipStream_t s);
void launch_resolve(const FrameDev& f, const UniformsDev& u, hipStream_t s);
void launch_cover(const SceneDev& sc, const CoverViews& a, uint32_t max_boxes_per_instance, uint32_t* mask_block, hipStream_t s);
void launch_query(const SceneDev& sc, const float4* rays, HitRec* out, uint32_t n, int32_t* ovf_stack, uint32_t* counters, bool any_hit,
                  bool counting, const LaunchCfg& cfg, hipStream_t s);
void launch_hit_attr(const SceneDev& sc, const HitRec* hits, float4* attr, uint32_t n, hipStream_t s);
void launch_query_flags(const SceneDev& sc, const float4* rays, const uint32_t* words, uint32_t query_word, HitRec* out, uint32_t n,
                        int32_t* ovf_stack, uint32_t* counters, const LaunchCfg& cfg, hipStream_t s);
void launch_hit_kind(const SceneDev& sc, const float4* rays, const HitRec* hits, float4* attr, uint32_t n, hipStream_t s);
void launch_query_hits(const SceneDev& sc, const float4* rays, const uint32_t* words, uint32_t query_word, uint32_t n, uint32_t k, HitRec* hits,
                       float4* attr, uint32_t* counts, int32_t* ovf_stack, uint32_t* counters, const LaunchCfg& cfg, hipStream_t s);
void launch_closest_scale(const SceneDev& sc, float* inst_scale, hipStream_t s);
void launch_closest_point(const SceneDev& sc, const float4* points, uint32_t cull_mask, const float* inst_scale, HitRec* hits, uint32_t n, int32_t* ovf_stack,
                          uint32_t* counters, bool counting, const LaunchCfg& cfg, hipStream_t s);
void launch_closest_side(const SceneDev& sc, const float4* points, const HitRec* hits, float4* attr, uint32_t n, hipStream_t s);
void launch_overlap_boxes(const SceneDev& sc, const float4* boxes, uint32_t cull_mask, const float* inst_scale, bool any, uint32_t k, void* ids, uint32_t* counts,
                          uint32_t n, int32_t* ovf_stack, uint32_t* counters, bool counting, const LaunchCfg& cfg, hipStream_t s);
void launch_sweep_spheres(const SceneDev& sc, const float4* sweeps, uint32_t cull_mask, const float* inst_scale, HitRec* hits, uint32_t n, int32_t* ovf_stack,
                          uint32_t* counters, bool counting, const LaunchCfg& cfg, hipStream_t s);
void launch_sweep_side(const SceneDev& sc, const float4* sweeps, const HitRec* hits, float4* attr, uint32_t n, hipStream_t s);
void launch_point_inside(const SceneDev& sc, const float4* points, uint32_t cull_mask, uint32_t n_dirs, uint32_t* words, uint32_t* counts, uint32_t n,
                         int32_t* ovf_stack, uint32_t* counters, bool counting, const LaunchCfg& cfg, hipStream_t s);
void launch_sign_distance(const float4* points, const uint32_t* words, HitRec* hits, uint32_t n, hipStream_t s);
uint32_t ray_ingest_block_count(uint32_t n);
void launch_ray_ingest(const SceneDev& sc, const FrameDev& f, const float4* rays, uint32_t n, hipStream_t s);
// ... 11 lines not shown
```

Before: 34860.

## Finish pixels inside beam shading and resolve only flagged pixels

Adds a per-pixel resum flag buffer so pixels whose samples are all final get written directly in the beam-shade kernel, and the resolve pass re-sums only the flagged pixels. With no materials it writes a provisional lit color at shade time, so the shadow kernel only overwrites occluded samples and skips the sh_c store and load. It also replaces the per-pixel divide by a reciprocal multiply for power-of-two sample counts. The cost is extra flag writes and more control flow, plus correctness risk in the new bookkeeping.

```diff
diff --git a/vulkan_raytracing_amd/api.py b/vulkan_raytracing_amd/api.py
--- a/vulkan_raytracing_amd/api.py
+++ b/vulkan_raytracing_amd/api.py
@@ -331,6 +331,14 @@
     def set_timing(self, on):
         self._chk(self.L.rt_set_timing(self.h, int(on)), "rt_set_timing")
 
+    def debug_resum_words(self):
+        got = C.c_size_t(0)
+        self.L.rt_debug_snapshot(self.h, 100, _p(np.zeros(1, np.uint8)), 0, C.byref(got))
+        a = np.zeros(got.value // 4, np.uint32)
+        if a.nbytes:
+            self._chk(self.L.rt_debug_snapshot(self.h, 100, _p(a), a.nbytes, C.byref(got)), "rt_debug_snapshot")
+        return a
+
     def set_param(self, name, value):
         self._chk(self.L.rt_set_param(self.h, name.encode(), int(value)), "rt_set_param")
         if name in ("output_rgba8", "output_bgra8"):
diff --git a/vulkan_raytracing_amd/csrc/kernels.hip b/vulkan_raytracing_amd/csrc/kernels.hip
--- a/vulkan_raytracing_amd/csrc/kernels.hip
+++ b/vulkan_raytracing_amd/csrc/kernels.hip
@@ -322,13 +322,19 @@
   return mk3(div255(__builtin_fmaf(rb, wv, ra * iv)), div255(__builtin_fmaf(gb, wv, ga * iv)), div255(__builtin_fmaf(bb, wv, ba * iv)));
 }
 
-__device__ __forceinline__ void store_pixel(const FrameDev& f, uint32_t p, float4 px) {
+template <typename F>
+__device__ __forceinline__ void store_pixel(const F& f, uint32_t p, float4 px) {
   if (f.out_rgba8) {
     auto q = [](float v) -> unsigned char { v = fminf(fmaxf(v, 0.0f), 1.0f); return (unsigned char)(v * 255.0f + 0.5f); };
     reinterpret_cast<uchar4*>(f.out)[p] = f.out_rgba8 == 2 ? make_uchar4(q(px.z), q(px.y), q(px.x), q(px.w)) : make_uchar4(q(px.x), q(px.y), q(px.z), q(px.w));
   } else {
     f.out[p] = px;
   }
+}
+__device__ __forceinline__ float4 sample_mean(float r, float g, float b, float al, uint32_t spp) {
+  const float nn = (float)spp;
+  if ((spp & (spp - 1u)) == 0u) { const float inv = 1.0f / nn; return make_float4(r * inv, g * inv, b * inv, al * inv); }
+  return make_float4(r / nn, g / nn, b / nn, al / nn);
 }
 constexpr float PIXEL_DONE = 2.0f;
 
@@ -661,7 +667,6 @@
     F3 right = mk3(u.right[0], u.right[1], u.right[2]), up = mk3(u.up[0], u.up[1], u.up[2]), fwd = mk3(u.forward[0], u.forward[1], u.forward[2]);
     if (f.batch_k > 1) { right = mk3(bt.right[fi][0], bt.right[fi][1], bt.right[fi][2]); up = mk3(bt.up[fi][0], bt.up[fi][1], bt.up[fi][2]); fwd = mk3(bt.forward[fi][0], bt.forward[fi][1], bt.forward[fi][2]); }
     const uint32_t fy = frame_row(f, ly);
-    const float nn = (float)spp;
     float r = 0.f, g = 0.f, b = 0.f, al = 0.f;
     if (gridDim.z == 1u) {
       float4 col = make_float4(0.f, 0.f, 0.f, 0.f);
@@ -684,7 +689,7 @@
         r += c.x; g += c.y; b += c.z; al += 1.0f;
       }
     }
-    store_pixel(f, fi * f.out_frame_stride + ly * (uint32_t)f.width + x, make_float4(r / nn, g / nn, b / nn, al / nn));
+    store_pixel(f, fi * f.out_frame_stride + ly * (uint32_t)f.width + x, sample_mean(r, g, b, al, spp));
     return;
   }
 #ifdef RT_ALT_KERNELS
@@ -762,16 +767,16 @@
   if (fuse) {
     bool all = true;
     for (uint32_t w = 0; w < blockDim.y; w++) all = all && ((s_miss[w] >> lane) & 1ull) != 0ull;
+    const uint32_t p = ly * (uint32_t)f.width + x;
     if (all) {
       if (threadIdx.y == 0) {
         float r = 0.f, g = 0.f, b = 0.f, al = 0.f;
         for (uint32_t w = 0; w < blockDim.y; w++) { const float4 c = s_col[w][lane]; r += c.x; g += c.y; b += c.z; al += c.w; }
-        const float nn = (float)spp;
-        const uint32_t p = ly * (uint32_t)f.width + x;
-        store_pixel(f, fi * f.out_frame_stride + p, make_float4(r / nn, g / nn, b / nn, al / nn));
-        st_stream(&f.sample_color[fi * spp * npx1 + p], make_float4(0.f, 0.f, 0.f, PIXEL_DONE));
+        store_pixel(f, fi * f.out_frame_stride + p, sample_mean(r, g, b, al, spp));
+        if (f.resum == nullptr) st_stream(&f.sample_color[fi * spp * npx1 + p], make_float4(0.f, 0.f, 0.f, PIXEL_DONE));
       }
     } else if (missed) st_stream(&f.sample_color[sid], miss_col);
+    if (f.resum != nullptr && threadIdx.y == 0 && live) f.resum[p] = all ? 0u : 1u;
   }
   if (survive || run_tile) {
     const uint32_t v = shard * f.shard_cap + slot;
@@ -808,6 +813,9 @@
     const uint32_t* sh_e;
     const uint32_t* ray_words;
   };
+  uint32_t* resum;
+  uint32_t frame_pixels;
+  int provisional_lit;
 };
 
 constexpr int MODE_CLOSEST = 0;
@@ -927,13 +935,25 @@
       const int2 k = s_outq[wave][lane];
       if (MODE == MODE_CLOSEST) { st_stream(&a.hit_a[k.x], r); st_stream(&a.hit_inst[k.x], k.y); }
       else if (MODE == MODE_SHADOW) {
-        float cr = 0.08f, cg = 0.24f, cb = 0.08f;
-        if (r.x != 0.0f || a.sc.n_materials != 0) {
-          const float4 shc = ld_stream(&a.sh_c[(uint32_t)k.y]);
-          if (r.x != 0.0f) { cr = shc.x; cg = shc.y; cb = shc.z; }
-          else { const F3 amb = ambient_of(a.sc, __float_as_uint(shc.w)); cr = amb.x; cg = amb.y; cb = amb.z; }
+        const bool lit = r.x != 0.0f;
+        if (a.provisional_lit) {
+          if (!lit) st_stream(&a.sample_color[(uint32_t)k.x], make_float4(0.08f, 0.24f, 0.08f, 1.0f));
+        } else {
+          float cr = 0.08f, cg = 0.24f, cb = 0.08f;
+          if (lit || a.sc.n_materials != 0) {
+            const float4 shc = ld_stream(&a.sh_c[(uint32_t)k.y]);
+            if (lit) { cr = shc.x; cg = shc.y; cb = shc.z; }
+            else { const F3 amb = ambient_of(a.sc, __float_as_uint(shc.w)); cr = amb.x; cg = amb.y; cb = amb.z; }
+          }
+          st_stream(&a.sample_color[(uint32_t)k.x], make_float4(cr, cg, cb, 1.0f));
         }
-        st_stream(&a.sample_color[(uint32_t)k.x], make_float4(cr, cg, cb, 1.0f));
+        uint32_t* const resum = a.resum;
+        if (!lit && resum != nullptr) {
+          const uint32_t npx = a.frame_pixels;
+          uint32_t p = (uint32_t)k.x;
+          for (int t = 0; t < 3; t++) p = p >= npx ? p - npx : p;
+          resum[p] = 1u;
+        }
       }
       else { HitRec h; h.t = r.x; h.u = r.y; h.v = r.z; h.prim = (int)__float_as_uint(r.w); h.inst = k.y; a.raw_out[k.x] = h; }
     }
@@ -1332,8 +1352,12 @@
   if constexpr (PIN) asm volatile("" : "+v"(r));
   return make_float4(r, 0.24f, r, 1.0f);
 }
+constexpr uint32_t SLOT_NONE = 0u;
+constexpr uint32_t SLOT_FINAL = 1u;
+constexpr uint32_t SLOT_PROVISIONAL = 2u;
 template <bool TILE, bool BATCH, bool RUNS, bool REG, typename A>
-__device__ __forceinline__ void shade_slot(const A& a, const int bounce, const uint32_t shard, const uint32_t q, const bool in_range, const int inst_r, const float4 h_r) {
+__device__ __forceinline__ void shade_slot(const A& a, const int bounce, const uint32_t shard, const uint32_t q, const bool in_range, const int inst_r, const float4 h_r,
+                                           const uint32_t row_r, const bool defer, float* const out_r) {
   const auto& f = a.f;
   const auto& U = a.u;
   const int cur = bounce & 1, nxt = cur ^ 1;
@@ -1344,6 +1368,11 @@
   uint32_t sh_ent = ENTRY_FROM_ROOT;
   uint32_t sid = SID_DEAD;
   int inst = HIT_DEAD;
+  if (REG && defer) out_r[192] = __uint_as_float(SLOT_NONE);
+  auto put_final = [&](const float4 c) {
+    if (REG && defer) { out_r[0] = c.x; out_r[64] = c.y; out_r[128] = c.z; out_r[192] = __uint_as_float(SLOT_FINAL); }
+    else st_stream(&f.sample_color[sid], c);
+  };
   if (in_range) { if constexpr (REG) inst = inst_r; else inst = ld_stream(&f.hit_inst[q]); }
   if (inst != HIT_DEAD) {
     const float4 rd = ld_stream(&f.ray_d[cur][q]);
@@ -1351,7 +1380,7 @@
     const F3 d = mk3(rd.x, rd.y, rd.z);
     if (inst < 0) {
       const F3 c = sample_sky(a.sc, mk3(d.x, d.y, -d.z));
-      st_stream(&f.sample_color[sid], make_float4(c.x, c.y, c.z, 1.0f));
+      put_final(make_float4(c.x, c.y, c.z, 1.0f));
     } else {
       float4 h = h_r;
       if constexpr (!REG) h = ld_stream(&f.hit_a[q]);
@@ -1372,7 +1401,7 @@
       const bool last = (uint32_t)bounce >= U.max_bounce_count;
       if (type == 0u) {
         if (dot3(d, N) >= 0.0f) {
-          st_stream(&f.sample_color[sid], ambient_default<REG>());
+          put_final(ambient_default<REG>());
         } else {
           no = fma3(0.01f, N, P);
           F3 light = mk3(U.light_position[0], U.light_position[1], U.light_position[2]);
@@ -1386,7 +1415,7 @@
           const float NdotL = dot3(N, L), NdotH = dot3(N, Hh);
           const float dl = fmaxf(0.0f, NdotL);
           const float sp = M ? pow_int(fmaxf(0.0f, NdotH), (uint32_t)M->ns) : pow100(fmaxf(0.0f, NdotH));
-          const uint32_t i = sid / (uint32_t)(f.rows * f.width) - fi * U.samples_per_pixel;
+          const uint32_t i = (REG && U.samples_per_pixel <= 4u) ? row_r : sid / (uint32_t)(f.rows * f.width) - fi * U.samples_per_pixel;
           float w = 1.0f;
           for (uint32_t k = 0; k < i; k++) w = w * 0.9f;
           const F3 kd = M ? mk3(M->kd[0], M->kd[1], M->kd[2]) : mk3(0.2f, 1.0f, 0.2f);
@@ -1399,10 +1428,10 @@
           push_shadow = true;
           if (f.settle_dead_shadow_rays && __float_as_uint(sh_c.x) == __float_as_uint(amb.x) && __float_as_uint(sh_c.y) == __float_as_uint(amb.y) &&
               __float_as_uint(sh_c.z) == __float_as_uint(amb.z)) {
-            st_stream(&f.sample_color[sid], make_float4(amb.x, amb.y, amb.z, 1.0f));
+            put_final(make_float4(amb.x, amb.y, amb.z, 1.0f));
             push_shadow = false; settled = true;
           }
-          if (f.light_entry != nullptr) {
+          if (push_shadow && f.light_entry != nullptr) {
             const F3 v = sub3(no, light);
             const float ax = __builtin_fabsf(v.x), ay = __builtin_fabsf(v.y), az = __builtin_fabsf(v.z);
             const int axis = (ax >= ay && ax >= az) ? 0 : (ay >= az ? 1 : 2);
@@ -1446,7 +1475,7 @@
       }
       if (push_next && last) {
         push_next = false;
-        st_stream(&f.sample_color[sid], ambient_default<REG>());
+        put_final(ambient_default<REG>());
       }
     }
   }
@@ -1456,6 +1485,10 @@
       __hip_atomic_fetch_add(f.counters + cnt_tail(Q_SHADOW0, (int)shard), (uint32_t)__builtin_popcountll(m_st), __ATOMIC_RELAXED, __HIP_MEMORY_SCOPE_AGENT);
       __hip_atomic_fetch_add(f.counters + cnt_work(Q_DEAD, (int)shard), (uint32_t)__builtin_popcountll(m_st), __ATOMIC_RELAXED, __HIP_MEMORY_SCOPE_AGENT);
     }
+  }
+  if (push_shadow) {
+    if (REG && defer) { out_r[0] = sh_c.x; out_r[64] = sh_c.y; out_r[128] = sh_c.z; out_r[192] = __uint_as_float(SLOT_PROVISIONAL); }
+    else if (f.provisional_lit) st_stream(&f.sample_color[sid], make_float4(sh_c.x, sh_c.y, sh_c.z, 1.0f));
   }
   const uint32_t slot_n = wave_alloc(push_next, f.counters + cnt_tail(bounce + 1, (int)shard));
   if (push_next) {
@@ -1480,7 +1513,7 @@
       const uint32_t v = f.sh_base + shard * f.shard_cap + slot_s;
       st_stream(&f.sh_o[v], make_float4(no.x, no.y, no.z, sh_tmax));
       st_stream(&f.sh_d[v], make_float4(nd.x, nd.y, nd.z, __uint_as_float(sid)));
-      st_stream(&f.sh_c[v], make_float4(sh_c.x, sh_c.y, sh_c.z, sh_w));
+      if (!f.provisional_lit) st_stream(&f.sh_c[v], make_float4(sh_c.x, sh_c.y, sh_c.z, sh_w));
       if (f.sh_e != nullptr) f.sh_e[v] = sh_ent;
     }
   }
@@ -1512,7 +1545,7 @@
     for (int t = 0; t < N_SHARDS; t++) n = (shard == (uint32_t)t) ? cnt[t] : n;
     if (base >= n) continue;
     const uint32_t q = shard * f.shard_cap + ((TILE && pass) ? f.shard_cap - n : 0u) + base + lane;
-    shade_slot<TILE, BATCH, RUNS, false>(a, bounce, shard, q, base + lane < n, HIT_DEAD, make_float4(0.f, 0.f, 0.f, 0.f));
+    shade_slot<TILE, BATCH, RUNS, false>(a, bounce, shard, q, base + lane < n, HIT_DEAD, make_float4(0.f, 0.f, 0.f, 0.f), 0u, false, nullptr);
   }
   }
 }
@@ -1580,14 +1613,13 @@
     if (!tile_is_sky(f, fi, blockIdx.x, by, trow * gridDim.x + blockIdx.x) && x < (uint32_t)f.width && ly < (uint32_t)f.rows) {
       const uint32_t p1 = ly * (uint32_t)f.width + x;
       const size_t s0 = (size_t)fi * u.samples_per_pixel * npx1 + p1;
-      if (f.sample_color[s0].w != PIXEL_DONE) {
+      if (f.resum != nullptr ? f.resum[p1] != 0u : f.sample_color[s0].w != PIXEL_DONE) {
         float r = 0.f, g = 0.f, b = 0.f, al = 0.f;
         for (uint32_t i = 0; i < u.samples_per_pixel; i++) {
           const float4 c = ld_stream(&f.sample_color[s0 + (size_t)i * npx1]);
           r += c.x; g += c.y; b += c.z; al += c.w;
         }
-        const float nn = (float)u.samples_per_pixel;
-        store_pixel(f, fi * f.out_frame_stride + p1, make_float4(r / nn, g / nn, b / nn, al / nn));
+        store_pixel(f, fi * f.out_frame_stride + p1, sample_mean(r, g, b, al, u.samples_per_pixel));
       }
     }
   }
@@ -1770,6 +1802,7 @@
   a.u.light_intensity = u.light_intensity;
   a.u.max_bounce_count = u.max_bounce_count; a.u.samples_per_pixel = u.samples_per_pixel;
   a.u.center_object_type = u.center_object_type; a.u.orbiting_object_type = u.orbiting_object_type;
+  a.out = f.out; a.out_rgba8 = f.out_rgba8; a.provisional_lit = f.provisional_lit; a.resum = f.resum;
   hipLaunchKernelGGL(k_beam_shade, dim3(cfg.trace_blocks), dim3(256), 0, s, a, (uint32_t)f.pixel_runs);
 }
 
@@ -1784,6 +1817,7 @@
   TraceArgs a = make_args(sc, f.counters, Q_SHADOW, f.shard_cap, f.ovf_stack);
   a.ray_o = f.sh_o + f.sh_base; a.ray_d = f.sh_d + f.sh_base; a.sh_c = f.sh_c + f.sh_base;
   a.sample_color = f.sample_color;
+  a.resum = f.resum; a.frame_pixels = (uint32_t)(f.rows * f.width); a.provisional_lit = f.provisional_lit;
 #ifdef RT_ALT_KERNELS
   if (cfg.packet != 0 && cfg.variant == 0) {
     const bool le = f.light_entry != nullptr && f.sh_e != nullptr;
diff --git a/vulkan_raytracing_amd/csrc/kernels_beam.inc b/vulkan_raytracing_amd/csrc/kernels_beam.inc
--- a/vulkan_raytracing_amd/csrc/kernels_beam.inc
+++ b/vulkan_raytracing_amd/csrc/kernels_beam.inc
@@ -52,6 +52,10 @@
   const EntryRec* light_entry;
   int width, rows, light_tiles, settle_dead_shadow_rays;
   BeamShadeUniforms u;
+  float4* out;
+  int out_rgba8;
+  int provisional_lit;
+  uint32_t* resum;
 };
 struct BeamShadeFrame {
   float4* ray_o[2]; float4* ray_d[2];
@@ -61,6 +65,7 @@
   const EntryRec* light_entry;
   uint32_t shard_cap;
   int width, rows, light_tiles, settle_dead_shadow_rays;
+  int provisional_lit;
   static constexpr int pixel_runs = 64;
   static constexpr uint32_t sh_base = 0u;
 };
@@ -300,14 +305,44 @@
       const BeamShadeArgs* ka = (const BeamShadeArgs*)__builtin_amdgcn_kernarg_segment_ptr();
       asm volatile("" : "+s"(ka));
       const BeamShadeFrame sf{{const_cast<float4*>(ka->ray_o), ka->next_o}, {const_cast<float4*>(ka->ray_d), ka->next_d}, ka->sh_o, ka->sh_d, ka->sh_c, ka->sh_e, ka->sample_color,
-                              ka->counters, ka->light_entry, ka->shard_cap, ka->width, ka->rows, ka->light_tiles, ka->settle_dead_shadow_rays};
+                              ka->counters, ka->light_entry, ka->shard_cap, ka->width, ka->rows, ka->light_tiles, ka->settle_dead_shadow_rays, ka->provisional_lit};
       const BeamShadeView sv{ka->sc, sf, ka->u};
+      const uint32_t npx = (uint32_t)(sf.rows * sf.width);
+      const bool defer = ka->resum != nullptr;
 #pragma nounroll
       for (uint32_t j = 0; j < S; j++) {
         const float tj = j == 0u ? bt0 : (j == 1u ? bt1 : (j == 2u ? bt2 : bt3));
-        const float* const b = bst + 256u * j;
+        float* const b = bst + 256u * j;
         const int ij = (alive >> j) & 1u ? __float_as_int(b[192]) : HIT_DEAD;
-        shade_slot<false, false, false, true>(sv, 0, run_shard, v0 + 64u * j, true, ij, make_float4(tj, b[0], b[64], b[128]));
+        shade_slot<false, false, false, true>(sv, 0, run_shard, v0 + 64u * j, true, ij, make_float4(tj, b[0], b[64], b[128]), j, defer, b);
+      }
+      if (defer) {
+        bool resolved = true, provisional = false, any = false;
+        float r = 0.f, g = 0.f, bl = 0.f, al = 0.f;
+        uint32_t p = 0;
+        for (uint32_t j = 0; j < S; j++) {
+          const float* const b = bst + 256u * j;
+          const uint32_t kind = __float_as_uint(b[192]);
+          resolved = resolved && kind != SLOT_NONE;
+          provisional = provisional || kind == SLOT_PROVISIONAL;
+          if (kind != SLOT_NONE) {
+            if (!any) p = __float_as_uint(ld_stream(&sf.ray_d[0][v0 + 64u * j]).w) - j * npx;
+            any = true;
+            r += b[0]; g += b[64]; bl += b[128]; al += 1.0f;
+          }
+        }
+        const BeamShadeArgs* kf = (const BeamShadeArgs*)__builtin_amdgcn_kernarg_segment_ptr();
+        asm volatile("" : "+s"(kf));
+        if (resolved) {
+          const struct { float4* out; int out_rgba8; } of{kf->out, kf->out_rgba8};
+          store_pixel(of, p, sample_mean(r, g, bl, al, kf->u.samples_per_pixel));
+          kf->resum[p] = 0u;
+        }
+        if (any && (!resolved || provisional))
+          for (uint32_t j = 0; j < S; j++) {
+            const float* const b = bst + 256u * j;
+            if (__float_as_uint(b[192]) != SLOT_NONE) st_stream(&kf->sample_color[j * npx + p], make_float4(b[0], b[64], b[128], 1.0f));
+          }
       }
     } else {
 #define RT_BEAM_OUT(j) if (j < S) { \
diff --git a/vulkan_raytracing_amd/csrc/rt_api.cpp b/vulkan_raytracing_amd/csrc/rt_api.cpp
--- a/vulkan_raytracing_amd/csrc/rt_api.cpp
+++ b/vulkan_raytracing_amd/csrc/rt_api.cpp
@@ -173,6 +173,8 @@
   bool out_bgra = false;
   bool async_pending = false;
   int async_w = 0, async_h = 0;
+  const uint32_t* last_resum = nullptr; size_t last_resum_words = 0;
+  uint32_t* d_resum = nullptr;
   uint32_t* d_counters = nullptr;
   int cnt_parity = 0;
   int32_t* d_ovf = nullptr;
@@ -194,6 +196,7 @@
   EntryRec* d_entry = nullptr;
   size_t entry_alloc_tiles = 0;
   int camera_records = 1;
+  int pixel_finish = 1;
   int dead_shadow_rays = 1;
   int shadow_beams = 0;
   bool sh_double = false;
@@ -798,6 +801,9 @@
   c->frame_capacity = 0;
   const size_t sh_cap = (want_double ? 2 : 1) * capacity;
   r = alloc_queues(c, c->frame, capacity, sh_cap, capacity); if (r) return r;
+  if (c->d_resum) { HIP_TRY(c, hipFree(c->d_resum)); c->d_resum = nullptr; c->last_resum = nullptr; c->last_resum_words = 0; }
+  HIP_TRY(c, hipMalloc((void**)&c->d_resum, 2 * capacity * sizeof(uint32_t)));
+  HIP_TRY(c, hipMemset(c->d_resum, 0xFF, 2 * capacity * sizeof(uint32_t)));
   c->sh_double = want_double;
   c->frame_capacity = capacity;
   return RT_OK;
@@ -1037,6 +1043,9 @@
   f.pixel_runs = beam_on ? 64 * (int)std::min<uint32_t>(u.samples_per_pixel, 4u) : 0;
   f.shadow_runs = (beam_on && c->shadow_beams && K == 1 && std::isfinite(u.light_position[0]) && std::isfinite(u.light_position[1]) && std::isfinite(u.light_position[2])) ? 1u : 0u;
   f.sh_base = f.shadow_runs ? (uint32_t)capacity : 0u;
+  f.resum = (c->pixel_finish && K == 1 && u.samples_per_pixel <= 4u && !tile_on) ? c->d_resum + (size_t)c->cnt_parity * c->frame_capacity : nullptr;
+  c->last_resum = f.resum; c->last_resum_words = f.resum ? (size_t)rows * (size_t)W : 0;
+  f.provisional_lit = (c->pixel_finish && sc.n_materials == 0 && !f.shadow_runs && cfg.variant == 0 && cfg.packet == 0) ? 1 : 0;
   if (c->jitter_table && rows > 0) { r = jitter_table_for(c, f, u.samples_per_pixel, s, &f.jitter); if (r) return r; }
   if (!c->timing || c->timed_frames >= 64) { c->ev_used = 0; c->spans.clear(); c->timed_frames = 0; }
   if (c->timing) c->timed_frames++;
@@ -1263,7 +1272,7 @@
   hipSetDevice(c->device);
   wait_queries(c, c);
   hipDeviceSynchronize();
-  void* ptrs[] = {c->d_inst[0], c->d_inst[1], c->d_out_own, c->d_counters, c->d_ovf, c->d_cover_mask, c->d_entry, c->d_light_entry, c->d_fault_total, c->d_tile_blob, c->d_blob_arena, c->d_blob_list};
+  void* ptrs[] = {c->d_inst[0], c->d_inst[1], c->d_out_own, c->d_resum, c->d_counters, c->d_ovf, c->d_cover_mask, c->d_entry, c->d_light_entry, c->d_fault_total, c->d_tile_blob, c->d_blob_arena, c->d_blob_list};
   for (void* p : ptrs) if (p) hipFree(p);
   free_queues(c->frame);
   free_queues(c->shade);
@@ -1712,6 +1721,7 @@
   if (k == "pixel_beams") { c->pixel_beams = value != 0; return RT_OK; }
   if (k == "fused_shade") { c->fused_shade = value != 0; return RT_OK; }
   if (k == "camera_records") { c->camera_records = value != 0; return RT_OK; }
+  if (k == "pixel_finish") { c->pixel_finish = value != 0; return RT_OK; }
   if (k == "dead_shadow_rays") { c->dead_shadow_rays = value != 0; return RT_OK; }
   if (k == "shadow_beams") {
     if (value != 0 && !alt_kernels_built()) return fail(c, RT_ERR_INVALID_ARGUMENT, "shadow_beams is not in the product library (measured slower): build librt_mi355x_alt.so with `make alt` and load it (RT_LIB_VARIANT=alt)");
@@ -1829,13 +1839,21 @@
 int rt_debug_snapshot(rt_ctx* c, int what, void* out, size_t capacity_bytes, size_t* bytes) {
   if (!c) return RT_ERR_INVALID_ARGUMENT;
   if (!out) return fail(c, RT_ERR_INVALID_ARGUMENT, "rt_debug_snapshot: out is NULL");
-  if (what < 0 || what > 8) return fail(c, RT_ERR_INVALID_ARGUMENT, "rt_debug_snapshot: what must be 0..8");
+  if ((what < 0 || what > 8) && what != 100) return fail(c, RT_ERR_INVALID_ARGUMENT, "rt_debug_snapshot: what must be 0..8 or 100");
   Scene* S = c->scene;
   if (!c->tlas_valid || !S->blas_linked || !S->arrays_ready) return fail(c, RT_ERR_NOT_READY, "rt_debug_snapshot: the context has no valid TLAS (rt_set_instances)");
   { int q = quiesce_scene(c); if (q) return q; }
   HIP_TRY(c, hipSetDevice(c->device));
   HIP_TRY(c, hipStreamSynchronize(c->stream));
   if (c->tgpu.stream) HIP_TRY(c, hipStreamSynchronize(c->tgpu.stream));
+  if (what == 100) {
+    if (c->frame_pending) HIP_TRY(c, hipStreamSynchronize(c->frame_stream));
+    const size_t need = c->last_resum_words * sizeof(uint32_t);
+    if (bytes) *bytes = need;
+    if (need > capacity_bytes) return fail(c, RT_ERR_INVALID_ARGUMENT, "rt_debug_snapshot: the buffer holds " + std::to_string(capacity_bytes) + " bytes, item 100 needs " + std::to_string(need));
+    if (need) HIP_TRY(c, hipMemcpy(out, c->last_resum, need, hipMemcpyDeviceToHost));
+    return RT_OK;
+  }
   const int par = c->parity;
   const size_t tlas_nodes = c->batch_k > 1 ? (size_t)c->batch_k * (size_t)c->tlas_stride[par] : (size_t)c->tlas_node_count[par];
   size_t n_cover = 0;
diff --git a/vulkan_raytracing_amd/csrc/rt_kernels.h b/vulkan_raytracing_amd/csrc/rt_kernels.h
--- a/vulkan_raytracing_amd/csrc/rt_kernels.h
+++ b/vulkan_raytracing_amd/csrc/rt_kernels.h
@@ -72,6 +72,8 @@
   int pixel_runs;
   uint32_t shadow_runs;
   uint32_t sh_base;
+  uint32_t* resum;
+  int provisional_lit;
 };
 
 struct CoverArgs {
```

After: 35080 (median of 6 runs). No clear change (+0.6%).
